# rojas-diego/tokengeex

Measured on AMD Instinct MI355X. Metric: MB/s raw bytes encoded (and tokens/s) at 32K/64K vocab, 1/2/4/8 GPUs, higher is better.
Workload: dtype f64

## Files before the change

include/tgx.h:

```cpp
#ifndef TGX_H
#define TGX_H

#include <stddef.h>
#include <stdint.h>

#ifdef __cplusplus
extern "C" {
#endif

#define TGX_ABI_VERSION 1

typedef enum tgx_status {
    TGX_OK = 0,
    TGX_ERR_IO = 1,
    TGX_ERR_JSON = 2,
    TGX_ERR_TOKEN_ID_OOB = 3,
    TGX_ERR_NO_PATH = 4,
    TGX_ERR_DEVICE = 5,
    TGX_ERR_Z_NOT_NORMAL = 6,
    TGX_ERR_INVALID = 7,
    TGX_ERR_UNSUPPORTED = 8
} tgx_status;

#define TGX_MAX_TOKEN_LEN 64
// ... 180 lines not shown
const void *tgx_text_bytes_device(const tgx_text *t);
const void *tgx_text_offsets_device(const tgx_text *t);
void tgx_text_free(tgx_text *t);
tgx_status tgx_corpus_from_text(const tgx_text *t, tgx_corpus **out);
tgx_status tgx_decode_rows_host(const uint8_t *vocab_bytes, const uint64_t *vocab_offs, uint32_t vocab_size,
                                const uint8_t *special_bytes, const uint64_t *special_offs, uint32_t n_specials,
                                const void *ids, uint32_t id_kind, const uint64_t *id_offs, uint64_t n_rows,
                                uint64_t row_len, const uint8_t *mask, const int32_t *lengths, uint32_t skip_id,
                                int include_special, uint8_t **out_text, uint64_t *out_offs, uint64_t *n_replaced,
                                uint64_t *bad_sample, uint64_t *bad_id);

#define TGX_SPAN_CHARS 8u
tgx_status tgx_result_spans_device(tgx_model *m, const tgx_result *r, const uint8_t *special_bytes,
                                   const uint64_t *special_offs, uint32_t n_specials, uint32_t flags, void *stream,
                                   void *d_spans);
tgx_status tgx_result_pad_spans_device(tgx_model *m, const tgx_result *r, const uint8_t *special_bytes,
                                       const uint64_t *special_offs, uint32_t n_specials, uint32_t row_len,
                                       uint32_t bos_id, uint32_t eos_id, uint32_t flags, void *stream, void *d_spans);
tgx_status tgx_spans_host(const uint8_t *vocab_bytes, const uint64_t *vocab_offs, uint32_t vocab_size,
                          const uint8_t *special_bytes, const uint64_t *special_offs, uint32_t n_specials,
                          const uint32_t *ids, const uint64_t *offs, uint64_t n_rows, uint32_t row_len,
                          uint32_t bos_id, uint32_t eos_id, uint32_t flags, void *out);

tgx_status tgx_corpus_upload(int device, const uint8_t *text, const uint64_t *offs,
                             uint64_t n_samples, tgx_corpus **out);
void tgx_corpus_free(tgx_corpus *c);
uint64_t tgx_corpus_num_samples(const tgx_corpus *c);
uint64_t tgx_corpus_num_bytes(const tgx_corpus *c);

tgx_status tgx_encode_corpus(tgx_model *m, tgx_corpus *c, double dropout, uint64_t seed,
                             tgx_result **out);

double tgx_sample_u01(uint64_t seed, uint64_t sample, uint64_t pos, uint32_t len);
tgx_status tgx_encode_batch_sample(tgx_model *m, const uint8_t *text, const uint64_t *offs,
                                   uint64_t n_samples, double alpha, uint64_t seed,
                                   double *logz, tgx_result **out);
tgx_status tgx_encode_corpus_sample(tgx_model *m, tgx_corpus *c, double alpha, uint64_t seed,
                                    double *logz, tgx_result **out);

#define TGX_MAX_NBEST 16
tgx_status tgx_encode_batch_nbest(tgx_model *m, const uint8_t *text, const uint64_t *offs, uint64_t n_samples,
                                  uint32_t nbest, double *scores, uint32_t *n_found, tgx_result **out);
tgx_status tgx_encode_corpus_nbest(tgx_model *m, tgx_corpus *c, uint32_t nbest,
                                   double *scores, uint32_t *n_found, tgx_result **out);

tgx_status tgx_count_tokens(tgx_model *m, tgx_corpus *c, uint64_t *freq);

tgx_status tgx_count_pairs(tgx_model *m, tgx_corpus *c, uint64_t **keys, uint64_t **counts,
                           uint64_t *n_pairs);
tgx_status tgx_count_pairs_top(tgx_model *m, tgx_corpus *c, uint64_t max_pairs, uint64_t **keys,
                               uint64_t **counts, uint64_t *n_pairs, uint64_t *n_total);

tgx_status tgx_estep(tgx_model *m, tgx_corpus *c, uint64_t snippet_len, double dropout,
                     uint64_t seed, double *expected, double *logz_sum);

void tgx_free(void *p);
void tgx_pool_trim(int device);
void *tgx_host_alloc(uint64_t bytes);
void tgx_host_free(void *p);

double tgx_digamma(double x);
tgx_status tgx_prune_m_step(const double *expected, const uint8_t *keep, uint32_t vocab_size,
                            uint32_t *out_idx, double *out_score, uint32_t *out_n);
tgx_status tgx_prune_alternatives(const tgx_flat_trie *trie, const uint8_t *bytes, const uint64_t *offs,
                                  const double *scores, uint32_t vocab_size, uint8_t *always_keep,
                                  uint32_t *alt_offs, uint32_t **alt_ids);
tgx_status tgx_model_prune_alternatives(const tgx_model *m, uint8_t *always_keep, uint32_t *alt_offs, uint32_t **alt_ids);
tgx_status tgx_prune_select(const uint64_t *freq, const uint8_t *keep, const uint8_t *always_keep,
                            const uint32_t *alt_offs, const uint32_t *alt_ids, const double *scores,
                            uint32_t vocab_size, uint64_t n_samples, uint32_t pruned_size,
                            uint32_t *out_idx, uint32_t *out_n);

int tgx_last_kernel_times(const tgx_model *m, const char **names, float *ms, int cap);
uint64_t tgx_last_algorithmic_bytes(const tgx_model *m);
uint32_t tgx_last_encode_waves_per_cu(const tgx_model *m);
uint64_t tgx_last_encode_redo_samples(const tgx_model *m);
uint64_t tgx_last_encode_long_samples(const tgx_model *m);
uint64_t tgx_last_estep_pieces(const tgx_model *m);
uint64_t tgx_last_estep_redo(const tgx_model *m);
uint32_t tgx_last_encode_corun_cus(const tgx_model *m);
uint32_t tgx_encode_corun_timeouts(const tgx_model *m);
uint32_t tgx_model_score_values(const tgx_model *m);
uint32_t tgx_last_encode_hot_values(const tgx_model *m);

static inline double tgx_dropout_u01(uint64_t seed, uint64_t sample, uint64_t pos, uint32_t len) {
    uint64_t x = seed ^ (sample * 0x9E3779B97F4A7C15ULL) ^ (pos * 0xC2B2AE3D27D4EB4FULL) ^
                 ((uint64_t)len * 0x165667B19E3779F9ULL);
    x ^= x >> 30;
    x *= 0xBF58476D1CE4E5B9ULL;
    x ^= x >> 27;
    x *= 0x94D049BB133111EBULL;
    x ^= x >> 31;
    return (double)(x >> 11) * (1.0 / 9007199254740992.0);
}

#ifdef __cplusplus
}
#endif
#endif
```

tokengeex_amd/_lib.py:

```python
from __future__ import annotations

import ctypes as C
import os

import numpy as np

_HERE = os.path.dirname(os.path.abspath(__file__))
LIB_PATH = os.path.join(_HERE, "libtgx.so")

OK, ERR_IO, ERR_JSON, ERR_TOKEN_ID_OOB, ERR_NO_PATH, ERR_DEVICE, ERR_Z_NOT_NORMAL, ERR_INVALID, \
    ERR_UNSUPPORTED = range(9)
MAX_TOKEN_LEN = 64
MAX_NBEST = 16
ESTEP_SNIPPET_LEN = 81920
NO_ID = 0xFFFFFFFF
LAYOUT_PAD_LEFT, LAYOUT_TRUNC_LEFT, LAYOUT_I64 = 1, 2, 4
FRONT_CRLF = 1
SPAN_CHARS = 8

_vp, _u64, _u32, _i, _d = C.c_void_p, C.c_uint64, C.c_uint32, C.c_int, C.c_double
_pvp, _pu64 = C.POINTER(C.c_void_p), C.POINTER(C.c_uint64)
SYMBOLS = {
    "tgx_last_error": (C.c_char_p, []),
    "tgx_last_error_detail": (None, [_pu64, _pu64, _pu64]),
    "tgx_abi_version": (_i, []),
    "tgx_device_count": (_i, []),
    "tgx_model_create": (_i, [_vp, _vp, _vp, _u32, _i, _pvp]),
    "tgx_model_create_ex": (_i, [_vp, _vp, _vp, _u32, _i, _u32, _pvp]),
    "tgx_model_create_derived": (_i, [_vp, _vp, _u32, _vp, _u32, _pvp]),
    "tgx_model_destroy": (None, [_vp]),
    "tgx_model_vocab_size": (_u32, [_vp]),
    "tgx_model_max_token_len": (_u32, [_vp]),
    "tgx_model_trie_bytes": (_u64, [_vp]),
    "tgx_model_device": (_i, [_vp]),
    "tgx_common_prefix_search": (_i, [_vp, _vp, _u64, _vp, _vp, _u64, _pu64]),
    "tgx_flat_trie_build": (_i, [_vp, _vp, _vp, _u32, _pvp]),
    "tgx_flat_trie_free": (None, [_vp]),
    "tgx_flat_trie_search": (_u64, [_vp, _vp, _u64, _vp, _vp, _u64]),
    "tgx_flat_trie_search8": (_u64, [_vp, _vp, _vp, _vp, _u32, _vp, _u64, _vp, _vp, _u64, C.POINTER(C.c_uint32), _pu64,
                                     C.POINTER(C.c_double)]),
    "tgx_flat_trie_stats": (None, [_vp, _pu64, _pu64, C.POINTER(C.c_uint32)]),
    "tgx_flat_trie_copy": (None, [_vp, _vp, _vp, _vp]),
    "tgx_tok_hash_selftest": (_i, [_vp, _vp, _u32, C.POINTER(C.c_uint32), _pu64]),
    "tgx_dropout_u01_host": (_d, [_u64, _u64, _u64, _u32]),
    "tgx_encode_batch": (_i, [_vp, _vp, _vp, _u64, _d, _u64, _pvp]),
    "tgx_encode_batch_host": (_i, [_vp, _vp, _vp, _u64, _d, _u64, _vp, _u64, _vp, _pu64]),
    "tgx_encode_batch_multi": (_i, [_vp, _u32, _vp, _vp, _u64, _d, _u64, _vp, _u64, _vp, _pu64]),
    "tgx_result_num_samples": (_u64, [_vp]),
    "tgx_result_num_tokens": (_u64, [_vp]),
    "tgx_result_ids": (_vp, [_vp]),
    "tgx_result_offsets": (_vp, [_vp]),
    "tgx_result_copy_ids": (_i, [_vp, _vp, _u64]),
    "tgx_result_copy_offsets": (_i, [_vp, _vp, _u64]),
    "tgx_result_ids_device": (_vp, [_vp]),
    "tgx_result_offsets_device": (_vp, [_vp]),
    "tgx_result_free": (None, [_vp]),
    "tgx_corpus_upload": (_i, [_i, _vp, _vp, _u64, _pvp]),
    "tgx_corpus_free": (None, [_vp]),
    "tgx_corpus_num_samples": (_u64, [_vp]),
    "tgx_corpus_num_bytes": (_u64, [_vp]),
    "tgx_encode_corpus": (_i, [_vp, _vp, _d, _u64, _pvp]),
    "tgx_count_tokens": (_i, [_vp, _vp, _vp]),
    "tgx_count_pairs": (_i, [_vp, _vp, _pvp, _pvp, _pu64]),
    "tgx_count_pairs_top": (_i, [_vp, _vp, _u64, _pvp, _pvp, _pu64, _pu64]),
    "tgx_estep": (_i, [_vp, _vp, _u64, _d, _u64, _vp, C.POINTER(C.c_double)]),
    "tgx_split_specials": (_i, [_vp, _vp, _u64, _vp, _vp, _u32, _vp, _pvp, _pvp, _pvp, _pu64]),
    "tgx_pack_segments": (_i, [_vp, _vp, _vp, _vp, _u64, _i, _vp, _vp, _pu64]),
    "tgx_normalize_segments": (_i, [_u32, _vp, _vp, _vp, _u64, _pvp, _pvp]),
    "tgx_unidata_version": (C.c_char_p, []),
    "tgx_assemble_ids": (_i, [_vp, _vp, _u64, _vp, _vp, _u32, _vp, _vp]),
    "tgx_decode_batch": (_i, [_vp, _vp, _u32, _vp, _vp, _u32, _vp, _vp, _u64, _i, _pvp, _vp, _pu64, _pu64]),
    "tgx_utf8_lossy": (_u64, [_vp, _u64, _vp]),
    "tgx_substring_df": (_i, [_i, _vp, _u64, _vp, _vp, _vp, _vp, _u64, _u32, _d, _u64, _pvp, _pvp, _pvp, _pu64, _pu64, _pu64]),
    "tgx_substring_df_top": (_i, [_i, _vp, _u64, _vp, _vp, _vp, _vp, _u64, _u32, _d, _u64, _u64, _pvp, _pvp, _pvp, _pu64, _pu64, _pu64,
                                  _pu64, C.POINTER(C.c_uint32)]),
    "tgx_generate_u01": (_d, [_u64, _u64, _u64]),
    "tgx_free": (None, [_vp]),
    "tgx_pool_trim": (None, [_i]),
    "tgx_host_alloc": (_vp, [_u64]),
    "tgx_host_free": (None, [_vp]),
    "tgx_digamma": (_d, [_d]),
    "tgx_prune_m_step": (_i, [_vp, _vp, _u32, _vp, _vp, C.POINTER(C.c_uint32)]),
    "tgx_prune_alternatives": (_i, [_vp, _vp, _vp, _vp, _u32, _vp, _vp, _pvp]),
    "tgx_model_prune_alternatives": (_i, [_vp, _vp, _vp, _pvp]),
    "tgx_prune_select": (_i, [_vp, _vp, _vp, _vp, _vp, _vp, _u32, _u64, _u32, _vp, C.POINTER(C.c_uint32)]),
    "tgx_last_kernel_times": (_i, [_vp, C.POINTER(C.c_char_p), C.POINTER(C.c_float), _i]),
    "tgx_last_algorithmic_bytes": (_u64, [_vp]),
    "tgx_last_encode_waves_per_cu": (_u32, [_vp]),
    "tgx_last_encode_redo_samples": (_u64, [_vp]),
    "tgx_model_score_values": (_u32, [_vp]),
    "tgx_last_encode_hot_values": (_u32, [_vp]),
    "tgx_last_encode_long_samples": (_u64, [_vp]),
    "tgx_last_estep_pieces": (_u64, [_vp]),
    "tgx_last_estep_redo": (_u64, [_vp]),
    "tgx_last_encode_corun_cus": (_u32, [_vp]),
    "tgx_encode_corun_timeouts": (_u32, [_vp]),
    "tgx_sample_u01": (_d, [_u64, _u64, _u64, _u32]),
    "tgx_encode_batch_sample": (_i, [_vp, _vp, _vp, _u64, _d, _u64, _vp, _pvp]),
    "tgx_encode_corpus_sample": (_i, [_vp, _vp, _d, _u64, _vp, _pvp]),
    "tgx_encode_batch_nbest": (_i, [_vp, _vp, _vp, _u64, _u32, _vp, _vp, _pvp]),
    "tgx_encode_corpus_nbest": (_i, [_vp, _vp, _u32, _vp, _vp, _pvp]),
    "tgx_result_device": (_i, [_vp]),
    "tgx_result_layout_info": (_i, [_vp, _u32, _u32, _pu64, _pu64]),
    "tgx_result_pad_device": (_i, [_vp, _u32, _u32, _u32, _u32, _u32, _vp, _vp, _vp, _vp, _pu64]),
    "tgx_result_pack_device": (_i, [_vp, _u32, _u32, _u32, _u32, _u32, _vp, _vp, _vp, _vp, _pu64]),
    "tgx_layout_pad_host": (_i, [_vp, _vp, _u64, _u32, _u32, _u32, _u32, _u32, _vp, _vp, _vp, _pu64]),
    "tgx_layout_pack_host": (_i, [_vp, _vp, _u64, _u32, _u32, _u32, _u32, _u32, _vp, _vp, _vp, _pu64]),
    "tgx_assemble_result": (_i, [_vp, _vp, _vp, _vp, _u64, _u32, _pvp]),
    "tgx_result_vocab_size": (_u32, [_vp]),
    "tgx_assemble_host": (_i, [_vp, _vp, _u64, _vp, _vp, _u64, _u32, _u32, _vp, _u64, _vp]),
    "tgx_decode_result": (_i, [_vp, _vp, _vp, _vp, _u32, _i, _vp, _pvp, _pu64, _pu64]),
    "tgx_decode_padded": (_i, [_vp, _vp, _u64, _u64, _u32, _vp, _vp, _u32, _vp, _vp, _u32, _i, _vp, _pvp, _pu64, _pu64]),
    "tgx_text_num_rows": (_u64, [_vp]),
    "tgx_text_num_bytes": (_u64, [_vp]),
    "tgx_text_num_replaced": (_u64, [_vp]),
    "tgx_text_device": (_i, [_vp]),
    "tgx_text_copy_bytes": (_i, [_vp, _vp, _u64]),
    "tgx_text_copy_offsets": (_i, [_vp, _vp, _u64]),
    "tgx_text_bytes_device": (_vp, [_vp]),
    "tgx_text_offsets_device": (_vp, [_vp]),
    "tgx_text_free": (None, [_vp]),
    "tgx_corpus_from_text": (_i, [_vp, _pvp]),
    "tgx_decode_rows_host": (_i, [_vp, _vp, _u32, _vp, _vp, _u32, _vp, _u32, _vp, _u64, _u64, _vp, _vp, _u32, _i, _pvp, _vp, _pu64,
                                  _pu64, _pu64]),
    "tgx_result_spans_device": (_i, [_vp, _vp, _vp, _vp, _u32, _u32, _vp, _vp]),
    "tgx_result_pad_spans_device": (_i, [_vp, _vp, _vp, _vp, _u32, _u32, _u32, _u32, _u32, _vp, _vp]),
    "tgx_spans_host": (_i, [_vp, _vp, _u32, _vp, _vp, _u32, _vp, _vp, _u64, _u32, _u32, _u32, _u32, _vp]),
    "tgx_result_window_info": (_i, [_vp, _u32, _u32, _u32, _u32, _u32, _pu64]),
    "tgx_result_window_pad_device": (_i, [_vp, _u32, _u32, _u32, _u32, _u32, _u32, _vp, _u64, _vp, _vp, _vp, _vp, _vp]),
    "tgx_result_window_spans_device": (_i, [_vp, _vp, _vp, _vp, _u32, _u32, _u32, _u32, _u32, _u32, _vp, _u64, _vp]),
    "tgx_layout_windows_host": (_i, [_vp, _vp, _u64, _u32, _u32, _u32, _u32, _u32, _u32, _u64, _vp, _vp, _vp, _vp, _vp, _pu64]),
    "tgx_window_spans_host": (_i, [_vp, _vp, _u32, _vp, _vp, _u32, _vp, _vp, _u64, _u32, _u32, _u32, _u32, _u32, _u64, _vp, _pu64]),
    "tgx_corpus_split_specials": (_i, [_vp, _vp, _vp, _u32, _u32, _pvp, _pvp]),
    "tgx_plan_num_samples": (_u64, [_vp]),
    "tgx_plan_num_segments": (_u64, [_vp]),
    "tgx_plan_num_encoded": (_u64, [_vp]),
    "tgx_plan_device": (_i, [_vp]),
    "tgx_plan_copy": (_i, [_vp, _vp, _u64, _vp, _u64]),
    "tgx_plan_free": (None, [_vp]),
    "tgx_assemble_result_plan": (_i, [_vp, _vp, _vp, _u32, _pvp]),
    "tgx_front_last_times": (_i, [C.POINTER(C.c_char_p), C.POINTER(C.c_float), _i]),
    "tgx_corpus_copy_text": (_i, [_vp, _vp, _u64]),
    "tgx_corpus_copy_offsets": (_i, [_vp, _vp, _u64]),
    "tgx_front_host": (_i, [_vp, _vp, _u64, _vp, _vp, _u32, _u32, _vp, _pvp, _pu64, _pvp, _pvp, _pu64]),
}


class TokenGeeXError(Exception):

    def __init__(self, message: str, status: int = -1, sample: int | None = None,
                 pos: int | None = None, length: int | None = None):
        super().__init__(message)
        self.status, self.sample, self.pos, self.length = status, sample, pos, length


def _share_torch_hip_runtime() -> None:
    import sys
    if os.environ.get("TGX_HIP_RUNTIME", "") == "system" or "torch" in sys.modules:
        return
    import importlib.util
    try:
        spec = importlib.util.find_spec("torch")
    except (ImportError, ValueError):
        return
    for root in (spec.submodule_search_locations or []) if spec else []:
        path = os.path.join(root, "lib", "libamdhip64.so")
        if os.path.exists(path):
            try:
                C.CDLL(path, mode=C.RTLD_GLOBAL)
            except OSError:
                pass
            return


# ... 880 lines not shown
        scores = np.empty(max(n * int(nbest), 1), np.float64)
        n_found = np.empty(max(n, 1), np.uint32)
        h = C.c_void_p()
        check(lib.tgx_encode_batch_nbest(self._h, ptr(flat) if flat.size else None, ptr(offs), n, int(nbest), ptr(scores),
                                         ptr(n_found), C.byref(h)))
        return NativeResult(h), scores[:n * int(nbest)], n_found[:n]

    def encode_corpus_nbest(self, corpus: NativeCorpus, nbest: int):
        n = corpus.num_samples
        scores = np.empty(max(n * int(nbest), 1), np.float64)
        n_found = np.empty(max(n, 1), np.uint32)
        h = C.c_void_p()
        check(lib.tgx_encode_corpus_nbest(self._h, corpus._h, int(nbest), ptr(scores), ptr(n_found), C.byref(h)))
        return NativeResult(h), scores[:n * int(nbest)], n_found[:n]

    def count_tokens(self, corpus: NativeCorpus, freq: np.ndarray | None = None) -> np.ndarray:
        if freq is None:
            freq = np.zeros(self.vocab_size, np.uint64)
        assert freq.dtype == np.uint64 and freq.shape[0] == self.vocab_size and freq.flags.c_contiguous
        check(lib.tgx_count_tokens(self._h, corpus._h, ptr(freq)))
        return freq

    def count_pairs(self, corpus: NativeCorpus) -> tuple[np.ndarray, np.ndarray]:
        keys, counts, n = C.c_void_p(), C.c_void_p(), C.c_uint64()
        check(lib.tgx_count_pairs(self._h, corpus._h, C.byref(keys), C.byref(counts), C.byref(n)))
        k = n.value
        ka = np.ctypeslib.as_array(C.cast(keys, C.POINTER(C.c_uint64)), shape=(max(k, 1),))[:k].copy()
        ca = np.ctypeslib.as_array(C.cast(counts, C.POINTER(C.c_uint64)), shape=(max(k, 1),))[:k].copy()
        lib.tgx_free(keys)
        lib.tgx_free(counts)
        return ka, ca

    def count_pairs_top(self, corpus: NativeCorpus, max_pairs: int) -> tuple[np.ndarray, np.ndarray, int]:
        keys, counts, n, tot = C.c_void_p(), C.c_void_p(), C.c_uint64(), C.c_uint64()
        check(lib.tgx_count_pairs_top(self._h, corpus._h, int(max_pairs), C.byref(keys), C.byref(counts),
                                      C.byref(n), C.byref(tot)))
        k = n.value
        ka = np.ctypeslib.as_array(C.cast(keys, C.POINTER(C.c_uint64)), shape=(max(k, 1),))[:k].copy()
        ca = np.ctypeslib.as_array(C.cast(counts, C.POINTER(C.c_uint64)), shape=(max(k, 1),))[:k].copy()
        lib.tgx_free(keys)
        lib.tgx_free(counts)
        return ka, ca, tot.value

    def estep(self, corpus: NativeCorpus, snippet_len: int = ESTEP_SNIPPET_LEN, dropout: float = 0.0,
              seed: int = 0, expected: np.ndarray | None = None) -> tuple[np.ndarray, float]:
        if expected is None:
            expected = np.zeros(self.vocab_size, np.float64)
        assert expected.dtype == np.float64 and expected.shape[0] == self.vocab_size
        z = C.c_double()
        check(lib.tgx_estep(self._h, corpus._h, snippet_len, float(dropout), seed & (2**64 - 1),
                            ptr(expected), C.byref(z)))
        return expected, z.value

    def common_prefix_search(self, s: bytes) -> list[tuple[int, int]]:
        buf = np.frombuffer(s, dtype=np.uint8)
        cap = len(s) + 1
        ids, lens = np.zeros(cap, np.uint32), np.zeros(cap, np.uint32)
        cnt = C.c_uint64()
        check(lib.tgx_common_prefix_search(self._h, ptr(buf) if len(s) else None, len(s), ptr(ids),
                                           ptr(lens), cap, C.byref(cnt)))
        return [(int(ids[i]), int(lens[i])) for i in range(cnt.value)]

    def last_kernel_times(self) -> dict[str, float]:
        names = (C.c_char_p * 8)()
        ms = (C.c_float * 8)()
        n = lib.tgx_last_kernel_times(self._h, names, ms, 8)
        return {names[i].decode(): float(ms[i]) for i in range(n)}

    def last_algorithmic_bytes(self) -> int:
        return lib.tgx_last_algorithmic_bytes(self._h)

    def last_encode_waves_per_cu(self) -> int:
        return lib.tgx_last_encode_waves_per_cu(self._h)

    def last_encode_redo_samples(self) -> int:
        return lib.tgx_last_encode_redo_samples(self._h)

    def score_values(self) -> int:
        return lib.tgx_model_score_values(self._h)

    def last_encode_hot_values(self) -> int:
        return lib.tgx_last_encode_hot_values(self._h)

    def last_encode_long_samples(self) -> int:
        return lib.tgx_last_encode_long_samples(self._h)

    def last_estep_pieces(self) -> int:
        return lib.tgx_last_estep_pieces(self._h)

    def last_estep_redo(self) -> int:
        return lib.tgx_last_estep_redo(self._h)

    def last_encode_corun_cus(self) -> int:
        return lib.tgx_last_encode_corun_cus(self._h)

    def encode_corun_timeouts(self) -> int:
        return lib.tgx_encode_corun_timeouts(self._h)


class FlatTrie:

    def __init__(self, tokens: list[bytes], scores):
        flat, offs = pack(tokens)
        sc = np.ascontiguousarray(scores, dtype=np.float64)
        h = C.c_void_p()
        check(lib.tgx_flat_trie_build(ptr(flat) if flat.size else None, ptr(offs), ptr(sc), len(tokens),
                                      C.byref(h)))
        self._h = h
        self._flat, self._offs, self._sc = flat, offs, sc

    def common_prefix_search8(self, s: bytes, max_hot: int = 6600):
        buf = np.frombuffer(s, dtype=np.uint8)
        cap = len(s) + 1
        ids, lens = np.zeros(cap, np.uint32), np.zeros(cap, np.uint32)
        nh, nc, cov = C.c_uint32(), C.c_uint64(), C.c_double()
        k = lib.tgx_flat_trie_search8(self._h, ptr(self._flat) if self._flat.size else None, ptr(self._offs), ptr(self._sc),
                                      max_hot, ptr(buf) if len(s) else None, len(s), ptr(ids), ptr(lens), cap,
                                      C.byref(nh), C.byref(nc), C.byref(cov))
        if k == 2**64 - 1:
            raise TokenGeeXError("8-byte records need fewer than 2^23 slots")
        return [(int(ids[i]), int(lens[i])) for i in range(k)], {"n_hot": nh.value, "n_cold": nc.value, "hot_coverage": cov.value}

    def __del__(self):
        if getattr(self, "_h", None):
            lib.tgx_flat_trie_free(self._h)
            self._h = None

    def common_prefix_search(self, s: bytes) -> list[tuple[int, int]]:
        buf = np.frombuffer(s, dtype=np.uint8)
        cap = len(s) + 1
        ids, lens = np.zeros(cap, np.uint32), np.zeros(cap, np.uint32)
        k = lib.tgx_flat_trie_search(self._h, ptr(buf) if len(s) else None, len(s), ptr(ids), ptr(lens), cap)
        return [(int(ids[i]), int(lens[i])) for i in range(k)]

    def stats(self) -> dict:
        a, b, c = C.c_uint64(), C.c_uint64(), C.c_uint32()
        lib.tgx_flat_trie_stats(self._h, C.byref(a), C.byref(b), C.byref(c))
        return {"n_slots": a.value, "n_nodes": b.value, "max_token_len": c.value,
                "fill": b.value / max(1, a.value)}

    @property
    def max_token_len(self) -> int:
        return self.stats()["max_token_len"]

    def table(self):
        n = self.stats()["n_slots"]
        check, base, tokid = np.zeros(n, np.uint32), np.zeros(n, np.uint32), np.zeros(n, np.uint32)
        lib.tgx_flat_trie_copy(self._h, ptr(check), ptr(base), ptr(tokid))
        return check, base, tokid


    def prune_alternatives(self, tokens: list[bytes], scores) -> tuple[np.ndarray, np.ndarray, np.ndarray]:
        flat, offs = pack(tokens)
        sc = np.ascontiguousarray(scores, dtype=np.float64)
        V = len(tokens)
        always_keep = np.zeros(V, np.uint8)
        alt_offs = np.zeros(V + 1, np.uint32)
        p = C.c_void_p()
        check(lib.tgx_prune_alternatives(self._h, ptr(flat) if flat.size else None, ptr(offs), ptr(sc), V,
                                         ptr(always_keep), ptr(alt_offs), C.byref(p)))
        k = int(alt_offs[V])
        ids = np.ctypeslib.as_array(C.cast(p, C.POINTER(C.c_uint32)), shape=(max(k, 1),))[:k].copy()
        lib.tgx_free(p)
        return always_keep, alt_offs, ids


# ... 58 lines not shown
```

tokengeex_amd/build.py:

```python
from __future__ import annotations

import os
import shutil
import subprocess
import sys

HERE = os.path.dirname(os.path.abspath(__file__))
CSRC = os.path.join(HERE, "csrc")
OUT = os.path.join(HERE, "libtgx.so")
SOURCES = ["kernels.hip", "estep.hip", "encode2.hip", "encode4l.hip", "encode5.hip", "estep4.hip", "estep4l.hip", "estep7.hip", "cuts.hip", "pairs.hip", "generate.hip", "sample.hip", "nbest.hip", "layout.hip", "assemble.hip", "decode.hip", "spans.hip", "front.hip", "tgx_api.cpp", "host_twins.cpp", "trie_build.cpp", "prune_host.cpp", "frontback.cpp", "unicode_norm.cpp"]
HEADERS = ["api_internal.h", "kernels.h", "sample.h", "nbest.h", "layout.h", "assemble.h", "decode.h", "spans.h", "front.h", "device_common.h", "trace_body.h", "trie_build.h", "unicode_tables.h", os.path.join("..", "..", "include", "tgx.h")]
ARCH = "gfx950"


def _hipcc() -> str:
    for cand in (os.environ.get("HIPCC"), shutil.which("hipcc"), "/opt/rocm/bin/hipcc"):
        if cand and os.path.exists(cand):
            return cand
    raise RuntimeError("hipcc not found")


def needs_build() -> bool:
    if not os.path.exists(OUT):
        return True
    t = os.path.getmtime(OUT)
    deps = [os.path.join(CSRC, f) for f in SOURCES + HEADERS] + [os.path.abspath(__file__)]
    return any(os.path.getmtime(d) > t for d in deps)


SYNTH_OUT = os.path.join(HERE, "libtgx_synth.so")


def build_synth(force: bool = False) -> str:
    src = os.path.join(CSRC, "synth_gen.c")
    if not force and os.path.exists(SYNTH_OUT) and os.path.getmtime(SYNTH_OUT) >= os.path.getmtime(src):
        return SYNTH_OUT
    subprocess.check_call(["gcc", "-O2", "-std=c11", "-fPIC", "-shared", "-o", SYNTH_OUT + ".tmp", src, "-lm"])
    os.replace(SYNTH_OUT + ".tmp", SYNTH_OUT)
    return SYNTH_OUT


FAST_OUT = os.path.join(HERE, "_tgxfast.so")


def build_pyfast(force: bool = False) -> str:
    import sysconfig
    src = os.path.join(CSRC, "pyfast.c")
    if not force and os.path.exists(FAST_OUT) and os.path.getmtime(FAST_OUT) >= os.path.getmtime(src):
        return FAST_OUT
    inc = sysconfig.get_paths()["include"]
    subprocess.check_call(["gcc", "-O2", "-std=c11", "-fPIC", "-shared", "-pthread", "-I", inc, "-o", FAST_OUT + ".tmp", src])
    os.replace(FAST_OUT + ".tmp", FAST_OUT)
    return FAST_OUT


def build(force: bool = False, verbose: bool = False) -> str:
    from concurrent.futures import ThreadPoolExecutor
    build_synth(force)
    build_pyfast(force)
    if not force and not needs_build():
        return OUT
    objdir = os.path.join(CSRC, "build")
    os.makedirs(objdir, exist_ok=True)
    hdr_time = max(os.path.getmtime(os.path.join(CSRC, h)) for h in HEADERS)
    hdr_time = max(hdr_time, os.path.getmtime(os.path.abspath(__file__)))
    flags = [f"--offload-arch={ARCH}", "-O3", "-std=c++17", "-fPIC",
             "-ffp-contract=off",
             "-munsafe-fp-atomics",
             "-Wall", "-Wno-unused-result", "-Wno-pass-failed", "-x", "hip"]
    flags += os.environ.get("TGX_EXTRA_HIPCC_FLAGS", "").split()
    jobs = []
    objs = []
    for s in SOURCES:
        src = os.path.join(CSRC, s)
        obj = os.path.join(objdir, s + ".o")
        objs.append(obj)
        if force or not os.path.exists(obj) or os.path.getmtime(obj) < max(os.path.getmtime(src), hdr_time):
            jobs.append([_hipcc()] + flags + ["-c", src, "-o", obj])

    def run(cmd):
        if verbose:
            print(" ".join(cmd), flush=True)
        subprocess.check_call(cmd)

    with ThreadPoolExecutor(max_workers=min(6, max(1, len(jobs)))) as ex:
        list(ex.map(run, jobs))
    link = [_hipcc(), f"--offload-arch={ARCH}", "-shared", "-fPIC"] + objs + ["-o", OUT + ".tmp", "-Wl,-rpath,/opt/rocm/lib"]
    if verbose:
        print(" ".join(link), flush=True)
    subprocess.check_call(link)
    os.replace(OUT + ".tmp", OUT)
    return OUT


# ... 3 lines not shown
```

tokengeex_amd/csrc/device_common.h:

```cpp
#pragma once
#include <hip/hip_runtime.h>
#include <stdint.h>

namespace tgx {

__device__ __forceinline__ uint32_t readlane_u32(uint32_t v, uint32_t lane) {
    return (uint32_t)__builtin_amdgcn_readlane((int)v, (int)lane);
}
__device__ __forceinline__ uint64_t readlane_u64(uint64_t v, uint32_t lane) {
    uint32_t lo = readlane_u32((uint32_t)v, lane);
    uint32_t hi = readlane_u32((uint32_t)(v >> 32), lane);
    return ((uint64_t)hi << 32) | lo;
}
__device__ __forceinline__ double readlane_f64(double v, uint32_t lane) {
    return __longlong_as_double((long long)readlane_u64((uint64_t)__double_as_longlong(v), lane));
}
__device__ __forceinline__ uint64_t first_u64(uint64_t v) {
    uint32_t lo = (uint32_t)__builtin_amdgcn_readfirstlane((int)(uint32_t)v);
    uint32_t hi = (uint32_t)__builtin_amdgcn_readfirstlane((int)(uint32_t)(v >> 32));
    return ((uint64_t)hi << 32) | lo;
}
__device__ __forceinline__ uint64_t rotl64(uint64_t x, uint32_t r) {
    r &= 63u;
    return (x << r) | (x >> ((64u - r) & 63u));
}

__device__ __forceinline__ double dropout_u01(uint64_t seed, uint64_t sample, uint64_t pos, uint32_t len) {
    uint64_t x = seed ^ (sample * 0x9E3779B97F4A7C15ULL) ^ (pos * 0xC2B2AE3D27D4EB4FULL) ^
                 ((uint64_t)len * 0x165667B19E3779F9ULL);
    x ^= x >> 30;
    x *= 0xBF58476D1CE4E5B9ULL;
    x ^= x >> 27;
    x *= 0x94D049BB133111EBULL;
    x ^= x >> 31;
    return (double)(x >> 11) * (1.0 / 9007199254740992.0);
}

template <class T>
__device__ __forceinline__ T lds_ld(uint32_t off) { return *(const __attribute__((address_space(3))) T*)(uintptr_t)off; }
template <class T>
__device__ __forceinline__ void lds_st(uint32_t off, T v) { *(__attribute__((address_space(3))) T*)(uintptr_t)off = v; }

typedef uint32_t u32x2_t __attribute__((ext_vector_type(2)));
typedef uint32_t u32x4_t __attribute__((ext_vector_type(4)));
__device__ __forceinline__ __amdgpu_buffer_rsrc_t make_rsrc(const void* base, uint32_t bytes) {
    return __builtin_amdgcn_make_buffer_rsrc(const_cast<void*>(base), 0, (int)bytes, 0x00020000);
}
__device__ __forceinline__ uint2 buf_ld8(__amdgpu_buffer_rsrc_t rs, uint32_t off) {
    const u32x2_t v = __builtin_amdgcn_raw_buffer_load_b64(rs, (int)off, 0, 0);
    return make_uint2(v.x, v.y);
}
__device__ __forceinline__ double buf_ld_f64(__amdgpu_buffer_rsrc_t rs, uint32_t off) {
    const u32x2_t v = __builtin_amdgcn_raw_buffer_load_b64(rs, (int)off, 0, 0);
    return __hiloint2double((int)v.y, (int)v.x);
}


constexpr uint32_t kFront = 2;
__host__ __device__ inline uint32_t wave_lds_entries(uint32_t lm) { return 64u * lm + 64u + kFront; }
__host__ __device__ inline uint32_t wave_lds_bytes(uint32_t lm) {
    return wave_lds_entries(lm) * 12u + 128u;
}

__device__ __forceinline__ uint32_t sel_u32(uint64_t mask, uint32_t t, uint32_t f) {
    uint32_t r;
    asm("v_cndmask_b32_e64 %0, %1, %2, %3" : "=v"(r) : "v"(f), "v"(t), "s"(mask));
    return r;
}
template <int IMM>
__device__ __forceinline__ uint32_t sel_imm_u32(uint64_t mask, uint32_t f) {
    uint32_t r;
    asm("v_cndmask_b32_e64 %0, %1, %2, %3" : "=v"(r) : "v"(f), "n"(IMM), "s"(mask));
    return r;
}
__device__ __forceinline__ double sel_f64(uint64_t mask, double t, double f) {
    const uint64_t tb = (uint64_t)__double_as_longlong(t), fb = (uint64_t)__double_as_longlong(f);
    const uint32_t lo = sel_u32(mask, (uint32_t)tb, (uint32_t)fb);
    const uint32_t hi = sel_u32(mask, (uint32_t)(tb >> 32), (uint32_t)(fb >> 32));
    return __longlong_as_double((long long)(((uint64_t)hi << 32) | lo));
}


template <int CTRL>
__device__ __forceinline__ uint32_t row_bcast_u32(uint32_t v) {
    return (uint32_t)__builtin_amdgcn_update_dpp(0, (int)v, CTRL, 0xF, 0xF, false);
}
template <int U>
__device__ __forceinline__ double row_bcast_f64(double v) {
    double r;
    asm volatile("s_nop 1\n\tv_mov_b64_dpp %0, %1 row_newbcast:%2 row_mask:0xf bank_mask:0xf"
                 : "=v"(r) : "v"(v), "n"(U));
    return r;
}

constexpr uint64_t kRowLane0 = 0x0001000100010001ULL;

__device__ __forceinline__ uint64_t wave_fetch_add(unsigned long long* counter, uint32_t n) {
    uint64_t got, saved;
    const uint64_t inc = n;
    const uint32_t zero = 0;
    asm volatile(
        "s_mov_b64 %1, exec\n\t"
        "s_mov_b64 exec, 1\n\t"
        "global_atomic_add_x2 %0, %2, %3, %4 sc0\n\t"
        "s_mov_b64 exec, %1\n\t"
        "s_waitcnt vmcnt(0)"
        : "=&v"(got), "=&s"(saved) : "v"(zero), "v"(inc), "s"(counter) : "memory");
    const uint32_t lo = (uint32_t)__builtin_amdgcn_readfirstlane((int)(uint32_t)got);
    const uint32_t hi = (uint32_t)__builtin_amdgcn_readfirstlane((int)(uint32_t)(got >> 32));
    return ((uint64_t)hi << 32) | lo;
}

__device__ __forceinline__ uint64_t claim_rows(unsigned long long* queue, bool need_new, uint32_t r) {
    const uint64_t want = __builtin_amdgcn_ballot_w64(need_new) & kRowLane0;
    uint64_t k = ~0ull;
    if (want != 0) {
        const uint64_t base = wave_fetch_add(queue, (uint32_t)__builtin_popcountll(want));
        if (need_new) k = base + (uint64_t)__builtin_popcountll(want & ((1ull << (r * 16u)) - 1ull));
    }
    return k;
}

__device__ __forceinline__ uint64_t claim_rows_chunk(unsigned long long* queue, bool need_new, uint32_t r, uint32_t chunk) {
    const uint64_t want = __builtin_amdgcn_ballot_w64(need_new) & kRowLane0;
    uint64_t k = ~0ull;
    if (want != 0) {
        const uint64_t base = wave_fetch_add(queue, (uint32_t)__builtin_popcountll(want) * chunk);
        if (need_new) k = base + (uint64_t)__builtin_popcountll(want & ((1ull << (r * 16u)) - 1ull)) * chunk;
    }
    return k;
}

__device__ __forceinline__ uint4 load_rec(const uint4* __restrict__ trie, uint32_t t) {
    uint4 r = trie[t];
    asm volatile("" : "+v"(r.x), "+v"(r.y), "+v"(r.z), "+v"(r.w));
    return r;
}

__device__ __forceinline__ uint64_t bp8_base(uint64_t beg, uint32_t s) { return (beg + 128ull * s) & ~3ull; }
__device__ __forceinline__ uint32_t bp8_perm(uint32_t j) { return (j & ~63u) | ((j & 15u) << 2) | ((j >> 4) & 3u); }


constexpr uint32_t kNoStep = 0xFFu;

template <int U>
__device__ __forceinline__ void relax4_step(double sv, double& acc, uint32_t& bpv, uint32_t& fin, uint32_t& fhi) {
    constexpr uint64_t MU = kRowLane0 << U;
    const double best = row_bcast_f64<U>(acc);
    fin = sel_u32(MU, bpv, fin);
    fhi = sel_u32(MU, (uint32_t)((uint64_t)__double_as_longlong(acc) >> 32), fhi);
    const double cand = best + sv;
    const uint64_t take = __builtin_amdgcn_fcmp(cand, acc, 2 ) | MU;
    acc = sel_f64(take, cand, acc);
    bpv = sel_imm_u32<U>(take, bpv);
}

template <int U>
__device__ __forceinline__ void relax5_step(double sv, double& acc, uint32_t& bpv, uint32_t& fin, uint32_t& fhi) {
    constexpr uint64_t MU = kRowLane0 << U;
    const double best = row_bcast_f64<U>(acc);
    fin = sel_u32(MU, bpv, fin);
    fhi = sel_u32(MU, (uint32_t)((uint64_t)__double_as_longlong(acc) >> 32), fhi);
    const double acc_r = sel_f64(MU, -__builtin_huge_val(), acc);
    const double cand = best + sv;
    const uint64_t take = __builtin_amdgcn_fcmp(cand, acc_r, 2 );
    asm("v_max_f64 %0, %1, %2" : "=v"(acc) : "v"(acc_r), "v"(cand));
    bpv = sel_imm_u32<U>(take, bpv);
}


__device__ __forceinline__ uint32_t rotl32_dev(uint32_t x, int r) { return __builtin_rotateleft32(x, (uint32_t)r); }
__device__ __forceinline__ uint64_t tok_hash64_dev(uint32_t w0, uint32_t w1, uint32_t w2, uint32_t w3, uint32_t len, uint32_t seed) {
    uint32_t a = (w0 ^ (len << 27) ^ seed) * 0x85EBCA6Bu;
    a ^= a >> 15;
    uint32_t b = a;
    a = (a + w1) * 0xC2B2AE35u;
    a ^= a >> 13;
    b = rotl32_dev(b, 11) ^ a;
    a = (a + w2) * 0x27D4EB2Fu;
    a ^= a >> 16;
    b = rotl32_dev(b, 11) ^ a;
    a = (a + w3) * 0x165667B1u;
    a ^= a >> 15;
    b = rotl32_dev(b, 11) + (w0 ^ rotl32_dev(w1, 8) ^ rotl32_dev(w2, 16) ^ rotl32_dev(w3, 24));
    return ((uint64_t)b << 32) | a;
}


__device__ __forceinline__ uint64_t tok_hash64_long_dev(const uint32_t* w, uint32_t len, uint32_t seed) {
    uint32_t a = (w[0] ^ (len << 27) ^ seed) * 0x85EBCA6Bu;
    a ^= a >> 15;
    uint32_t b = a;
    a = (a + w[1]) * 0xC2B2AE35u;
    a ^= a >> 13;
    b = rotl32_dev(b, 11) ^ a;
    a = (a + w[2]) * 0x27D4EB2Fu;
    a ^= a >> 16;
    b = rotl32_dev(b, 11) ^ a;
    a = (a + w[3]) * 0x165667B1u;
    a ^= a >> 15;
    b = rotl32_dev(b, 11) + (w[0] ^ rotl32_dev(w[1], 8) ^ rotl32_dev(w[2], 16) ^ rotl32_dev(w[3], 24));
    if (len > 16u) {
        a = (a + w[4]) * 0x85EBCA6Bu;
        a ^= a >> 15;
        b = rotl32_dev(b, 11) ^ a;
        a = (a + w[5]) * 0xC2B2AE35u;
        a ^= a >> 13;
        b = rotl32_dev(b, 11) ^ a;
        a = (a + w[6]) * 0x27D4EB2Fu;
        a ^= a >> 16;
        b = rotl32_dev(b, 11) ^ a;
        a = (a + w[7]) * 0x165667B1u;
        a ^= a >> 15;
        b = rotl32_dev(b, 11) + (w[4] ^ rotl32_dev(w[5], 8) ^ rotl32_dev(w[6], 16) ^ rotl32_dev(w[7], 24));
    }
    return ((uint64_t)b << 32) | a;
}


__device__ __forceinline__ int row_max_exponent(double acc) {
    int e = (acc == 0.0) ? -100000 : __builtin_amdgcn_frexp_exp(acc);
    e = max(e, __builtin_amdgcn_update_dpp(e, e, 0x121, 0xF, 0xF, false));
    e = max(e, __builtin_amdgcn_update_dpp(e, e, 0x122, 0xF, 0xF, false));
    e = max(e, __builtin_amdgcn_update_dpp(e, e, 0x124, 0xF, 0xF, false));
    e = max(e, __builtin_amdgcn_update_dpp(e, e, 0x128, 0xF, 0xF, false));
    return e;
}

template <int U>
__device__ __forceinline__ void e4l_fwd_step(double sv, double& acc, double& fin) {
    constexpr uint64_t MU = kRowLane0 << U;
    fin = sel_f64(MU, acc, fin);
    const double best = row_bcast_f64<U>(acc);
    const double cand = best * sv;
    acc = sel_f64(MU, cand, acc + cand);
}


}
```

tokengeex_amd/csrc/encode5.hip:

```cpp
#include <hip/hip_runtime.h>
#include <stdint.h>

#include <type_traits>

#include "device_common.h"
#include "kernels.h"

namespace tgx {

constexpr uint32_t kE5RowStride = 512;
constexpr uint32_t kE5GroupBytes = 4 * kE5RowStride;

template <int PPL>
struct WalkCtx {
    __amdgpu_buffer_rsrc_t trie;
    uint32_t s, l32;
    double dropout;
    uint64_t seed;
    bool estep_rule = false;
};

struct Res5 {
    __amdgpu_buffer_rsrc_t cold;
    uint32_t tab;
// ... 79 lines not shown
            uint32_t base[PPL], n_alive = 0;
#pragma unroll
            for (int g = 0; g < PPL; ++g) {
                bm[g] = __builtin_amdgcn_ballot_w64(alive[g]);
                base[g] = n_alive;
                n_alive += (uint32_t)__builtin_popcountll(bm[g]);
            }
            if (n_alive <= 64u) {
                pack<1>(W, R, bytes, maxd, wlane, alive, off_cut, bm, base, n_alive);
                return;
            }
            if (PPL >= 3 && n_alive <= 128u) {
                pack<(PPL >= 3 ? 2 : 1)>(W, R, bytes, maxd, wlane, alive, off_cut, bm, base, n_alive);
                return;
            }
#pragma unroll
            for (int g = 0; g < PPL; ++g) rec[g] = buf_ld8(W.trie, alive[g] ? off_cut[g] : 0u);
            Walk5<DROPOUT, LONG, RES, PPL, D + 1, SKIP, 0, PK>::run(W, R, bytes, maxd, pg, wlane, alive, rec, c);
        } else {
            Walk5<DROPOUT, LONG, RES, PPL, D + 1, SKIP, CK, PK>::run(W, R, bytes, maxd, pg, wlane, alive, rec, c);
        }
    }

    template <int P2>
    static __device__ __forceinline__ void pack(const WalkCtx<PPL>& W, Res5& R, const uint32_t (&bytes)[PPL][4], const uint32_t (&maxd)[PPL],
                                                const uint32_t (&wlane)[PPL], const bool (&alive)[PPL], const uint32_t (&off)[PPL],
                                                const uint64_t (&bm)[PPL], const uint32_t (&base)[PPL], uint32_t n_alive) {
        constexpr int Q0 = CK >> 2;
        constexpr int NW = 2 + 4 - Q0;
        const uint32_t lane = __builtin_amdgcn_mbcnt_hi(~0u, __builtin_amdgcn_mbcnt_lo(~0u, 0u));
        uint32_t v2[P2][NW];
#pragma unroll
        for (int t = 0; t < P2; ++t)
#pragma unroll
            for (int i = 0; i < NW; ++i) v2[t][i] = 0u;
#pragma unroll
        for (int g = 0; g < PPL; ++g) {
            const uint32_t cnt = (uint32_t)__builtin_popcountll(bm[g]);
            const uint32_t below = __builtin_amdgcn_mbcnt_hi((uint32_t)(bm[g] >> 32), __builtin_amdgcn_mbcnt_lo((uint32_t)bm[g], 0u));
            const uint32_t dst = (base[g] + (alive[g] ? below : cnt + lane - below)) & 63u;
            uint32_t v[NW];
            v[0] = off[g];
            v[1] = (PK ? wlane[g] : (wlane[g] | W.l32)) | (maxd[g] << 24);
#pragma unroll
            for (int q = Q0; q < 4; ++q) v[2 + q - Q0] = bytes[g][q];
            const uint32_t t = (lane - base[g]) & 63u;
            const bool got = t < cnt;
            const bool hi = base[g] + t >= 64u;
#pragma unroll
            for (int i = 0; i < NW; ++i) {
                const uint32_t x = (uint32_t)__builtin_amdgcn_ds_permute((int)(dst << 2), (int)v[i]);
#pragma unroll
                for (int s2 = 0; s2 < P2; ++s2)
                    if (got && (P2 == 1 || (s2 == 1) == hi)) v2[s2][i] = x;
            }
        }
        WalkCtx<P2> W2{W.trie, W.s, W.l32, W.dropout, W.seed, W.estep_rule};
        uint32_t bytes2[P2][4], maxd2[P2], pg2[P2], wl2[P2], c2[P2];
        bool alive2[P2];
        uint2 rec2[P2];
#pragma unroll
        for (int s2 = 0; s2 < P2; ++s2) {
            alive2[s2] = 64u * (uint32_t)s2 + lane < n_alive;
            wl2[s2] = v2[s2][1] & 0xFFFFFFu;
            maxd2[s2] = v2[s2][1] >> 24;
            pg2[s2] = 0u;
#pragma unroll
            for (int q = 0; q < 4; ++q) bytes2[s2][q] = q < Q0 ? 0u : v2[s2][2 + (q < Q0 ? 0 : q - Q0)];
            c2[s2] = (bytes2[s2][Q0] >> ((CK & 3) * 8)) & 0xFFu;
            rec2[s2] = buf_ld8(W.trie, alive2[s2] ? v2[s2][0] : 0u);
        }
        Walk5<DROPOUT, LONG, RES, P2, CK, SKIP, 0, true>::run(W2, R, bytes2, maxd2, pg2, wl2, alive2, rec2, c2);
    }
};
template <bool DROPOUT, bool LONG, bool RES, int PPL, bool SKIP, int CK, bool PK>
struct Walk5<DROPOUT, LONG, RES, PPL, 16, SKIP, CK, PK> {
    static __device__ __forceinline__ void run(const WalkCtx<PPL>&, Res5& R, const uint32_t (&)[PPL][4], const uint32_t (&)[PPL],
                                               const uint32_t (&)[PPL], const uint32_t (&)[PPL], bool (&)[PPL], uint2 (&)[PPL],
                                               uint32_t (&)[PPL]) {
        if (RES) R.complete();
    }
};

template <int N>
__device__ __forceinline__ void e5_scores_issue(uint32_t tab, const uint32_t (&iw)[8], int first, u32x2_t (&sp)[N]) {
#pragma unroll
    for (int u = 0; u < N; ++u) {
        const int v = first + u;
        const uint32_t a = (v & 1) ? ((iw[v >> 1] >> 16) << 3) : ((iw[v >> 1] & 0xFFFFu) << 3);
        sp[u] = lds_ld<u32x2_t>(tab + a);
    }
}
__device__ __forceinline__ double e5_score_value(const u32x2_t& p) { return __hiloint2double((int)p.y, (int)p.x); }

template <int N>
__device__ __forceinline__ void e5_scores_cold(uint32_t tab, __amdgpu_buffer_rsrc_t cold, const uint32_t (&iw)[8], int first,
                                               uint32_t hot_bytes, double (&sv)[N]) {
    uint32_t a[N];
#pragma unroll
    for (int u = 0; u < N; ++u) {
        const int v = first + u;
        a[u] = (v & 1) ? ((iw[v >> 1] >> 16) << 3) : ((iw[v >> 1] & 0xFFFFu) << 3);
        sv[u] = lds_ld<double>(tab + (a[u] < hot_bytes ? a[u] : 0u));
    }
    static_assert(N == 4 || N == 8, "e5_scores_cold: four or eight values at a time");
    if (N == 8) asm volatile("" : "+v"(sv[0]), "+v"(sv[1]), "+v"(sv[2]), "+v"(sv[3]), "+v"(sv[4 % N]), "+v"(sv[5 % N]), "+v"(sv[6 % N]), "+v"(sv[7 % N]));
    else asm volatile("" : "+v"(sv[0]), "+v"(sv[1]), "+v"(sv[2]), "+v"(sv[3]));
#pragma unroll
    for (int u = 0; u < N; ++u)
        if (a[u] >= hot_bytes) sv[u] = buf_ld_f64(cold, a[u] - hot_bytes);
}

template <bool COLD>
__device__ __forceinline__ double e5_score_one(uint32_t tab, __amdgpu_buffer_rsrc_t cold, uint32_t rank, uint32_t hot_bytes) {
    const uint32_t a = rank << 3;
    double v = lds_ld<double>(tab + ((!COLD || a < hot_bytes) ? a : 0u));
    if (COLD) {
        asm volatile("" : "+v"(v));
        if (a >= hot_bytes) v = buf_ld_f64(cold, a - hot_bytes);
    }
    return v;
}

constexpr uint32_t kE5LongCap = 62;
constexpr uint32_t kE5LongBytes = 8u + kE5LongCap * 4u;
constexpr uint32_t kFarCode = 0x80u;

__device__ __forceinline__ uint32_t e5_winner_len_m1(uint32_t code, uint32_t l) {
    return (code & kFarCode) ? (code & 31u) : ((l - code - 1u) & 15u);
}

template <int U>
__device__ __forceinline__ void relax5l_step(double sv, double& acc, uint32_t& bpv, double& far, uint32_t& fbp, uint32_t& fin, double& fval) {
    constexpr uint64_t MU = kRowLane0 << U;
    fin = sel_u32(MU, bpv, fin);
    fval = sel_f64(MU, acc, fval);
    const double best = row_bcast_f64<U>(acc);
    const double cur = sel_f64(MU, far, acc);
    const uint32_t curbp = sel_u32(MU, fbp, bpv);
    far = sel_f64(MU, -__builtin_huge_val(), far);
    const double cand = best + sv;
    const uint64_t take = __builtin_amdgcn_fcmp(cand, cur, 2 );
    asm("v_max_f64 %0, %1, %2" : "=v"(acc) : "v"(cur), "v"(cand));
    bpv = sel_imm_u32<U>(take, curbp);
}

template <bool DROPOUT>
__device__ __forceinline__ void e5_long_tail(__amdgpu_buffer_rsrc_t trie, const uint8_t* __restrict__ text16, uint32_t rec_x, bool alive,
                                             uint32_t maxd, uint32_t lane, uint32_t g, uint32_t list_off, double dropout, uint64_t seed,
                                             uint32_t s, uint32_t pg) {
    bool more = alive && maxd > 16u;
    if (__builtin_amdgcn_ballot_w64(more) == 0) return;
    struct __attribute__((packed, aligned(1))) Bytes16 { uint32_t w[4]; };
    Bytes16 b{{0u, 0u, 0u, 0u}};
    if (more) b = *reinterpret_cast<const Bytes16*>(text16);
    uint32_t x = rec_x;
#pragma unroll 1
    for (uint32_t d = 16u; d < 32u; ++d) {
        more = more && d < maxd;
        if (__builtin_amdgcn_ballot_w64(more) == 0) break;
        const uint32_t bi = d - 16u;
        const uint32_t word = (bi & 8u) ? ((bi & 4u) ? b.w[3] : b.w[2]) : ((bi & 4u) ? b.w[1] : b.w[0]);
        const uint32_t c = (word >> ((bi & 3u) * 8u)) & 0xFFu;
        const uint2 rec = buf_ld8(trie, more ? ((x ^ (c << 3)) & 0xFFFFFFu) : 0u);
        more = more && (rec.x >> 24) == c;
        const uint32_t rank = rec.y & 0xFFFFu;
        bool term = more && rank != 0u;
        if (DROPOUT) {
            if (term) term = dropout < dropout_u01(seed, s, pg, d + 1u);
        }
        if (term) {
            const uint32_t slot = __hip_atomic_fetch_add((__attribute__((address_space(3))) uint32_t*)(uintptr_t)list_off, 1u, __ATOMIC_RELAXED, __HIP_MEMORY_SCOPE_WORKGROUP);
            if (slot < kE5LongCap) lds_st<uint32_t>(list_off + 8u + slot * 4u, lane | (g << 6) | (d << 8) | (rank << 16));
        }
        x = rec.x;
    }
}

#define E5_STAMP(i)                                                    \
    if (P.stamps) {                                                    \
        __builtin_amdgcn_sched_barrier(0);                             \
        const uint64_t _now = (uint64_t)__builtin_amdgcn_s_memtime(); \
        __builtin_amdgcn_s_waitcnt(0xC07F);                            \
        __builtin_amdgcn_sched_barrier(0);                             \
        seg[i] += _now - t_last;                                       \
        t_last = _now;                                                 \
    }

template <bool DROPOUT, bool COLD, int PPL, bool LONG, int CK = 0>
__global__ __launch_bounds__(1024, (PPL == 1 ? 8 : (PPL == 2 ? 6 : (PPL == 3 ? 4 : 1)))) void encode5_kernel(EncodeParams P, Encode5Params Q) {
    static_assert(!LONG || PPL == 4, "the long-token build runs four positions per lane");
    extern __shared__ __align__(16) unsigned char smem[];
    constexpr uint32_t LM = LONG ? 32 : 16;
    constexpr uint32_t SPAN = 16u * PPL;
    const uint32_t lane = threadIdx.x & 63u;
    const uint32_t l = lane & 15u, r = lane >> 4;
    const uint32_t wave = threadIdx.x >> 6;
    const uint2* __restrict__ trie = reinterpret_cast<const uint2*>(Q.trie8);
    const __amdgpu_buffer_rsrc_t trie_b = make_rsrc(Q.trie8, Q.trie_bytes);
    const uint32_t lds0 = (uint32_t)reinterpret_cast<uintptr_t>(smem);
    double* const score_tab = reinterpret_cast<double*>(smem);
    const uint32_t hot_bytes = 8u * (Q.n_hot + 1u);
    const __amdgpu_buffer_rsrc_t values = make_rsrc(reinterpret_cast<const unsigned char*>(Q.values) + hot_bytes, 8u * (Q.n_values - Q.n_hot));
    const uint2* rootc = reinterpret_cast<const uint2*>(smem + Q.root_off);
    unsigned char* wbase = smem + Q.idx_off + (size_t)wave * (PPL * kE5GroupBytes);
    {
        for (uint32_t i = threadIdx.x; i <= Q.n_hot; i += blockDim.x) score_tab[i] = Q.values[i];
        uint2* rw = reinterpret_cast<uint2*>(smem + Q.root_off);
        for (uint32_t i = threadIdx.x; i < 256u; i += blockDim.x) rw[i] = trie[(Q.root_base & ~255u) + i];
        if (Q.started && threadIdx.x == 0u) __hip_atomic_fetch_add(Q.started, 1u, __ATOMIC_RELAXED, __HIP_MEMORY_SCOPE_SYSTEM);
        __syncthreads();
    }
    const __amdgpu_buffer_rsrc_t cold_values = values;

    uint32_t s = 0, n = 0, p0 = 0;
    uint64_t beg = 0;
    bool live = false, need_new = true;
    const double ninf = -__builtin_huge_val();
    double acc = ninf, far = ninf;
    uint32_t bpv = kNoStep, fbp = kFarCode;
    bool redo = false;
    uint32_t wn[4 * PPL + 1];
    uint32_t pk = 0, pk_j = 0;
    bool pk_dirty = false;
#pragma unroll
    for (int q = 0; q <= 4 * PPL; ++q) wn[q] = 0;
    const uint32_t my_col = r * kE5RowStride + ((l - 1u) & 15u) * 32u;
    const uint32_t wbase_off = lds0 + Q.idx_off + wave * (PPL * kE5GroupBytes);
    const uint32_t wr_off = wbase_off + r * kE5RowStride + l * 2u;
    const uint32_t col_off = wbase_off + my_col;
    const uint32_t list_off = lds0 + Q.list_off + wave * ((kE5LongBytes + 15u) & ~15u);
    uint64_t seg[5] = {0, 0, 0, 0, 0};
    uint64_t t_last = P.stamps ? (uint64_t)__builtin_amdgcn_s_memtime() : 0;
    uint32_t iters = 0;

    uint64_t local_next = 0, local_end = 0;
    for (;;) {
        {
            uint64_t k = ~0ull;
            const bool have_local = need_new && local_next < local_end;
            if (have_local) k = local_next++;
            const uint64_t kc = claim_rows_chunk(P.queue, need_new && !have_local, r, Q.claim_chunk);
            if (need_new && !have_local) {
                k = kc;
                local_next = kc + 1u;
                local_end = kc + Q.claim_chunk;
            }
            if (need_new) {
                live = k < P.n_samples;
                if (live) {
                    s = P.order[k];
                    beg = P.offs[s];
                    n = (uint32_t)(P.offs[s + 1] - beg);
                }
            }
        }
        if (need_new) {
            p0 = 0;
            acc = (l == 0u) ? 0.0 : ninf;
            bpv = kNoStep;
            pk_dirty = false;
            if (LONG) {
                far = ninf;
                fbp = kFarCode;
                redo = false;
            }
        }
        const bool fresh_row = need_new;
        need_new = false;
        if (__builtin_amdgcn_ballot_w64(live) == 0) break;
        iters++;
        E5_STAMP(0)

        const uintptr_t addr = reinterpret_cast<uintptr_t>(P.text + (live ? beg + p0 + l : 0));
        const uint32_t sh = (uint32_t)(addr & 3u);
        const uint32_t* __restrict__ wp = reinterpret_cast<const uint32_t*>(addr & ~uintptr_t(3));
        uint32_t w[4 * PPL + 1];
        if (fresh_row) {
#pragma unroll
            for (int q = 0; q <= 4 * PPL; ++q) w[q] = wp[q];
        } else {
#pragma unroll
            for (int q = 0; q <= 4 * PPL; ++q) w[q] = wn[q];
        }
        uint32_t bytes[PPL][4];
#pragma unroll
        for (int g = 0; g < PPL; ++g)
#pragma unroll
            for (int q = 0; q < 4; ++q) bytes[g][q] = __builtin_amdgcn_alignbyte(w[4 * g + q + 1], w[4 * g + q], sh);

#pragma unroll
        for (int g = 0; g < PPL; ++g) {
            uint4* mine = reinterpret_cast<uint4*>(wbase + g * kE5GroupBytes + my_col);
            mine[0] = make_uint4(0, 0, 0, 0);
            mine[1] = make_uint4(0, 0, 0, 0);
        }
        if (LONG && lane == 0u) lds_st<uint32_t>(list_off, 0u);
        __builtin_amdgcn_wave_barrier();
        E5_STAMP(1)

        uint32_t pg[PPL], maxd[PPL];
        uint32_t wlane[PPL];
        bool alive[PPL];
        uint2 rec[PPL];
        uint32_t c[PPL];
#pragma unroll
        for (int g = 0; g < PPL; ++g) {
            pg[g] = p0 + 16u * g + l;
            const uint32_t rem = (live && pg[g] < n) ? (n - pg[g]) : 0u;
            maxd[g] = rem < LM ? rem : LM;
            alive[g] = maxd[g] > 0 && !(P.flags & 1u);
            wlane[g] = wr_off + g * kE5GroupBytes;
            c[g] = bytes[g][0] & 0xFFu;
            rec[g] = rootc[(Q.root_base ^ c[g]) & 255u];
        }
        {
            uint32_t l32 = l * 32u;
            asm volatile("" : "+v"(l32));
            WalkCtx<PPL> W{trie_b, s, l32, P.dropout, P.seed};
            Res5 no_res{};
            Walk5<DROPOUT, LONG, false, PPL, 0, COLD && PPL < 4, CK>::run(W, no_res, bytes, maxd, pg, wlane, alive, rec, c);
        }
        if (LONG) {
#pragma unroll
            for (int g = 0; g < PPL; ++g)
                e5_long_tail<DROPOUT>(trie_b, P.text + (live ? beg + pg[g] + 16u : 0), rec[g].x, alive[g], maxd[g], lane, (uint32_t)g, list_off,
                                      P.dropout, P.seed, s, pg[g]);
        }
        __builtin_amdgcn_wave_barrier();
        E5_STAMP(2)
        {
            const uint32_t* __restrict__ np = wp + 4 * PPL;
#pragma unroll
            for (int q = 0; q <= 4 * PPL; ++q) wn[q] = np[q];
        }

        if (!(P.flags & 32u)) __builtin_amdgcn_s_setprio(0);
        uint32_t fin[PPL];
        bool reached[PPL];
        if (!(P.flags & 2u)) {
            uint32_t iw[8], iwn[8];
            auto load_iw = [&](int g, uint32_t (&w)[8]) {
                const u32x4_t ia = lds_ld<u32x4_t>(col_off + g * kE5GroupBytes), ib = lds_ld<u32x4_t>(col_off + g * kE5GroupBytes + 16u);
                w[0] = ia.x; w[1] = ia.y; w[2] = ia.z; w[3] = ia.w;
                w[4] = ib.x; w[5] = ib.y; w[6] = ib.z; w[7] = ib.w;
            };
            u32x2_t sa[4], sb[4];
            load_iw(0, iw);
            if (!COLD) e5_scores_issue<4>(lds0, iw, 0, sa);
#pragma unroll
            for (int g = 0; g < PPL; ++g) {
                uint32_t (&cw)[8] = (g & 1) ? iwn : iw;
                uint32_t (&nw)[8] = (g & 1) ? iw : iwn;
                fin[g] = kNoStep;
                uint32_t fhi = 0xFFF00000u;
                bool slow = false;
                uint32_t n_list = 0;
                if (LONG) {
                    n_list = (uint32_t)__builtin_amdgcn_readfirstlane((int)lds_ld<uint32_t>(list_off));
                    slow = n_list != 0u || __builtin_amdgcn_ballot_w64((uint32_t)((uint64_t)__double_as_longlong(far) >> 32) != 0xFFF00000u) != 0;
                }
                if (LONG && slow) {
                    auto rank_of = [&](int u) { return (u & 1) ? (cw[u >> 1] >> 16) : (cw[u >> 1] & 0xFFFFu); };
                    double fval = ninf;
                    relax5l_step<0>(e5_score_one<COLD>(lds0, cold_values, rank_of(0), hot_bytes), acc, bpv, far, fbp, fin[g], fval);
                    relax5l_step<1>(e5_score_one<COLD>(lds0, cold_values, rank_of(1), hot_bytes), acc, bpv, far, fbp, fin[g], fval);
                    relax5l_step<2>(e5_score_one<COLD>(lds0, cold_values, rank_of(2), hot_bytes), acc, bpv, far, fbp, fin[g], fval);
                    relax5l_step<3>(e5_score_one<COLD>(lds0, cold_values, rank_of(3), hot_bytes), acc, bpv, far, fbp, fin[g], fval);
                    relax5l_step<4>(e5_score_one<COLD>(lds0, cold_values, rank_of(4), hot_bytes), acc, bpv, far, fbp, fin[g], fval);
                    relax5l_step<5>(e5_score_one<COLD>(lds0, cold_values, rank_of(5), hot_bytes), acc, bpv, far, fbp, fin[g], fval);
                    relax5l_step<6>(e5_score_one<COLD>(lds0, cold_values, rank_of(6), hot_bytes), acc, bpv, far, fbp, fin[g], fval);
                    relax5l_step<7>(e5_score_one<COLD>(lds0, cold_values, rank_of(7), hot_bytes), acc, bpv, far, fbp, fin[g], fval);
                    relax5l_step<8>(e5_score_one<COLD>(lds0, cold_values, rank_of(8), hot_bytes), acc, bpv, far, fbp, fin[g], fval);
                    relax5l_step<9>(e5_score_one<COLD>(lds0, cold_values, rank_of(9), hot_bytes), acc, bpv, far, fbp, fin[g], fval);
                    relax5l_step<10>(e5_score_one<COLD>(lds0, cold_values, rank_of(10), hot_bytes), acc, bpv, far, fbp, fin[g], fval);
                    relax5l_step<11>(e5_score_one<COLD>(lds0, cold_values, rank_of(11), hot_bytes), acc, bpv, far, fbp, fin[g], fval);
                    relax5l_step<12>(e5_score_one<COLD>(lds0, cold_values, rank_of(12), hot_bytes), acc, bpv, far, fbp, fin[g], fval);
                    relax5l_step<13>(e5_score_one<COLD>(lds0, cold_values, rank_of(13), hot_bytes), acc, bpv, far, fbp, fin[g], fval);
                    relax5l_step<14>(e5_score_one<COLD>(lds0, cold_values, rank_of(14), hot_bytes), acc, bpv, far, fbp, fin[g], fval);
                    relax5l_step<15>(e5_score_one<COLD>(lds0, cold_values, rank_of(15), hot_bytes), acc, bpv, far, fbp, fin[g], fval);
                    const uint32_t cnt = n_list < kE5LongCap ? n_list : kE5LongCap;
#pragma unroll 1
                    for (uint32_t i = 0; i < cnt; ++i) {
                        const uint32_t e = (uint32_t)__builtin_amdgcn_readfirstlane((int)lds_ld<uint32_t>(list_off + 8u + i * 4u));
                        if (((e >> 6) & 3u) != (uint32_t)g) continue;
                        const uint32_t src = e & 63u, d = (e >> 8) & 31u;
                        const double score = e5_score_one<COLD>(lds0, cold_values, e >> 16, hot_bytes);
                        const double cand = readlane_f64(fval, src) + score;
                        const uint32_t tt = (src & 15u) + d + 1u;
                        const bool mine = (lane >> 4) == (src >> 4) && l == (tt & 15u);
                        const bool to_far = tt >= 32u;
                        const double curv = to_far ? far : acc;
                        const uint32_t curc = to_far ? fbp : bpv;
                        const bool longer = !(curc & kFarCode) || d > (curc & 31u);
                        const bool take = mine && (cand > curv || (cand == curv && longer));
                        if (take && to_far) {
                            far = cand;
                            fbp = kFarCode | d;
                        }
                        if (take && !to_far) {
                            acc = cand;
                            bpv = kFarCode | d;
                        }
                    }
                    reached[g] = fval > ninf;
                    if (g + 1 < PPL) {
                        load_iw(g + 1, nw);
                        if (!COLD) e5_scores_issue<4>(lds0, nw, 0, sa);
                    }
                    continue;
                }
                if (COLD) {
                    double sv[8], sw[8];
                    e5_scores_cold<8>(lds0, cold_values, cw, 0, hot_bytes, sv);
                    e5_scores_cold<8>(lds0, cold_values, cw, 8, hot_bytes, sw);
                    if (g + 1 < PPL) load_iw(g + 1, nw);
                    relax5_step<0>(sv[0], acc, bpv, fin[g], fhi);
                    relax5_step<1>(sv[1], acc, bpv, fin[g], fhi);
                    relax5_step<2>(sv[2], acc, bpv, fin[g], fhi);
                    relax5_step<3>(sv[3], acc, bpv, fin[g], fhi);
                    relax5_step<4>(sv[4], acc, bpv, fin[g], fhi);
                    relax5_step<5>(sv[5], acc, bpv, fin[g], fhi);
                    relax5_step<6>(sv[6], acc, bpv, fin[g], fhi);
                    relax5_step<7>(sv[7], acc, bpv, fin[g], fhi);
                    relax5_step<8>(sw[0], acc, bpv, fin[g], fhi);
                    relax5_step<9>(sw[1], acc, bpv, fin[g], fhi);
                    relax5_step<10>(sw[2], acc, bpv, fin[g], fhi);
                    relax5_step<11>(sw[3], acc, bpv, fin[g], fhi);
                    relax5_step<12>(sw[4], acc, bpv, fin[g], fhi);
                    relax5_step<13>(sw[5], acc, bpv, fin[g], fhi);
                    relax5_step<14>(sw[6], acc, bpv, fin[g], fhi);
                    relax5_step<15>(sw[7], acc, bpv, fin[g], fhi);
                } else {
                    e5_scores_issue<4>(lds0, cw, 4, sb);
                    if (g + 1 < PPL) load_iw(g + 1, nw);
                    relax5_step<0>(e5_score_value(sa[0]), acc, bpv, fin[g], fhi);
                    relax5_step<1>(e5_score_value(sa[1]), acc, bpv, fin[g], fhi);
                    relax5_step<2>(e5_score_value(sa[2]), acc, bpv, fin[g], fhi);
                    relax5_step<3>(e5_score_value(sa[3]), acc, bpv, fin[g], fhi);
                    e5_scores_issue<4>(lds0, cw, 8, sa);
                    relax5_step<4>(e5_score_value(sb[0]), acc, bpv, fin[g], fhi);
                    relax5_step<5>(e5_score_value(sb[1]), acc, bpv, fin[g], fhi);
                    relax5_step<6>(e5_score_value(sb[2]), acc, bpv, fin[g], fhi);
                    relax5_step<7>(e5_score_value(sb[3]), acc, bpv, fin[g], fhi);
                    e5_scores_issue<4>(lds0, cw, 12, sb);
                    relax5_step<8>(e5_score_value(sa[0]), acc, bpv, fin[g], fhi);
                    relax5_step<9>(e5_score_value(sa[1]), acc, bpv, fin[g], fhi);
                    relax5_step<10>(e5_score_value(sa[2]), acc, bpv, fin[g], fhi);
                    relax5_step<11>(e5_score_value(sa[3]), acc, bpv, fin[g], fhi);
                    if (g + 1 < PPL) e5_scores_issue<4>(lds0, nw, 0, sa);
                    relax5_step<12>(e5_score_value(sb[0]), acc, bpv, fin[g], fhi);
                    relax5_step<13>(e5_score_value(sb[1]), acc, bpv, fin[g], fhi);
                    relax5_step<14>(e5_score_value(sb[2]), acc, bpv, fin[g], fhi);
                    relax5_step<15>(e5_score_value(sb[3]), acc, bpv, fin[g], fhi);
                }
                reached[g] = fhi != 0xFFF00000u;
            }
        } else {
#pragma unroll
            for (int g = 0; g < PPL; ++g) {
                fin[g] = kNoStep;
                reached[g] = true;
            }
        }
        __builtin_amdgcn_wave_barrier();
        if (!(P.flags & 32u)) __builtin_amdgcn_s_setprio(2);
        E5_STAMP(3)

        uint8_t* const bpw = P.bp8 + bp8_base(beg, s);
#pragma unroll
        for (int g = 0; g < PPL; ++g)
            if (live && pg[g] >= 1u && pg[g] <= n) {
                const uint32_t b = reached[g] ? (LONG ? e5_winner_len_m1(fin[g], l) : ((l - fin[g] - 1u) & 15u)) : 0xFFu;
                const uint32_t j = pg[g] - 1u, kq = (j >> 4) & 3u;
                pk = (kq == 0u) ? b : (pk | (b << (8u * kq)));
                pk_j = j;
                pk_dirty = true;
                if (kq == 3u) {
                    __builtin_nontemporal_store(pk, reinterpret_cast<uint32_t*>(bpw + (bp8_perm(j) & ~3u)));
                    pk_dirty = false;
                }
            }
        if (LONG) {
            const uint32_t n_all = (uint32_t)__builtin_amdgcn_readfirstlane((int)lds_ld<uint32_t>(list_off));
            if (n_all > kE5LongCap) {
                if (live && !redo && l == 0u) P.redo_list[atomicAdd(P.redo_count, 1ULL)] = s;
                redo = true;
            }
        }
        if (live && n - p0 < SPAN && pk_dirty) {
            __builtin_nontemporal_store(pk, reinterpret_cast<uint32_t*>(bpw + (bp8_perm(pk_j) & ~3u)));
            pk_dirty = false;
        }
        if (live) {
            const uint32_t left = n - p0;
            if (left < SPAN) {
#pragma unroll
                for (int g = 0; g < PPL; ++g)
                    if (left == 16u * g + l) P.status[s] = (n == 0u || reached[g]) ? 1u : 0u;
                need_new = true;
            } else {
                p0 += SPAN;
            }
        }
        E5_STAMP(4)
    }
    if (P.stamps && lane == 0) {
        unsigned long long* o = P.stamps + (size_t)(blockIdx.x * (blockDim.x >> 6) + wave) * 8u;
        for (int i = 0; i < 5; ++i) o[i] = seg[i];
        o[5] = iters;
    }
}

constexpr uint32_t kE6Walkers = 3;
constexpr uint32_t kE6Slots = kE6Walkers + 2u;
struct E6Ctrl {
    uint32_t epoch;
    uint32_t s, n, trip0;
    uint64_t beg;
    uint32_t relax_done;
    uint32_t pad_;
    uint32_t walk_done[8];
    uint32_t ack[4];
    uint32_t pool_used[8];
    uint32_t pad2_[4];
};
constexpr uint32_t kE6Done = 0xFFFFFFFFu;

__device__ __forceinline__ uint32_t lds_load(const uint32_t* p) { return __hip_atomic_load(p, __ATOMIC_RELAXED, __HIP_MEMORY_SCOPE_WORKGROUP); }
__device__ __forceinline__ void lds_store(uint32_t* p, uint32_t v) { __hip_atomic_store(p, v, __ATOMIC_RELAXED, __HIP_MEMORY_SCOPE_WORKGROUP); }

template <bool COLD>
__device__ __forceinline__ void e6_load_quarter(uint32_t tab, __amdgpu_buffer_rsrc_t cold, uint32_t hot_bytes,
                                                const uint32_t (&iw)[8], int q, double (&sv)[4]) {
    if (COLD) {
        e5_scores_cold<4>(tab, cold, iw, 4 * q, hot_bytes, sv);
    } else {
        u32x2_t sp[4];
        e5_scores_issue<4>(tab, iw, 4 * q, sp);
#pragma unroll
        for (int u = 0; u < 4; ++u) sv[u] = e5_score_value(sp[u]);
    }
}

template <bool DROPOUT, bool COLD>
__global__ __launch_bounds__(64 * (1 + 4 * kE6Walkers), 8) void encode6_kernel(EncodeParams P, Encode5Params Q) {
    extern __shared__ __align__(16) unsigned char smem[];
    constexpr uint32_t LM = 16;
    constexpr uint32_t K = kE6Walkers, G = kE6Slots;
    const uint32_t lane = threadIdx.x & 63u;
    const uint32_t l = lane & 15u, r = lane >> 4;
    const uint32_t wave = (uint32_t)__builtin_amdgcn_readfirstlane((int)(threadIdx.x >> 6));
    const uint2* __restrict__ trie = reinterpret_cast<const uint2*>(Q.trie8);
    const __amdgpu_buffer_rsrc_t trie_b = make_rsrc(Q.trie8, Q.trie_bytes);
    const uint32_t lds0 = (uint32_t)reinterpret_cast<uintptr_t>(smem);
    double* const score_tab = reinterpret_cast<double*>(smem);
    const uint32_t shift = COLD ? 4u * G * Q.pool : 0u;
    const uint32_t hot_bytes = 8u * (1u + shift + Q.n_hot);
    const __amdgpu_buffer_rsrc_t values = make_rsrc(reinterpret_cast<const unsigned char*>(Q.values) + 8u * (Q.n_hot + 1u), 8u * (Q.n_values - Q.n_hot));
    const uint2* rootc = reinterpret_cast<const uint2*>(smem + Q.root_off);
    E6Ctrl* const ctrl_all = reinterpret_cast<E6Ctrl*>(smem + Q.ctrl_off);
    {
        if (threadIdx.x == 0u) score_tab[0] = Q.values[0];
        for (uint32_t i = threadIdx.x; i < shift; i += blockDim.x) score_tab[1u + i] = Q.values[0];
        for (uint32_t i = threadIdx.x; i < Q.n_hot; i += blockDim.x) score_tab[1u + shift + i] = Q.values[1u + i];
        uint2* rw = reinterpret_cast<uint2*>(smem + Q.root_off);
        for (uint32_t i = threadIdx.x; i < 256u; i += blockDim.x) rw[i] = trie[(Q.root_base & ~255u) + i];
        uint32_t* cw = reinterpret_cast<uint32_t*>(ctrl_all);
        for (uint32_t i = threadIdx.x; i < 4u * sizeof(E6Ctrl) / 4u; i += blockDim.x) cw[i] = 0u;
        uint4* ring = reinterpret_cast<uint4*>(smem + Q.ring_off);
        for (uint32_t i = threadIdx.x; i < 4u * G * kE5GroupBytes / 16u; i += blockDim.x) ring[i] = make_uint4(0, 0, 0, 0);
        __syncthreads();
    }
    const double ninf = -__builtin_huge_val();

    if (wave == 0u) {
        __builtin_amdgcn_s_setprio(3);
        E6Ctrl* const ctrl = ctrl_all + r;
        uint32_t s = 0, n = 0, n_trips = 0, tau = 0, trip0 = 0, epoch = 0, slot = 0;
        uint64_t beg = 0;
        bool live = false, need_new = true, exhausted = false;
        double acc = ninf;
        uint32_t bpv = kNoStep, pk = 0, pk_j = 0;
        bool pk_dirty = false;
        for (;;) {
            if (__builtin_amdgcn_ballot_w64(need_new) != 0) {
                for (;;) {
                    const bool read = !need_new || epoch == 0u || l >= K || lds_load(&ctrl->ack[l]) == epoch;
                    if (__builtin_amdgcn_ballot_w64(!read) == 0) break;
                    __builtin_amdgcn_s_sleep(1);
                }
                const uint64_t k = claim_rows(P.queue, need_new && !exhausted, r);
                if (need_new) {
                    live = !exhausted && k < P.n_samples;
                    if (live) {
                        s = P.order[k];
                        beg = P.offs[s];
                        n = (uint32_t)(P.offs[s + 1] - beg);
                        n_trips = n / 64u + 1u;
                        tau = 0;
                        acc = (l == 0u) ? 0.0 : ninf;
                        bpv = kNoStep;
                        pk_dirty = false;
                        if (l == 0u) {
                            ctrl->s = s;
                            ctrl->n = n;
                            ctrl->beg = beg;
                            ctrl->trip0 = trip0;
                        }
                    } else {
                        exhausted = true;
                    }
                }
                __builtin_amdgcn_fence(__ATOMIC_RELEASE, "workgroup");
                if (need_new) {
                    if (live) epoch++;
                    if (l == 0u) lds_store(&ctrl->epoch, live ? epoch : kE6Done);
                }
                need_new = false;
            }
            if (__builtin_amdgcn_ballot_w64(live) == 0) break;

            const uint32_t t = trip0 + tau;
            for (;;) {
                const bool ready = !live || lds_load(&ctrl->walk_done[slot]) == t + 1u;
                if (__builtin_amdgcn_ballot_w64(!ready) == 0) break;
                __builtin_amdgcn_s_sleep(1);
            }
            __builtin_amdgcn_fence(__ATOMIC_ACQUIRE, "workgroup");

            const uint32_t p0 = tau * 64u;
            const unsigned char* sbase = smem + Q.ring_off + (r * G + slot) * kE5GroupBytes + ((l - 1u) & 15u) * 32u;
            auto load_iw = [&](int g, uint32_t (&iw)[8]) {
                const uint4* ip = reinterpret_cast<const uint4*>(sbase + g * kE5RowStride);
                const uint4 ia = ip[0], ib = ip[1];
                iw[0] = ia.x; iw[1] = ia.y; iw[2] = ia.z; iw[3] = ia.w;
                iw[4] = ib.x; iw[5] = ib.y; iw[6] = ib.z; iw[7] = ib.w;
            };
            const double acc_in = acc;
            const uint32_t bpv_in = bpv;
            uint32_t fin[4];
            bool reached[4];
            auto relax_trip = [&](auto cold_tag) {
                constexpr bool C = decltype(cold_tag)::value;
                uint32_t iwa[8], iwb[8];
                double sva[4], svb[4];
                load_iw(0, iwa);
                e6_load_quarter<C>(lds0, values, hot_bytes, iwa, 0, sva);
#pragma unroll
                for (int g = 0; g < 4; ++g) {
                    uint32_t (&iw)[8] = (g & 1) ? iwb : iwa;
                    uint32_t (&iwn)[8] = (g & 1) ? iwa : iwb;
                    fin[g] = kNoStep;
                    uint32_t fhi = 0xFFF00000u;
                    e6_load_quarter<C>(lds0, values, hot_bytes, iw, 1, svb);
                    if (g < 3) load_iw(g + 1, iwn);
                    relax5_step<0>(sva[0], acc, bpv, fin[g], fhi);
                    relax5_step<1>(sva[1], acc, bpv, fin[g], fhi);
                    relax5_step<2>(sva[2], acc, bpv, fin[g], fhi);
                    relax5_step<3>(sva[3], acc, bpv, fin[g], fhi);
                    e6_load_quarter<C>(lds0, values, hot_bytes, iw, 2, sva);
                    relax5_step<4>(svb[0], acc, bpv, fin[g], fhi);
                    relax5_step<5>(svb[1], acc, bpv, fin[g], fhi);
                    relax5_step<6>(svb[2], acc, bpv, fin[g], fhi);
                    relax5_step<7>(svb[3], acc, bpv, fin[g], fhi);
                    e6_load_quarter<C>(lds0, values, hot_bytes, iw, 3, svb);
                    relax5_step<8>(sva[0], acc, bpv, fin[g], fhi);
                    relax5_step<9>(sva[1], acc, bpv, fin[g], fhi);
                    relax5_step<10>(sva[2], acc, bpv, fin[g], fhi);
                    relax5_step<11>(sva[3], acc, bpv, fin[g], fhi);
                    if (g < 3) e6_load_quarter<C>(lds0, values, hot_bytes, iwn, 0, sva);
                    relax5_step<12>(svb[0], acc, bpv, fin[g], fhi);
                    relax5_step<13>(svb[1], acc, bpv, fin[g], fhi);
                    relax5_step<14>(svb[2], acc, bpv, fin[g], fhi);
                    relax5_step<15>(svb[3], acc, bpv, fin[g], fhi);
                    reached[g] = fhi != 0xFFF00000u;
                }
            };
            bool unresolved = false;
            if (COLD) unresolved = live && (Q.pool == 0u || lds_load(&ctrl->pool_used[slot]) > Q.pool);
            if (COLD && __builtin_expect(__builtin_amdgcn_ballot_w64(unresolved) != 0, 0)) relax_trip(std::true_type{});
            else relax_trip(std::false_type{});
            if (!live) {
                acc = acc_in;
                bpv = bpv_in;
            }
            __builtin_amdgcn_fence(__ATOMIC_RELEASE, "workgroup");
            if (live && l == 0u) lds_store(&ctrl->relax_done, t + 1u);
            if (live) {
                uint8_t* const bpw = P.bp8 + bp8_base(beg, s);
#pragma unroll
                for (int g = 0; g < 4; ++g) {
                    const uint32_t pgq = p0 + 16u * g + l;
                    if (pgq >= 1u && pgq <= n) {
                        const uint32_t b = reached[g] ? ((l - fin[g] - 1u) & 15u) : 0xFFu;
                        const uint32_t j = pgq - 1u, kq = (j >> 4) & 3u;
                        pk = (kq == 0u) ? b : (pk | (b << (8u * kq)));
                        pk_j = j;
                        pk_dirty = true;
                        if (kq == 3u) {
                            __builtin_nontemporal_store(pk, reinterpret_cast<uint32_t*>(bpw + (bp8_perm(j) & ~3u)));
                            pk_dirty = false;
                        }
                    }
                }
                const uint32_t left = n - p0;
                if (left < 64u) {
                    if (pk_dirty) __builtin_nontemporal_store(pk, reinterpret_cast<uint32_t*>(bpw + (bp8_perm(pk_j) & ~3u)));
#pragma unroll
                    for (int g = 0; g < 4; ++g)
                        if (left == 16u * g + l) P.status[s] = (n == 0u || reached[g]) ? 1u : 0u;
                    trip0 += n_trips;
                    need_new = true;
                } else {
                    tau++;
                }
                slot = (slot + 1u == G) ? 0u : slot + 1u;
            }
        }
        return;
    }

    const uint32_t rw = (wave - 1u) & 3u, jw = (wave - 1u) >> 2;
    E6Ctrl* const ctrl = ctrl_all + rw;
    uint32_t seen = 0;
    for (;;) {
        uint32_t e;
        while ((e = lds_load(&ctrl->epoch)) == seen) __builtin_amdgcn_s_sleep(2);
        if (e == kE6Done) break;
        seen = e;
        __builtin_amdgcn_fence(__ATOMIC_ACQUIRE, "workgroup");
        const uint32_t s = ctrl->s, n = ctrl->n, trip0 = ctrl->trip0;
        const uint64_t beg = ctrl->beg;
        __builtin_amdgcn_fence(__ATOMIC_RELEASE, "workgroup");
        if (lane == 0u) lds_store(&ctrl->ack[jw], e);
        const uint32_t n_trips = n / 64u + 1u;
        const uint32_t tau0 = (jw + K - trip0 % K) % K;
        uint32_t slot = (trip0 + tau0) % G;
        for (uint32_t tau = tau0; tau < n_trips; tau += K, slot = (slot + K >= G) ? slot + K - G : slot + K) {
            const uint32_t t = trip0 + tau;
            while (t >= lds_load(&ctrl->relax_done) + G) __builtin_amdgcn_s_sleep(1);
            __builtin_amdgcn_fence(__ATOMIC_ACQUIRE, "workgroup");
            const uint32_t p0 = tau * 64u, pgl = p0 + lane;
            const uintptr_t addr = reinterpret_cast<uintptr_t>(P.text + beg + pgl);
            const uint32_t sh = (uint32_t)(addr & 3u);
            const uint32_t* __restrict__ wp = reinterpret_cast<const uint32_t*>(addr & ~uintptr_t(3));
            uint32_t wv[5];
#pragma unroll
            for (int q = 0; q < 5; ++q) wv[q] = wp[q];
            uint32_t bytes[1][4];
#pragma unroll
            for (int q = 0; q < 4; ++q) bytes[0][q] = __builtin_amdgcn_alignbyte(wv[q + 1], wv[q], sh);
            const uint32_t slot_off = Q.ring_off + (rw * G + slot) * kE5GroupBytes;
            {
// ... 166 lines not shown
                e5_scores_cold<8>(lds0, cold_values, iw, 0, hot_bytes, sv);
                e5_scores_cold<8>(lds0, cold_values, iw, 8, hot_bytes, sw);
            } else {
                u32x2_t sa[8], sb[8];
                e5_scores_issue<8>(lds0, iw, 0, sa);
                e5_scores_issue<8>(lds0, iw, 8, sb);
#pragma unroll
                for (int u = 0; u < 8; ++u) {
                    sv[u] = e5_score_value(sa[u]);
                    sw[u] = e5_score_value(sb[u]);
                }
            }
            double fin = 0.0;
            e4l_fwd_step<0>(sv[0], acc, fin);
            e4l_fwd_step<1>(sv[1], acc, fin);
            e4l_fwd_step<2>(sv[2], acc, fin);
            e4l_fwd_step<3>(sv[3], acc, fin);
            e4l_fwd_step<4>(sv[4], acc, fin);
            e4l_fwd_step<5>(sv[5], acc, fin);
            e4l_fwd_step<6>(sv[6], acc, fin);
            e4l_fwd_step<7>(sv[7], acc, fin);
            e4l_fwd_step<8>(sw[0], acc, fin);
            e4l_fwd_step<9>(sw[1], acc, fin);
            e4l_fwd_step<10>(sw[2], acc, fin);
            e4l_fwd_step<11>(sw[3], acc, fin);
            e4l_fwd_step<12>(sw[4], acc, fin);
            e4l_fwd_step<13>(sw[5], acc, fin);
            e4l_fwd_step<14>(sw[6], acc, fin);
            e4l_fwd_step<15>(sw[7], acc, fin);
            if (live && pg[g] <= n) {
                P.alpha[beg + s + pg[g]] = fin;
                if (!(fin > 0.0 && fin <= 1.7976931348623157e308)) atomicMax(P.range_flag, 1ULL);
                if (l == 0u) P.alpha_exp[ebase + (pg[g] >> 4)] = erow;
                if (pg[g] == n) {
                    const double z = log(fin) + (double)erow * 0.6931471805599453;
                    P.zarr[s] = z;
                    zsum += z;
                    const double az = fabs(z);
                    if (!(az >= 2.2250738585072014e-308 && az <= 1.7976931348623157e308)) atomicMin(P.err_snip, (unsigned long long)s);
                }
            }
            const int e = row_max_exponent(acc);
            if (e > -100000) {
                acc = ldexp(acc, -e);
                erow += e;
            }
        }
        __builtin_amdgcn_wave_barrier();
        if (live) {
            if (n - p0 < SPAN) need_new = true;
            else p0 += SPAN;
        }
    }
    if (zsum != 0.0) atomicAdd(P.logz_sum, zsum);
}

typedef void (*estep5_fn)(Estep4Params, Encode5Params);
static estep5_fn pick_estep5(bool dropout, bool cold, int ppl) {
#define TGX_E5F(D, C)                                                                        \
    (ppl == 1 ? estep5_fwd_kernel<D, C, 1> : ppl == 2 ? estep5_fwd_kernel<D, C, 2> : ppl == 3 ? estep5_fwd_kernel<D, C, 3> : estep5_fwd_kernel<D, C, 4>)
    if (dropout) return cold ? TGX_E5F(true, true) : TGX_E5F(true, false);
    return cold ? TGX_E5F(false, true) : TGX_E5F(false, false);
#undef TGX_E5F
}
hipError_t estep5_waves_per_simd(bool dropout, bool cold, int ppl, int* out) {
    hipFuncAttributes attr;
    hipError_t e = hipFuncGetAttributes(&attr, reinterpret_cast<const void*>(pick_estep5(dropout, cold, ppl)));
    if (e != hipSuccess) return e;
    const int regs = (attr.numRegs + 7) & ~7;
    *out = regs > 0 ? (512 / regs > 8 ? 8 : 512 / regs) : 8;
    return hipSuccess;
}
hipError_t launch_estep5_fwd(const Estep4Params& p, Encode5Params q, bool cold, int ppl, int waves, uint32_t blocks, hipStream_t stream) {
    const uint32_t lds = encode5_lds_layout(q.n_hot, false, waves, ppl, &q.list_off, &q.root_off, &q.idx_off);
    if (lds > 160u * 1024u || q.n_hot > q.n_values || (!cold && q.n_hot != q.n_values) || ppl < 1 || ppl > 4) return hipErrorInvalidValue;
    estep5_fn fn = pick_estep5(p.dropout > 0.0, cold, ppl);
    hipError_t e = hipFuncSetAttribute(reinterpret_cast<const void*>(fn), hipFuncAttributeMaxDynamicSharedMemorySize, 160 * 1024);
    if (e != hipSuccess) return e;
    hipLaunchKernelGGL(fn, dim3(blocks), dim3(64u * (uint32_t)waves), lds, stream, p, q);
    return hipGetLastError();
}

typedef void (*encode5_fn)(EncodeParams, Encode5Params);
static encode5_fn pick_encode5(bool dropout, bool cold, int ppl, bool long_tokens, int compact) {
    if (long_tokens) {
        if (cold) return dropout ? encode5_kernel<true, true, 4, true> : encode5_kernel<false, true, 4, true>;
        return dropout ? encode5_kernel<true, false, 4, true> : encode5_kernel<false, false, 4, true>;
    }
    if (dropout) {
        if (cold) {
            if (ppl == 1) return encode5_kernel<true, true, 1, false>;
            if (ppl == 2) return encode5_kernel<true, true, 2, false>;
            if (ppl == 3) return encode5_kernel<true, true, 3, false>;
            return encode5_kernel<true, true, 4, false>;
        }
        if (ppl == 1) return encode5_kernel<true, false, 1, false>;
        if (ppl == 2) return encode5_kernel<true, false, 2, false>;
        if (ppl == 3) return encode5_kernel<true, false, 3, false>;
        return encode5_kernel<true, false, 4, false>;
    }
#define TGX_E5K(C, PL) \
    (compact == 4 ? encode5_kernel<false, C, PL, false, 4> : compact == 5 ? encode5_kernel<false, C, PL, false, 5> \
     : compact == 6 ? encode5_kernel<false, C, PL, false, 6> : compact == 7 ? encode5_kernel<false, C, PL, false, 7> \
     : compact == 8 ? encode5_kernel<false, C, PL, false, 8> : encode5_kernel<false, C, PL, false, 0>)
    if (cold) {
        if (ppl == 1) return encode5_kernel<false, true, 1, false>;
        if (ppl == 2) return TGX_E5K(true, 2);
        if (ppl == 3) return TGX_E5K(true, 3);
        return TGX_E5K(true, 4);
    }
    if (ppl == 1) return encode5_kernel<false, false, 1, false>;
    if (ppl == 2) return TGX_E5K(false, 2);
    if (ppl == 3) return TGX_E5K(false, 3);
    return TGX_E5K(false, 4);
#undef TGX_E5K
}

uint32_t encode5_lds_layout(uint32_t n_hot, bool long_tokens, int waves, int ppl, uint32_t* list_off, uint32_t* root_off, uint32_t* idx_off) {
    const uint32_t lo = (8u * (n_hot + 1u) + 15u) & ~15u;
    const uint32_t score_bytes = lo + (long_tokens ? (uint32_t)waves * ((kE5LongBytes + 15u) & ~15u) : 0u);
    if (list_off) *list_off = lo;
    const uint32_t ro = (score_bytes + 15u) & ~15u;
    const uint32_t io = (ro + 2048u + 511u) & ~511u;
    if (root_off) *root_off = ro;
    if (idx_off) *idx_off = io;
    return io + (uint32_t)waves * (uint32_t)ppl * kE5GroupBytes;
}
uint32_t encode5_max_hot(bool long_tokens, int waves, int ppl, uint32_t budget) {
    const uint32_t fixed = encode5_lds_layout(0u, long_tokens, waves, ppl, nullptr, nullptr, nullptr) + 512u;
    return budget > fixed + 64u ? (budget - fixed) / 8u : 0u;
}

hipError_t encode5_waves_per_simd(bool dropout, bool cold, int ppl, bool long_tokens, int compact, int* out) {
    hipFuncAttributes attr;
    hipError_t e = hipFuncGetAttributes(&attr, reinterpret_cast<const void*>(pick_encode5(dropout, cold, ppl, long_tokens, compact)));
    if (e != hipSuccess) return e;
    const int regs = (attr.numRegs + 7) & ~7;
    *out = regs > 0 ? (512 / regs > 8 ? 8 : 512 / regs) : 8;
    return hipSuccess;
}

uint32_t encode6_lds_layout(uint32_t n_hot, uint32_t pool, uint32_t* root_off, uint32_t* ctrl_off, uint32_t* ring_off) {
    const uint32_t score_bytes = 8u * (1u + 4u * kE6Slots * pool + n_hot);
    const uint32_t ro = (score_bytes + 15u) & ~15u;
    const uint32_t co = ro + 2048u;
    const uint32_t go = (co + 4u * (uint32_t)sizeof(E6Ctrl) + 511u) & ~511u;
    if (root_off) *root_off = ro;
    if (ctrl_off) *ctrl_off = co;
    if (ring_off) *ring_off = go;
    return go + 4u * kE6Slots * kE5GroupBytes;
}
uint32_t encode6_pool_total(uint32_t pool) { return 4u * kE6Slots * pool; }
uint32_t encode6_max_hot(uint32_t budget, uint32_t pool) {
    const uint32_t fixed = encode6_lds_layout(0u, pool, nullptr, nullptr, nullptr) + 512u;
    return budget > fixed + 64u ? (budget - fixed) / 8u : 0u;
}
hipError_t launch_encode6(const EncodeParams& p, Encode5Params q, bool cold, uint32_t blocks, hipStream_t stream) {
    q.ring_slots = kE6Slots;
    if (!cold) q.pool = 0u;
    const uint32_t lds = encode6_lds_layout(q.n_hot, q.pool, &q.root_off, &q.ctrl_off, &q.ring_off);
    if (lds > 160u * 1024u || q.n_hot > q.n_values || (!cold && q.n_hot != q.n_values) ||
        (uint64_t)q.n_values + 4ull * kE6Slots * q.pool > 65535ull)
        return hipErrorInvalidValue;
    auto fn = cold ? (p.dropout > 0.0 ? encode6_kernel<true, true> : encode6_kernel<false, true>)
                   : (p.dropout > 0.0 ? encode6_kernel<true, false> : encode6_kernel<false, false>);
    hipError_t e = hipFuncSetAttribute(reinterpret_cast<const void*>(fn), hipFuncAttributeMaxDynamicSharedMemorySize, 160 * 1024);
    if (e != hipSuccess) return e;
    hipLaunchKernelGGL(fn, dim3(blocks), dim3(64u * (1u + 4u * kE6Walkers)), lds, stream, p, q);
    return hipGetLastError();
}

hipError_t launch_encode5(const EncodeParams& p, Encode5Params q, bool cold, int ppl, bool long_tokens, int compact, int waves, uint32_t blocks,
                          uint32_t min_lds, hipStream_t stream) {
    uint32_t lds = encode5_lds_layout(q.n_hot, long_tokens, waves, ppl, &q.list_off, &q.root_off, &q.idx_off);
    if (lds > 160u * 1024u || q.n_hot > q.n_values || (!cold && q.n_hot != q.n_values) || (long_tokens && ppl != 4) ||
        (compact != 0 && (compact < 4 || compact > 8)))
        return hipErrorInvalidValue;
    encode5_fn fn = pick_encode5(p.dropout > 0.0, cold, ppl, long_tokens, compact);
    hipError_t e = hipFuncSetAttribute(reinterpret_cast<const void*>(fn), hipFuncAttributeMaxDynamicSharedMemorySize, 160 * 1024);
    if (e != hipSuccess) return e;
    if (lds < min_lds && min_lds <= 160u * 1024u) lds = min_lds;
    hipLaunchKernelGGL(fn, dim3(blocks), dim3(64u * (uint32_t)waves), lds, stream, p, q);
    return hipGetLastError();
}

}
```

tokengeex_amd/csrc/kernels.h:

```cpp
#pragma once
#include <hip/hip_runtime.h>
#include <stdint.h>

#include "decode.h"
#include "spans.h"

namespace tgx {

constexpr uint32_t kTraceStride = 2;

struct EncodeParams {
    const uint8_t* text;
    const uint64_t* offs;
    const uint32_t* order;
    uint64_t n_samples;
    const void* trie;
    const uint32_t* tokid;
    uint32_t root_base;
    uint32_t n_slots;
    uint32_t lm;
    uint32_t* bp;
    uint32_t* tmp;
    uint32_t* counts;
    uint32_t* status;
// ... 155 lines not shown
struct Estep7Params {
    const uint8_t* text;
    const Estep7Work* work;
    Estep7Work host_work;
    const void* trie8t;
    uint32_t n_slots;
    uint32_t root_base;
    const double* wtab;
    uint32_t n_tok;
    uint32_t ovf_limit;
    uint32_t n_hot;
    double* expected;
    double dropout;
    uint64_t seed;
    uint32_t claim_chunk;
    uint32_t root_off, zero_off, idx_off;
    uint32_t flags;
    unsigned long long* stamps;
};
struct Estep7RedoParams {
    const uint8_t* text;
    const uint64_t* redo_offs;
    const uint32_t* redo_sample;
    const uint64_t* redo_base;
    const uint32_t* redo_snip;
    uint64_t n_redo;
    const uint64_t* tbase;
    const void* trie8t;
    uint32_t n_slots;
    uint32_t root_base;
    const double* wtab;
    uint32_t n_tok, n_hot;
    double* expected;
    double* zsnip;
    double* logz_sum;
    unsigned long long* range_flag;
    unsigned long long* queue;
    double* alpha;
    int32_t* aexp;
    unsigned char* mscratch;
    double dropout;
    uint64_t seed;
    uint32_t root_off, zero_off, idx_off;
};
uint32_t estep7_redo_max_hot(bool wide);
hipError_t launch_estep7_redo(Estep7RedoParams p, bool wide, uint32_t num_cus, hipStream_t stream);
uint32_t estep7_lds_layout(uint32_t n_hot, bool wide, int waves, int ppl, uint32_t* root_off, uint32_t* zero_off, uint32_t* idx_off);
uint32_t estep7_max_hot(bool wide, int waves, int ppl, uint32_t budget);
hipError_t estep7_waves_per_simd(bool dropout, bool cold, bool wide, int ppl, int* out);
hipError_t launch_estep7(Estep7Params p, bool wide, int ppl, int waves, uint32_t blocks, hipStream_t stream);
hipError_t launch_match_count(const uint8_t* text, uint64_t n_bytes, uint32_t chunk, uint64_t stride, const void* trie8t, uint32_t n_slots,
                              uint32_t root_base, uint32_t n_tok, unsigned int* counts, uint32_t num_cus, hipStream_t stream);
hipError_t launch_value_count(const uint8_t* text, uint64_t n_bytes, uint32_t chunk, uint64_t stride, const void* trie8, uint32_t n_slots,
                              uint32_t root_base, uint32_t n_values, uint32_t max_len, unsigned int* counts, uint32_t num_cus, hipStream_t stream);
hipError_t launch_rank_remap(void* trie8t, uint32_t n_slots, const uint32_t* perm, hipStream_t stream);
hipError_t launch_snip_z_check(const double* zsnip, uint64_t n_snips, unsigned long long* err_snip, hipStream_t stream);
hipError_t launch_piece_z_add(const double* zarr, const uint32_t* psnip, const uint32_t* order, uint64_t n_order, double* zsnip, hipStream_t stream);

hipError_t estep4_prepare();
hipError_t launch_estep4_fwd(const Estep4Params& p, uint32_t num_cus, hipStream_t stream);
hipError_t launch_estep4_bwd(const Estep4Params& p, uint32_t num_cus, hipStream_t stream);
hipError_t estep4l_prepare();
hipError_t launch_estep4l_fwd(const Estep4Params& p, int ppl, bool long_tokens, uint32_t num_cus, hipStream_t stream);
hipError_t launch_estep4l_bwd(const Estep4Params& p, int ppl, bool long_tokens, uint32_t num_cus, uint32_t groups_wanted, hipStream_t stream);
hipError_t launch_estep4_reduce(const double* rep, double* out, uint32_t n_slots, uint32_t n_replicas,
                                hipStream_t stream);

uint32_t estep_lds_bytes_per_block(uint32_t lm);
uint32_t estep_waves_per_block(uint32_t lm);
hipError_t estep_max_blocks_per_cu(uint32_t lm, int* out);
hipError_t launch_estep(const EstepParams& p, uint32_t blocks, hipStream_t stream);

uint32_t encode_lds_bytes_per_block(uint32_t lm);
uint32_t encode_waves_per_block(uint32_t lm);
hipError_t encode_max_blocks_per_cu(uint32_t lm, int* out);
hipError_t launch_encode(const EncodeParams& p, uint32_t blocks, hipStream_t stream);
uint32_t encode4_group_bytes();
hipError_t encode4_waves_per_simd(bool dropout, int ppl, bool root, int* out);
hipError_t launch_encode4(const EncodeParams& p, int ppl, int waves, uint32_t blocks, bool root, hipStream_t stream);
uint32_t encode4_lds_bytes(int waves, int ppl, bool root);
hipError_t launch_trace(const EncodeParams& p, uint32_t blocks, hipStream_t stream);
uint32_t encode5_lds_layout(uint32_t n_hot, bool long_tokens, int waves, int ppl, uint32_t* list_off, uint32_t* root_off, uint32_t* idx_off);
uint32_t encode5_max_hot(bool long_tokens, int waves, int ppl, uint32_t budget);
hipError_t encode5_waves_per_simd(bool dropout, bool cold, int ppl, bool long_tokens, int compact, int* out);
uint32_t encode6_lds_layout(uint32_t n_hot, uint32_t pool, uint32_t* root_off, uint32_t* ctrl_off, uint32_t* ring_off);
uint32_t encode6_max_hot(uint32_t budget, uint32_t pool);
uint32_t encode6_pool_total(uint32_t pool);
hipError_t estep5_waves_per_simd(bool dropout, bool cold, int ppl, int* out);
hipError_t launch_estep5_fwd(const struct Estep4Params& p, Encode5Params q, bool cold, int ppl, int waves, uint32_t blocks, hipStream_t stream);
hipError_t launch_encode6(const EncodeParams& p, Encode5Params q, bool cold, uint32_t blocks, hipStream_t stream);
hipError_t launch_encode5(const EncodeParams& p, Encode5Params q, bool cold, int ppl, bool long_tokens, int compact, int waves, uint32_t blocks,
                          uint32_t min_lds, hipStream_t stream);
hipError_t launch_encode2(const EncodeParams& p, uint32_t num_cus, bool permuted, hipStream_t stream);
hipError_t launch_trace32(const EncodeParams& p, uint32_t blocks, bool permuted, hipStream_t stream);
hipError_t launch_encode4l(const EncodeParams& p, uint32_t num_cus, hipStream_t stream);
hipError_t scan_temp_bytes(uint64_t n, size_t* bytes);
hipError_t launch_scan(uint32_t* counts, uint64_t* offsets, uint64_t n, void* temp, size_t temp_bytes, hipStream_t stream);
hipError_t launch_compact(const CompactParams& p, uint32_t blocks, bool rows, hipStream_t stream);

struct LayoutParams {
    const uint32_t* ids;
    const uint64_t* offs;
    uint64_t n_rows;
    uint32_t len;
    uint32_t pad, bos, eos;
    uint32_t flags;
    void* out;
    uint8_t* mask;
    int32_t* lengths;
    int32_t* doc;
    int32_t* pos;
    unsigned long long* counter;
};
hipError_t launch_layout_max_row(const uint64_t* offs, uint64_t n_rows, unsigned long long* max_out, hipStream_t stream);
hipError_t launch_layout_pad(const LayoutParams& p, hipStream_t stream);
hipError_t launch_layout_pack(const LayoutParams& p, uint64_t n_stream, uint64_t n_out, hipStream_t stream);
struct WindowParams {
    LayoutParams base;
    const uint64_t* wo;
    uint32_t stride;
    int32_t* window_row;
    int32_t* window_first;
};
hipError_t launch_layout_window_count(const uint64_t* offs, uint64_t n_rows, uint32_t room, uint32_t step, uint32_t* counts,
                                      unsigned long long* max_out, hipStream_t stream);
hipError_t launch_layout_windows(const WindowParams& q, uint64_t n_windows, hipStream_t stream);

struct AssembleParams {
    const uint32_t* ids;
    const uint64_t* offs;
    const uint64_t* seg_offs;
    const int32_t* seg_special;
    uint64_t* rank;
    uint64_t* starts;
    uint64_t n_segs, n_samples;
    uint64_t n_out;
    uint32_t vocab_size;
    uint32_t* out_ids;
    uint64_t* out_offs;
};
hipError_t assemble_scan_temp_bytes(uint64_t n_segs, size_t* bytes);
hipError_t launch_assemble_ranks(int32_t* seg_special, uint64_t* rank, uint64_t n_segs, void* temp, size_t temp_bytes, hipStream_t stream);
hipError_t launch_assemble_starts(const AssembleParams& p, hipStream_t stream);
hipError_t launch_assemble_fill(const AssembleParams& p, hipStream_t stream);

struct DecodeParams {
    DecodeTables tab;
    DecodeSrc src;
    uint32_t* meta;
    uint64_t* starts;
    uint64_t* specials;
    unsigned long long* bad_pos;
    unsigned long long* n_replaced;
    unsigned long long* n_specials_live;
    uint64_t n_raw;
    uint8_t* raw;
    uint32_t* flags;
    uint32_t* codes;
    uint64_t* row_offs;
    uint64_t* gpos;
    uint8_t* out;
};
hipError_t decode_scan_temp_bytes(uint64_t n, size_t* bytes);
hipError_t launch_decode_meta(const DecodeParams& p, void* temp, size_t temp_bytes, hipStream_t stream);
hipError_t launch_decode_specials(const DecodeParams& p, void* temp, size_t temp_bytes, hipStream_t stream);
hipError_t launch_decode_fill(const DecodeParams& p, hipStream_t stream);
hipError_t launch_decode_rows(const DecodeParams& p, hipStream_t stream);
hipError_t launch_decode_utf8(const DecodeParams& p, hipStream_t stream);
hipError_t decode_expand_temp_bytes(uint64_t n_groups, size_t* bytes);
hipError_t launch_decode_positions(const DecodeParams& p, void* temp, size_t temp_bytes, hipStream_t stream);
hipError_t launch_decode_expand(const DecodeParams& p, hipStream_t stream);

struct SpanParams {
    SpanTables tab;
    const uint32_t* ids;
// ... 19 lines not shown
```

tokengeex_amd/csrc/tgx_api.cpp:

```cpp
#include <hip/hip_runtime.h>

#include <algorithm>
#include <unordered_set>
#include <cstdarg>
#include <cstddef>
#include <cstdio>
#include <cstdlib>
#include <cmath>
#include <cstring>
#include <chrono>
#include <condition_variable>
#include <memory>
#include <mutex>
#include <new>
#include <numeric>
#include <string>
#include <thread>
#include <vector>

#include "../../include/tgx.h"
#include "api_internal.h"
#include "assemble.h"
#include "decode.h"
#include "front.h"
#include "kernels.h"
#include "layout.h"
#include "spans.h"
#include "nbest.h"
#include "sample.h"
#include "trie_build.h"

using namespace tgx::host;

tgx_status tgx_set_error(tgx_status st, const char* msg) {
    g_err_msg = msg ? msg : "";
    return st;
}
namespace {

#define HIP_TRY(expr)                                                                     \
    do {                                                                                  \
        hipError_t _e = (expr);                                                           \
        if (_e != hipSuccess)                                                             \
            return fail(TGX_ERR_DEVICE, "HIP error %d (%s) at %s:%d: %s", (int)_e,        \
                        hipGetErrorString(_e), __FILE__, __LINE__, #expr);                \
    } while (0)

struct PoolEntry {
    void* ptr;
    size_t bytes;
    int device;
};
std::mutex g_pool_mu;
std::vector<PoolEntry> g_pool;
size_t g_pool_bytes = 0;
constexpr size_t kPoolMaxBytes = 64ull << 30;

void pool_trim(int device) {
    std::vector<PoolEntry> victims;
    {
        std::lock_guard<std::mutex> lk(g_pool_mu);
        for (size_t i = 0; i < g_pool.size();) {
            if (device < 0 || g_pool[i].device == device) {
                victims.push_back(g_pool[i]);
                g_pool_bytes -= g_pool[i].bytes;
                g_pool.erase(g_pool.begin() + (long)i);
            } else {
                i++;
            }
        }
    }
    if (victims.empty()) return;
    int prev = -1;
    (void)hipGetDevice(&prev);
    for (const PoolEntry& e : victims) {
        (void)hipSetDevice(e.device);
        (void)hipFree(e.ptr);
    }
    if (prev >= 0) (void)hipSetDevice(prev);
}

hipError_t pool_alloc(int device, size_t bytes, void** out) {
    if (bytes == 0) bytes = 256;
    bytes = (bytes + 255) & ~size_t(255);
    {
        std::lock_guard<std::mutex> lk(g_pool_mu);
        size_t best = g_pool.size();
        for (size_t i = 0; i < g_pool.size(); i++) {
            const PoolEntry& e = g_pool[i];
            if (e.device != device || e.bytes < bytes || e.bytes > bytes * 2 + (1u << 20)) continue;
            if (best == g_pool.size() || e.bytes < g_pool[best].bytes) best = i;
        }
        if (best != g_pool.size()) {
            *out = g_pool[best].ptr;
            g_pool_bytes -= g_pool[best].bytes;
            g_pool.erase(g_pool.begin() + (long)best);
            return hipSuccess;
        }
    }
    hipError_t e = hipMalloc(out, bytes);
    if (e == hipErrorOutOfMemory) {
        (void)hipGetLastError();
        pool_trim(device);
        e = hipMalloc(out, bytes);
    }
    return e;
}

size_t rounded(size_t bytes) {
// ... 68 lines not shown
        ptr_ = nullptr;
    }
    T* get() const { return ptr_; }
    operator T*() const { return ptr_; }

private:
    int device_ = 0;
    T* ptr_ = nullptr;
    size_t bytes_ = 0;
};

struct KernelTime {
    const char* name;
    hipEvent_t start, stop;
    bool used;
};
constexpr int kMaxTimed = 8;
constexpr int kE5CompactDepth = 5;

struct DeviceCtrl {
    unsigned long long queue;
    unsigned long long err;
    unsigned long long queue6;
    struct Estep {
        unsigned long long queue;
        unsigned long long redo_count;
        unsigned long long queue_bwd;
        unsigned long long range_flag;
    } estep;
    unsigned long long encode_redo;
    unsigned long long longest;
    unsigned long long err_piece;
};
static_assert(offsetof(DeviceCtrl::Estep, redo_count) == 8 && offsetof(DeviceCtrl::Estep, queue_bwd) == 16 &&
                  offsetof(DeviceCtrl::Estep, range_flag) == 24 && sizeof(DeviceCtrl::Estep) == 32,
              "the E-step words are cleared by one memset");
struct HostCtrl {
    unsigned long long err;
    unsigned long long total_tokens;
};

}

struct tgx_model {
    int device = 0;
    uint32_t vocab_size = 0;
    uint32_t lm = 0;
    bool scores_finite = true;
    tgx::FlatTrie flat;
    void* d_trie = nullptr;
    uint32_t* d_tokid = nullptr;
    DeviceCtrl* d_ctrl = nullptr;
    HostCtrl* h_ctrl = nullptr;
    hipStream_t stream = nullptr;
    hipStream_t stream2 = nullptr;
    hipEvent_t ev_fork = nullptr, ev_join = nullptr;
    unsigned int* h_started = nullptr;
    int num_cus = 0;
    int blocks_per_cu = 0;
    std::vector<uint8_t> vocab_bytes;
    std::vector<uint64_t> vocab_offs;
    std::vector<double> vocab_scores;
    tgx::FlatTrie flat_rev;
    void* d_trie_rev = nullptr;
    bool rev_host_built = false;
    void* d_trie_w = nullptr;
    void* d_trie_rev_w = nullptr;
    uint64_t last_long_samples = 0;
    uint64_t last_estep_pieces = 0;
    uint32_t last_corun_cus = 0;
    double e7_overflow_share = 0.0;
    bool values_ranked = false;
    uint32_t corun_wait_timeouts = 0;
    uint64_t last_redo_samples = 0;
    int last_encode_waves_per_cu = 0;
    bool estep_linear_ok = false;
    tgx::TokHashTable tokhash;
    void* d_tokhash = nullptr;
    void* d_trie8 = nullptr;
    double* d_values = nullptr;
    std::vector<double> value_coverage;
    uint32_t n_values = 0, root_base8 = 0;
    uint32_t last_n_hot = 0;
    bool have_trie8 = false;
    bool encode_tables_ready = false;
    bool estep_trie8_tried = false;
    uint64_t estep_calls = 0;
    bool have_wvalues = false;
    double* d_wvalues = nullptr;
    bool tokhash_host_built = false;
    void* d_trie8t = nullptr;
    double* d_wtab = nullptr;
    std::vector<uint32_t> id_of_rank;
    uint32_t n_tok7 = 0, root_base7 = 0;
    bool trie8t_tried = false, have_trie8t = false;
    uint64_t last_estep_redo = 0;
    uint8_t* d_dec_len = nullptr;
    void* d_dec_slots = nullptr;
    uint8_t* d_dec_bytes = nullptr;
    uint64_t* d_dec_offs = nullptr;
    bool decode_tables_ready = false;
    uint16_t* d_span_words = nullptr;
    bool span_words_ready = false;
    int estep_blocks_per_cu = 0;
    KernelTime timed[kMaxTimed] = {};
    int n_timed = 0;
    uint64_t last_alg_bytes = 0;
    std::mutex mu;
};

struct tgx_corpus {
    int device = 0;
    uint64_t n_samples = 0, n_bytes = 0, max_len = 0;
    std::vector<uint64_t> h_offs;
    std::vector<uint32_t> h_sorted_len;
    std::vector<uint64_t> h_sorted_cum;
    PoolBuf<uint8_t> d_text_alloc;
    uint8_t* d_text = nullptr;
    PoolBuf<uint64_t> d_offs;
    PoolBuf<uint32_t> d_order;
    PoolBuf<uint32_t> d_bp, d_tmp, d_counts, d_status;
    PoolBuf<void> d_scan_tmp;
    size_t scan_tmp_bytes = 0;
    struct EstepWork {
        uint64_t snippet_len = 0;
        std::vector<uint64_t> soffs, sbase;
        std::vector<uint32_t> ssample, order;
        PoolBuf<uint64_t> d_soffs, d_sbase;
        PoolBuf<uint32_t> d_order, d_ssample;
        uint32_t window = 0;
        uint64_t n_windows = 0;
        PoolBuf<uint32_t> d_win_snip, d_win_k;
    } es;
    std::mutex mu;
};

struct tgx_result {
    int device = 0;
    uint32_t vocab_size = 0;
    uint64_t n_samples = 0, n_tokens = 0;
    PoolBuf<uint32_t> d_ids;
    PoolBuf<uint64_t> d_offs;
    std::unique_ptr<uint32_t[]> h_ids;
    std::vector<uint64_t> h_offs;
    bool have_ids = false, have_offs = false;
};

namespace {

class Pass {
public:
    explicit Pass(tgx_model* m) : m_(m) {}
    Pass(const Pass&) = delete;
    Pass& operator=(const Pass&) = delete;
    ~Pass() {
        if (ok_) return;
        (void)hipStreamSynchronize(m_->stream);
        if (m_->stream2) (void)hipStreamSynchronize(m_->stream2);
    }

    template <class T>
    hipError_t alloc(size_t bytes, T** out) {
        PoolBuf<void> b;
        const hipError_t e = b.alloc(m_->device, bytes);
        *out = static_cast<T*>(b.get());
        if (e == hipSuccess) scratch_.push_back(std::move(b));
// ... 197 lines not shown
        perm[order[r]] = r + 1u;
        v2[r + 1u] = values[order[r]];
        if (!w2.empty()) w2[r + 1u] = wvalues[order[r]];
        run += cnt[order[r]];
        cov[r + 1u] = total ? (double)run / (double)total : 1.0;
    }
    cov[nv] = 1.0;
    ok = hipMemcpyAsync(d_perm, perm.data(), ((size_t)nv + 1) * 4, hipMemcpyHostToDevice, m->stream) == hipSuccess &&
         tgx::launch_rank_remap(m->d_trie8, (uint32_t)m->flat.table.size(), d_perm, m->stream) == hipSuccess &&
         hipMemcpyAsync(m->d_values, v2.data(), ((size_t)nv + 1) * 8, hipMemcpyHostToDevice, m->stream) == hipSuccess &&
         (w2.empty() || hipMemcpyAsync(m->d_wvalues, w2.data(), ((size_t)nv + 1) * 8, hipMemcpyHostToDevice, m->stream) == hipSuccess) &&
         hipStreamSynchronize(m->stream) == hipSuccess;
    if (!ok) return fail(TGX_ERR_DEVICE, "value re-rank failed: %s", hipGetErrorString(hipGetLastError()));
    m->value_coverage = std::move(cov);
    hp.mark("re-rank");
    return pass.done();
}

tgx::EncodeParams base_encode_params(const tgx_model* m, const tgx_corpus* c, uint64_t seed) {
    tgx::EncodeParams p{};
    p.text = c->d_text;
    p.offs = c->d_offs;
    p.order = c->d_order;
    p.n_samples = c->n_samples;
    p.trie = m->d_trie;
    p.tokid = m->d_tokid;
    p.root_base = m->flat.table[0].base & ~tgx::kTerminalBit;
    p.lm = m->lm;
    p.n_slots = (uint32_t)m->flat.table.size();
    p.bp = c->d_bp;
    p.tmp = c->d_tmp;
    p.counts = c->d_counts;
    p.status = c->d_status;
    p.bp8 = reinterpret_cast<uint8_t*>(c->d_bp.get());
    p.tokhash = m->d_tokhash;
    p.tokhash_mask = m->tokhash.mask;
    p.tokhash_seed = m->tokhash.seed;
    p.err_sample = &m->d_ctrl->err;
    p.queue = &m->d_ctrl->queue;
    p.seed = seed;
    p.trace_carry = (c->n_samples && c->n_bytes / c->n_samples < 2048) ? 1u : 0u;
    p.trace_stride = tgx::kTraceStride;
    return p;
}

tgx_status redo_long_matches(tgx_model* m, tgx_corpus* c, const tgx::EncodeParams& p) {
    unsigned long long n_redo = 0;
    HIP_TRY(hipMemcpyAsync(&n_redo, &m->d_ctrl->encode_redo, 8, hipMemcpyDeviceToHost, m->stream));
    HIP_TRY(hipStreamSynchronize(m->stream));
    if (n_redo > c->n_samples) return fail(TGX_ERR_DEVICE, "redo list longer than the batch");
    m->last_redo_samples = n_redo;
    if (n_redo) {
        tgx::EncodeParams q = p;
        q.order = c->d_counts;
        q.n_samples = n_redo;
        HIP_TRY(hipMemsetAsync(&m->d_ctrl->queue, 0x00, 8, m->stream));
        time_begin(m, "encode2_kernel");
        HIP_TRY(tgx::launch_encode2(q, (uint32_t)m->num_cus, true, m->stream));
        time_end(m);
    }
    return TGX_OK;
}

tgx_status run_encode_kernel(tgx_model* m, tgx_corpus* c, double dropout, uint64_t seed, Pass& pass) {
    tgx_status st = ensure_scratch(c);
    if (st != TGX_OK) return st;
    HIP_TRY(hipMemsetAsync(&m->d_ctrl->queue, 0x00, 8, m->stream));
    HIP_TRY(hipMemsetAsync(&m->d_ctrl->err, 0xFF, 8, m->stream));
    tgx::EncodeParams p = base_encode_params(m, c, seed);
    p.dropout = dropout;
    if (const char* e = knob("TGX_TRACE_CARRY")) p.trace_carry = atoi(e) ? 1u : 0u;
    if (const char* e = knob("TGX_TRACE_STRIDE")) p.trace_stride = (uint32_t)std::min(3, std::max(0, atoi(e)));
    p.flags = debug_flags();
    const char* force = knob("TGX_PATH");
    const bool use4 = m->lm <= 16 && m->scores_finite && m->d_tokhash && !(force && strcmp(force, "fused") == 0);
    const bool use2 = !use4 && m->lm <= 32 && m->scores_finite && m->d_tokhash && !(force && strcmp(force, "fused") == 0);
    const bool long_tokens = m->lm > 16;
    const bool use5 = (use4 || use2) && m->have_trie8 &&
                      !(force && (strcmp(force, "rows4") == 0 || strcmp(force, "rows2") == 0 || strcmp(force, "rows4l") == 0));
    if (debug_on())
        fprintf(stderr, "[tgx] encode: S=%llu N=%llu lm=%u path=%s slots=%zu root_base=%u values=%u\n",
                (unsigned long long)c->n_samples, (unsigned long long)c->n_bytes, p.lm, use4 ? (use5 ? "rows5" : "rows4") : (use2 ? "rows2" : "fused"),
                m->flat.table.size(), p.root_base, m->n_values);
    if (use5) {
        {
            const tgx_status rst = ensure_value_ranks(m, c);
            if (rst != TGX_OK) return rst;
        }
        m->last_redo_samples = 0;
        int e6_bpc = 2;
        if (const char* e = knob("TGX_E6_BPC")) e6_bpc = std::min(4, std::max(1, atoi(e)));
        uint32_t n_hot6 = std::min(m->n_values, tgx::encode6_max_hot(160u * 1024u / (uint32_t)e6_bpc, 0u));
        uint32_t pool6 = 0;
        bool e6_usable = true;
        if (n_hot6 < m->n_values) {
            pool6 = 128;
            if (const char* e = knob("TGX_E6_POOL")) pool6 = (uint32_t)std::min(192, std::max(0, atoi(e)));
            if ((uint64_t)m->n_values + tgx::encode6_pool_total(pool6) > 65535ull) {
                pool6 = 0;
                e6_usable = knob("TGX_E6_POOL") != nullptr || knob("TGX_LONG_THRESHOLD") != nullptr;
            }
            n_hot6 = std::min(m->n_values, tgx::encode6_max_hot(160u * 1024u / (uint32_t)e6_bpc, pool6));
        }
        n_hot6 = knob_cap_hot("TGX_E5_HOT", n_hot6);
        const bool cold6 = n_hot6 < m->n_values;
        uint64_t n_long = 0;
        uint32_t corun_cus = 0;
        if (c->n_samples && !long_tokens && e6_usable) {
            const auto count_ge = [&](uint64_t thr) {
                return (uint64_t)(std::partition_point(c->h_sorted_len.begin(), c->h_sorted_len.end(),
                                                       [thr](uint32_t len) { return len >= thr; }) - c->h_sorted_len.begin());
            };
            if (const char* e = knob("TGX_LONG_THRESHOLD")) {
                const uint64_t thr = (uint64_t)std::max(0ll, atoll(e));
                if (thr) n_long = count_ge(thr);
            } else {
                const double N = (double)c->n_bytes;
                const double c5 = m->n_values > tgx::encode5_max_hot(false, 8, 4, 160u * 1024u) ? 0.135e-6 : 0.108e-6;
                auto cost = [&](uint64_t k) {
                    const double bytes_long = k ? (double)c->h_sorted_cum[k - 1] : 0.0;
                    const double t6 = k ? std::max((double)c->h_sorted_len[0] * (cold6 ? 0.042e-6 : 0.0369e-6), bytes_long / (cold6 ? 46e9 : 55e9)) + 20e-6 : 0.0;
                    const double rest_max = k < c->n_samples ? (double)c->h_sorted_len[k] : 0.0;
                    const double t5 = std::max(rest_max * c5, (N - bytes_long) / 88e9);
                    return t6 + t5;
                };
                double best = cost(0);
                for (uint64_t thr = 1024; thr <= c->max_len; thr *= 2) {
                    const uint64_t k = count_ge(thr);
                    const double ck = cost(k);
                    if (k && ck < best * 0.9) {
                        best = ck;
                        n_long = k;
                    }
                }
                const double c6 = cold6 ? 0.042e-6 : 0.0369e-6, r6 = (cold6 ? 46e9 : 55e9) / (double)m->num_cus;
                double best_co = best * 0.9;
                uint64_t k_co = 0;
                static const uint64_t thrs[] = {8192, 12288, 16384, 24576, 32768, 40960, 49152};
                static const uint32_t shares[] = {32, 48, 64, 96, 128, 160, 192};
                const bool corun_off = (knob("TGX_CORUN") && atoi(knob("TGX_CORUN")) == 0) || m->corun_wait_timeouts != 0 ||
                                       m->n_values > tgx::encode5_max_hot(false, 8, 4, 160u * 1024u);
                for (uint64_t thr : thrs) {
                    if (corun_off || thr > c->max_len || e6_bpc != 2) break;
                    const uint64_t k = count_ge(thr);
                    if (!k || k >= c->n_samples) continue;
                    const double bytes_long = (double)c->h_sorted_cum[k - 1];
                    const double r_max = (double)c->h_sorted_len[k], r_bytes = N - bytes_long;
                    for (uint32_t X : shares) {
                        if ((int)X >= m->num_cus) break;
                        const double t6 = std::max((double)c->h_sorted_len[0] * c6, bytes_long / (X * r6)) + 20e-6;
                        const double t5 = std::max(r_max * 0.12e-6, r_bytes / ((double)(m->num_cus - (int)X) / (double)m->num_cus * 70e9));
                        const double t = std::max(t5, t6);
                        if (t < best_co) {
                            best_co = t;
                            k_co = k;
                            corun_cus = X;
                        }
                    }
                }
                if (corun_cus) n_long = k_co;
            }
            if (const char* e = knob("TGX_CORUN")) {
                const int v = atoi(e);
                corun_cus = (v > 0 && v < m->num_cus && n_long > 0 && n_long < c->n_samples && e6_bpc == 2) ? (uint32_t)v : 0u;
            }
        }
        const int cus5 = m->num_cus - (int)corun_cus;
        const uint64_t rest_n = c->n_samples - n_long;
        const uint64_t rest_bytes = c->n_bytes - (n_long ? c->h_sorted_cum[n_long - 1] : 0);
        const uint64_t rest_max = rest_n ? c->h_sorted_len[n_long] : 0;
        int ppl = 4, bpc = 1, hot_waves = 16;
        int compact = kE5CompactDepth;
        if (const char* e = knob("TGX_E5_COMPACT")) compact = (strcmp(e, "off") == 0 || atoi(e) == 0) ? 0 : std::min(8, std::max(4, atoi(e)));
        {
            int ps4 = 0;
            HIP_TRY(tgx::encode5_waves_per_simd(dropout > 0.0, false, 4, long_tokens, compact, &ps4));
            hot_waves = std::min(16, ps4 * 4);
            const int least = long_tokens ? 12 : 13;
            while (hot_waves >= least && m->n_values > tgx::encode5_max_hot(long_tokens, hot_waves, 4, 160u * 1024u)) hot_waves--;
            if (hot_waves < least) {
                hot_waves = 0;
                if (!long_tokens) {
                    if (m->n_values <= tgx::encode5_max_hot(false, 13, 3, 160u * 1024u)) {
                        ppl = 3;
                        hot_waves = 13;
                    } else if (m->n_values <= tgx::encode5_max_hot(false, 16, 2, 160u * 1024u)) {
                        ppl = 2;
                    } else {
                        ppl = 3;
                    }
                }
            }
        }
        int balance_waves = 0;
        if (rest_max > 0) {
            const uint64_t rows_bal = (rest_bytes + rest_max - 1) / rest_max;
            const uint64_t wb = (rows_bal + 4ull * (uint64_t)cus5 - 1) / (4ull * (uint64_t)cus5);
            if (wb <= 10) {
                balance_waves = (int)std::max<uint64_t>(4, wb);
                ppl = 4;
                hot_waves = 0;
            }
        }
        if (const char* e = long_tokens ? nullptr : knob("TGX_PPL")) {
            const int v = atoi(e);
            if (v >= 1 && v <= 4) {
                ppl = v;
                bpc = ppl >= 3 ? 1 : 2;
            }
        }
        knob_int("TGX_BPC", 1, 8, &bpc);
        const uint32_t budget = 160u * 1024u / (uint32_t)bpc;
        bool cold = false;
        int per_simd = 0;
        HIP_TRY(tgx::encode5_waves_per_simd(dropout > 0.0, false, ppl, long_tokens, compact, &per_simd));
        int waves = std::min(16, (per_simd / bpc) * 4);
        if ((ppl == 4 || ppl == 3) && bpc == 1 && hot_waves > 0) waves = std::min(waves, hot_waves);
        if (m->n_values > tgx::encode5_max_hot(long_tokens, waves, ppl, budget)) {
            cold = true;
            HIP_TRY(tgx::encode5_waves_per_simd(dropout > 0.0, true, ppl, long_tokens, compact, &per_simd));
            waves = std::min(16, (per_simd / bpc) * 4);
        }
        if (balance_waves > 0 && ppl == 4 && bpc == 1) waves = std::min(waves, balance_waves);
        waves = waves_for_units(waves, rest_n, (uint64_t)cus5 * bpc);
        knob_int("TGX_WAVES", 1, 16, &waves);
        while (waves > 1 && tgx::encode5_max_hot(long_tokens, waves, ppl, budget) < 16u) waves--;
        uint32_t n_hot = std::min(m->n_values, tgx::encode5_max_hot(long_tokens, waves, ppl, budget));
        n_hot = knob_cap_hot("TGX_E5_HOT", n_hot);
        cold = n_hot < m->n_values;
        m->last_n_hot = n_hot;
        m->last_encode_waves_per_cu = std::min(bpc, per_simd / ((waves + 3) / 4)) * waves;
        const uint64_t rows_per_block = 4 * (uint64_t)waves;
        const uint32_t blocks5 = (uint32_t)std::max<uint64_t>(
            1, std::min<uint64_t>((rest_n + rows_per_block - 1) / rows_per_block, (uint64_t)cus5 * bpc));
        tgx::Encode5Params q{};
        q.trie8 = m->d_trie8;
        q.trie_bytes = (uint32_t)(m->flat.table.size() * sizeof(tgx::Trie8Rec));
        q.values = m->d_values;
        q.root_base = m->root_base8;
        q.n_values = m->n_values;
        q.n_hot = n_hot;
        q.claim_chunk = claim_chunk_for(c->n_bytes, c->n_samples);
        if (const char* e = knob("TGX_CLAIM_CHUNK")) q.claim_chunk = (uint32_t)std::min(64, std::max(1, atoi(e)));
        m->last_long_samples = n_long;
        m->last_corun_cus = n_long ? corun_cus : 0u;
        tgx::EncodeParams p6 = p;
        tgx::Encode5Params q6 = q;
        uint32_t blocks6 = 0;
        if (n_long) {
            p6.n_samples = n_long;
            blocks6 = (uint32_t)std::min<uint64_t>((n_long + 3) / 4, (uint64_t)(corun_cus ? (int)corun_cus : m->num_cus) * (uint64_t)e6_bpc);
            q6.n_hot = n_hot6;
            q6.pool = cold6 ? pool6 : 0u;
            if (!corun_cus) {
                time_begin(m, "encode6_kernel");
                HIP_TRY(tgx::launch_encode6(p6, q6, cold6, blocks6, m->stream));
                time_end(m);
                HIP_TRY(hipMemsetAsync(&m->d_ctrl->queue, 0x00, 8, m->stream));
            } else {
                if (!m->stream2) {
                    HIP_TRY(hipStreamCreateWithFlags(&m->stream2, hipStreamNonBlocking));
                    HIP_TRY(hipEventCreateWithFlags(&m->ev_fork, hipEventDisableTiming));
                    HIP_TRY(hipEventCreateWithFlags(&m->ev_join, hipEventDisableTiming));
                    HIP_TRY(hipHostMalloc((void**)&m->h_started, 64, hipHostMallocMapped | hipHostMallocPortable));
                }
                *reinterpret_cast<volatile unsigned int*>(m->h_started) = 0u;
                q.started = m->h_started;
                p6.queue = &m->d_ctrl->queue6;
                HIP_TRY(hipMemsetAsync(&m->d_ctrl->queue6, 0x00, 8, m->stream));
                HIP_TRY(hipEventRecord(m->ev_fork, m->stream));
                HIP_TRY(hipStreamWaitEvent(m->stream2, m->ev_fork, 0));
            }
            p.order = c->d_order + n_long;
            p.n_samples = c->n_samples - n_long;
        }
        const Stamps stamps5 = stamps_begin(m, pass, '1', (size_t)blocks5 * (size_t)waves);
        p.stamps = stamps5.d;
        time_begin(m, "encode5_kernel");
        {
            if (long_tokens) {
                p.redo_count = &m->d_ctrl->encode_redo;
                p.redo_list = c->d_counts;
                HIP_TRY(hipMemsetAsync(&m->d_ctrl->encode_redo, 0x00, 8, m->stream));
            }
            const hipError_t le = tgx::launch_encode5(p, q, cold, ppl, long_tokens, compact, waves, blocks5, corun_cus && n_long ? 84u * 1024u : 0u, m->stream);
            if (le != hipSuccess) return fail(TGX_ERR_DEVICE, "encode5 launch failed: %s", hipGetErrorString(le));
        }
        bool joined = false, joined_slot = false;
        if (n_long && corun_cus) {
            const bool slot = m->n_timed + 1 < kMaxTimed;
            if (slot) {
                KernelTime& tb = m->timed[m->n_timed + 1];
                tb.name = "encode6_kernel";
                tb.used = true;
                (void)hipEventRecord(tb.start, m->stream2);
            }
            {
                const auto t0 = std::chrono::steady_clock::now();
                volatile unsigned int* started = m->h_started;
                bool timed_out = false;
                while (*started < blocks5 && !(timed_out = std::chrono::steady_clock::now() - t0 >= std::chrono::milliseconds(2))) {
                }
                if (timed_out && *started < blocks5) m->corun_wait_timeouts++;
            }
            const hipError_t l6 = tgx::launch_encode6(p6, q6, cold6, blocks6, m->stream2);
            if (slot) (void)hipEventRecord(m->timed[m->n_timed + 1].stop, m->stream2);
            (void)hipEventRecord(m->ev_join, m->stream2);
            if (l6 != hipSuccess) return fail(TGX_ERR_DEVICE, "encode6 launch failed: %s", hipGetErrorString(l6));
            joined = true;
            joined_slot = slot;
        }
        time_end(m);
        if (joined) {
            if (joined_slot) m->n_timed++;
            HIP_TRY(hipStreamWaitEvent(m->stream, m->ev_join, 0));
        }
        if (stamps5.d) stamps_report(m, stamps5, ppl, "encode5 stamps", "iteration", {"switch", "text+reset", "walk", "relax", "store"});
        p.stamps = nullptr;
        if (long_tokens) {
            const tgx_status rst = redo_long_matches(m, c, p);
            if (rst != TGX_OK) return rst;
        }
        p.order = c->d_order;
        p.n_samples = c->n_samples;
        const uint32_t blocks_t = trace_blocks(m, c->n_samples);
        Stamps stamps_t;
        if (!long_tokens) stamps_t = stamps_begin(m, pass, '2', (size_t)blocks_t * 4);
        p.stamps = stamps_t.d;
        time_begin(m, long_tokens ? "trace32_kernel" : "trace_kernel");
        if (long_tokens) HIP_TRY(tgx::launch_trace32(p, blocks_t, true, m->stream));
        else HIP_TRY(tgx::launch_trace(p, blocks_t, m->stream));
        time_end(m);
        if (stamps_t.d) stamps_report(m, stamps_t, 0, "trace stamps", "window", {"setup", "loads", "hops", "append+lookups", "-"});
        p.stamps = nullptr;
    } else if (use4) {
        int ppl = 1, waves = 10, bpc = 2;
        const double gbps4[3] = {60.0, 50.0, 34.0}, chain4_ms[3] = {13.5, 10.7, 9.1};
        auto cost4 = [&](double bytes, double longest, int* ppl_out) {
            double best_t = 0;
            int best_ppl = 1;
            for (int i = 0; i < 3; i++) {
                const double t = std::max(bytes / (gbps4[i] * 1e9), longest / 65536.0 * chain4_ms[i] * 1e-3);
                if (i == 0 || t < best_t * 0.95) {
                    best_t = t;
                    best_ppl = 1 << i;
                }
            }
            if (ppl_out) *ppl_out = best_ppl;
            return best_t;
        };
        m->last_long_samples = 0;
        m->last_redo_samples = 0;
        cost4((double)c->n_bytes, c->n_samples ? (double)c->h_sorted_len[0] : 0.0, &ppl);
        if (const char* e = knob("TGX_PPL")) {
            const int v = atoi(e);
            if (v == 1 || v == 2 || v == 4) ppl = v;
        }
        if (ppl == 2) { waves = 5; bpc = 2; }
        if (ppl == 4) { waves = 5; bpc = 1; }
        knob_int("TGX_WAVES", 1, 16, &waves);
        knob_int("TGX_BPC", 1, 8, &bpc);
        bool root = ppl == 1;
        if (const char* e = knob("TGX_ROOT")) root = root && atoi(e) != 0;
        while (waves > 1 && tgx::encode4_lds_bytes(waves, ppl, root) > (160u * 1024u) / (uint32_t)bpc) waves--;
        {
            int per_simd = 0;
            HIP_TRY(tgx::encode4_waves_per_simd(dropout > 0.0, ppl, root, &per_simd));
            if (bpc * ((waves + 3) / 4) > per_simd && ppl == 1) {
                waves = 4;
                bpc = std::min(5, per_simd);
                root = false;
                HIP_TRY(tgx::encode4_waves_per_simd(dropout > 0.0, ppl, root, &per_simd));
            }
            m->last_encode_waves_per_cu = std::min(bpc * ((waves + 3) / 4), per_simd) * 4 >= bpc * waves
                                              ? bpc * waves
                                              : per_simd / ((waves + 3) / 4) * waves;
        }
        const uint64_t rows_per_block = 4 * (uint64_t)waves;
        const uint32_t blocks4 = (uint32_t)std::max<uint64_t>(
            1, std::min<uint64_t>((p.n_samples + rows_per_block - 1) / rows_per_block, (uint64_t)m->num_cus * bpc));
        Stamps stamps4;
        if (dropout <= 0.0 && ppl == 1) stamps4 = stamps_begin(m, pass, '1', (size_t)blocks4 * (size_t)waves);
        p.stamps = stamps4.d;
        time_begin(m, "encode4_kernel");
        HIP_TRY(tgx::launch_encode4(p, ppl, waves, blocks4, root, m->stream));
        time_end(m);
        if (stamps4.d) stamps_report(m, stamps4, 0, "stamps", "iteration", {"switch", "text", "walk", "relax", "store"});
        p.stamps = nullptr;
// ... 157 lines not shown
tgx_status tgx_model_create(const uint8_t* bytes, const uint64_t* offs, const double* scores,
                            uint32_t vocab_size, int device, tgx_model** out) {
    return tgx_model_create_ex(bytes, offs, scores, vocab_size, device, 0, out);
}

tgx_status tgx_model_create_ex(const uint8_t* bytes, const uint64_t* offs, const double* scores,
                               uint32_t vocab_size, int device, uint32_t flags, tgx_model** out) {
    if (!out) return fail(TGX_ERR_INVALID, "tgx_model_create: out is NULL");
    *out = nullptr;
    if (vocab_size && (!offs || !scores)) return fail(TGX_ERR_INVALID, "tgx_model_create: NULL vocab");
    if (vocab_size && !bytes && offs[vocab_size] != offs[0]) return fail(TGX_ERR_INVALID, "tgx_model_create: NULL token bytes");
    int ndev = 0;
    if (const tgx_status dst = require_device(&ndev)) return dst;
    if (device < 0 || device >= ndev)
        return fail(TGX_ERR_INVALID, "device %d out of range (have %d)", device, ndev);

    tgx::HostPhases hp("tgx_model_create");
    tgx_model* m = new tgx_model();
    m->device = device;
    m->vocab_size = vocab_size;
    static const uint64_t zero_offs[1] = {0};
    bool fused_estep = vocab_size != 0;
    for (uint32_t i = 0; i < vocab_size && fused_estep; i++)
        fused_estep = offs[i + 1] - offs[i] <= 16 && scores[i] >= -300.0 && scores[i] <= 300.0;
    std::thread rev_builder;
    if ((flags & TGX_MODEL_FOR_ESTEP) && vocab_size && !fused_estep)
        rev_builder = std::thread([m, bytes, offs, scores, vocab_size]() {
            const uint64_t o0 = offs[0];
            std::vector<uint8_t> rev((size_t)(offs[vocab_size] - o0));
            std::vector<uint64_t> ro(vocab_size + 1);
            for (uint32_t i = 0; i <= vocab_size; i++) ro[i] = offs[i] - o0;
            for (uint32_t i = 0; i < vocab_size; i++)
                for (uint64_t k = ro[i]; k < ro[i + 1]; k++) rev[k] = bytes[o0 + ro[i + 1] - 1 - (k - ro[i])];
            tgx::build_flat_trie(rev.data(), ro.data(), scores, vocab_size, &m->flat_rev);
        });
    std::thread hash_early;
    if (!(flags & TGX_MODEL_FOR_ESTEP) && vocab_size) {
        bool finite = true;
        uint64_t longest = 0;
        for (uint32_t i = 0; i < vocab_size; i++) {
            finite = finite && (scores[i] - scores[i] == 0.0);
            longest = std::max<uint64_t>(longest, offs[i + 1] - offs[i]);
        }
        if (finite && longest <= 32) {
            hash_early = std::thread([m, bytes, offs, vocab_size]() {
                std::vector<uint64_t> ro(vocab_size + 1);
                for (uint32_t i = 0; i <= vocab_size; i++) ro[i] = offs[i] - offs[0];
                tgx::build_tok_hash(bytes + offs[0], ro.data(), vocab_size, &m->tokhash);
            });
        }
    }
    hp.mark("scan of the vocabulary");
    tgx::build_flat_trie(bytes, vocab_size ? offs : zero_offs, scores, vocab_size, &m->flat);
    hp.mark("build_flat_trie");
    if (hash_early.joinable()) {
        hash_early.join();
        m->tokhash_host_built = true;
    }
    if (rev_builder.joinable()) {
        rev_builder.join();
        m->rev_host_built = true;
    }
    hp.mark("join hash / reverse builders");
    const tgx_status fst = finish_model_create(m, bytes, offs, scores, vocab_size, device, flags, out);
    hp.mark("finish (device tables)");
    return fst;
}

static tgx_status finish_model_create(tgx_model* m, const uint8_t* bytes, const uint64_t* offs, const double* scores,
                                      uint32_t vocab_size, int device, uint32_t flags, tgx_model** out) {
    std::unique_ptr<tgx_model, void (*)(tgx_model*)> owner(m, tgx_model_destroy);
    if (m->flat.max_token_len > TGX_MAX_TOKEN_LEN)
        return fail(TGX_ERR_UNSUPPORTED, "token of %u bytes exceeds TGX_MAX_TOKEN_LEN (%d)", m->flat.max_token_len,
                    TGX_MAX_TOKEN_LEN);
    if (m->flat.table.size() >= (1u << 26)) return fail(TGX_ERR_UNSUPPORTED, "trie needs more than 2^26 slots");
    m->lm = std::max<uint32_t>(4, (m->flat.max_token_len + 3) & ~3u);
    if (vocab_size) {
        m->vocab_bytes.assign(bytes + offs[0], bytes + offs[vocab_size]);
        m->vocab_offs.resize(vocab_size + 1);
        for (uint32_t i = 0; i <= vocab_size; i++) m->vocab_offs[i] = offs[i] - offs[0];
        m->vocab_scores.assign(scores, scores + vocab_size);
        for (uint32_t i = 0; i < vocab_size; i++)
            if (!(scores[i] - scores[i] == 0.0)) m->scores_finite = false;
    } else {
        m->vocab_offs.assign(1, 0);
    }

    HIP_TRY(hipSetDevice(device));
    hipDeviceProp_t prop;
    HIP_TRY(hipGetDeviceProperties(&prop, device));
    m->num_cus = prop.multiProcessorCount;
    HIP_TRY(hipStreamCreateWithFlags(&m->stream, hipStreamNonBlocking));
    size_t tbytes = m->flat.table.size() * sizeof(tgx::TrieRec);
    HIP_TRY(hipMalloc(&m->d_trie, tbytes));
    HIP_TRY(hipMalloc((void**)&m->d_tokid, m->flat.tokid.size() * 4));
    HIP_TRY(hipMalloc((void**)&m->d_ctrl, sizeof(DeviceCtrl)));
    if (!(flags & TGX_MODEL_FOR_ESTEP)) {
        const tgx_status est = ensure_encode_tables(m);
        if (est != TGX_OK) return est;
    }
    HIP_TRY(hipHostMalloc((void**)&m->h_ctrl, sizeof(HostCtrl), hipHostMallocDefault));
    HIP_TRY(hipMemcpyAsync(m->d_trie, m->flat.table.data(), tbytes, hipMemcpyHostToDevice, m->stream));
    HIP_TRY(hipMemcpyAsync(m->d_tokid, m->flat.tokid.data(), m->flat.tokid.size() * 4, hipMemcpyHostToDevice, m->stream));
    for (int i = 0; i < kMaxTimed; i++) {
        m->timed[i].used = false;
        m->timed[i].name = "";
        HIP_TRY(hipEventCreate(&m->timed[i].start));
        HIP_TRY(hipEventCreate(&m->timed[i].stop));
    }
    {
        int occ = 0;
        HIP_TRY(tgx::encode_max_blocks_per_cu(m->lm, &occ));
        m->blocks_per_cu = std::max(1, std::min(occ, 16));
    }
    HIP_TRY(hipStreamSynchronize(m->stream));
    *out = owner.release();
    return TGX_OK;
}

tgx_status tgx_model_create_derived(const tgx_model* parent, const uint32_t* keep_ids, uint32_t n_keep, const double* scores,
                                    uint32_t flags, tgx_model** out) {
    if (!out) return fail(TGX_ERR_INVALID, "tgx_model_create_derived: out is NULL");
    *out = nullptr;
    if (!parent || (n_keep && (!keep_ids || !scores))) return fail(TGX_ERR_INVALID, "tgx_model_create_derived: NULL argument");
    tgx::HostPhases hp("tgx_model_create_derived");
    const uint32_t PV = parent->vocab_size;
    for (uint32_t i = 0; i < n_keep; i++)
        if (keep_ids[i] >= PV || (i && keep_ids[i] <= keep_ids[i - 1])) return fail(TGX_ERR_INVALID, "tgx_model_create_derived: keep_ids must ascend within the parent's vocabulary");
    if (!(flags & TGX_MODEL_FOR_ESTEP) && parent->flat.table.size() > tgx::kTrie8MaxSlots && (uint64_t)n_keep * 2 <= PV)
        return fail(TGX_ERR_UNSUPPORTED, "tgx_model_create_derived: the parent's table has more slots than 8-byte records address; build this model from scratch");
    {
        uint64_t non_empty = 0, terminals = 0;
        for (uint32_t i = 0; i < PV; i++) non_empty += parent->vocab_offs[i + 1] > parent->vocab_offs[i];
        for (uint32_t t : parent->flat.tokid) terminals += t != tgx::kNoToken;
        if (terminals != non_empty) return fail(TGX_ERR_UNSUPPORTED, "tgx_model_create_derived: the parent vocabulary has duplicate tokens");
    }
    tgx_model* m = new tgx_model();
    m->device = parent->device;
    m->vocab_size = n_keep;
    std::vector<uint32_t> new_id(PV, tgx::kNoToken);
    for (uint32_t i = 0; i < n_keep; i++) new_id[keep_ids[i]] = i;
    std::vector<uint8_t> bytes;
    std::vector<uint64_t> offs(n_keep + 1, 0);
    uint32_t longest = 0;
    for (uint32_t i = 0; i < n_keep; i++) {
        const uint64_t b = parent->vocab_offs[keep_ids[i]], e = parent->vocab_offs[keep_ids[i] + 1];
        offs[i + 1] = offs[i] + (e - b);
        longest = std::max<uint32_t>(longest, (uint32_t)(e - b));
    }
    bytes.resize(offs[n_keep]);
    for (uint32_t i = 0; i < n_keep; i++) {
        const uint64_t b = parent->vocab_offs[keep_ids[i]], e = parent->vocab_offs[keep_ids[i] + 1];
        if (e > b) memcpy(bytes.data() + offs[i], parent->vocab_bytes.data() + b, (size_t)(e - b));
    }
    hp.mark("checks + bytes");
    auto derive = [&](const tgx::FlatTrie& src, tgx::FlatTrie* dst) {
        *dst = src;
        dst->max_token_len = longest;
        for (size_t t = 0; t < dst->tokid.size(); t++) {
            const uint32_t old = dst->tokid[t];
            if (old == tgx::kNoToken) continue;
            const uint32_t nid = new_id[old];
            tgx::TrieRec& r = dst->table[t];
            if (nid == tgx::kNoToken) {
                dst->tokid[t] = tgx::kNoToken;
                r.base &= ~tgx::kTerminalBit;
// ... 2907 lines not shown
        parts.push_back({ids, tc});
        time_begin(m, "nbest_compact_kernel");
        if (tgx::launch_nbest_compact(p, r->d_offs + R0, ids, (uint32_t)m->num_cus, m->stream) != hipSuccess)
            return fail(TGX_ERR_DEVICE, "nbest_compact_kernel launch failed");
        time_end(m);
        if (total && tgx::launch_offs_add(r->d_offs + R0, ns * k, total, m->stream) != hipSuccess)
            return fail(TGX_ERR_DEVICE, "offset launch failed");
        total += tc;
    }
    r->n_tokens = total;
    if (!r->d_ids) {
        if (r->d_ids.alloc(m->device, (size_t)total * 4 + 256) != hipSuccess)
            return fail(TGX_ERR_DEVICE, "out of device memory (result ids)");
        uint64_t at = 0;
        for (auto& pt : parts) {
            if (pt.second && hipMemcpyAsync(r->d_ids + at, pt.first, (size_t)pt.second * 4, hipMemcpyDeviceToDevice, m->stream) != hipSuccess)
                return fail(TGX_ERR_DEVICE, "n-best gather failed");
            at += pt.second;
        }
    }
    if ((scores && rows_all && hipMemcpyAsync(scores, d_scores, (size_t)rows_all * 8, hipMemcpyDeviceToHost, m->stream) != hipSuccess) ||
        (n_found && S && hipMemcpyAsync(n_found, d_nfound, (size_t)S * 4, hipMemcpyDeviceToHost, m->stream) != hipSuccess) ||
        hipStreamSynchronize(m->stream) != hipSuccess)
        return fail(TGX_ERR_DEVICE, "n-best pass failed: %s", hipGetErrorString(hipGetLastError()));
    m->h_ctrl->err = ~0ULL;
    if (hipMemcpy(&m->h_ctrl->err, &m->d_ctrl->err, 8, hipMemcpyDeviceToHost) != hipSuccess)
        return fail(TGX_ERR_DEVICE, "n-best pass failed");
    const tgx_status st = check_no_path(m, c);
    if (st != TGX_OK) return st;
    m->last_alg_bytes = c->n_bytes + 4 * r->n_tokens + 8 * (rows_all + 1) + 12 * rows_all;
    *out = pass.release_result();
    return pass.done();
}

tgx_status tgx_encode_corpus_nbest(tgx_model* m, tgx_corpus* c, uint32_t nbest, double* scores, uint32_t* n_found, tgx_result** out) {
    if (const tgx_status dst = require_device()) return dst;
    if (!m || !c || !out) return fail(TGX_ERR_INVALID, "tgx_encode_corpus_nbest: NULL argument");
    *out = nullptr;
    if (m->device != c->device) return fail(TGX_ERR_INVALID, "model and corpus on different devices");
    std::lock_guard<std::mutex> lk(m->mu);
    const tgx_status st = nbest_check(m, nbest);
    if (st != TGX_OK) return st;
    std::lock_guard<std::mutex> lkc(c->mu);
    return nbest_corpus_locked(m, c, nbest, scores, n_found, out);
}

tgx_status tgx_encode_batch_nbest(tgx_model* m, const uint8_t* text, const uint64_t* offs, uint64_t n_samples, uint32_t nbest,
                                  double* scores, uint32_t* n_found, tgx_result** out) {
    if (const tgx_status dst = require_device()) return dst;
    if (!m || !out) return fail(TGX_ERR_INVALID, "tgx_encode_batch_nbest: NULL argument");
    *out = nullptr;
    {
        std::lock_guard<std::mutex> lk(m->mu);
        const tgx_status st = nbest_check(m, nbest);
        if (st != TGX_OK) return st;
    }
    return on_uploaded_batch(m, text, offs, n_samples, [&](tgx_corpus* c) { return tgx_encode_corpus_nbest(m, c, nbest, scores, n_found, out); });
}


int tgx_last_kernel_times(const tgx_model* m, const char** names, float* ms, int cap) {
    if (!m) return 0;
    int n = 0;
    for (int i = 0; i < m->n_timed && n < cap; i++) {
        float t = 0.f;
        if (hipEventElapsedTime(&t, m->timed[i].start, m->timed[i].stop) != hipSuccess) t = -1.f;
        if (names) names[n] = m->timed[i].name;
        if (ms) ms[n] = t;
        n++;
    }
    return n;
}

uint32_t tgx_last_encode_waves_per_cu(const tgx_model* m) { return m ? (uint32_t)m->last_encode_waves_per_cu : 0u; }
uint64_t tgx_last_algorithmic_bytes(const tgx_model* m) { return m ? m->last_alg_bytes : 0; }
uint64_t tgx_last_encode_redo_samples(const tgx_model* m) { return m ? m->last_redo_samples : 0; }
uint64_t tgx_last_encode_long_samples(const tgx_model* m) { return m ? m->last_long_samples : 0; }
uint64_t tgx_last_estep_pieces(const tgx_model* m) { return m ? m->last_estep_pieces : 0; }
uint64_t tgx_last_estep_redo(const tgx_model* m) { return m ? m->last_estep_redo : 0; }
uint32_t tgx_last_encode_corun_cus(const tgx_model* m) { return m ? m->last_corun_cus : 0; }
uint32_t tgx_encode_corun_timeouts(const tgx_model* m) { return m ? m->corun_wait_timeouts : 0; }
uint32_t tgx_model_score_values(const tgx_model* m) { return m && m->have_trie8 ? m->n_values : 0u; }
uint32_t tgx_last_encode_hot_values(const tgx_model* m) { return m ? m->last_n_hot : 0u; }
```

Measured before the change: 71520.

## Add lean encode5 relax step with cheaper reset, DPP broadcast and fetch

Adds lean template variants of the encode5/encode6 Viterbi relax kernels. When scores have a bounded exponent, the step drops the per-step finish-high tracking and resets the accumulator by patching its high word, except in groups that contain a sample end. It also swaps the inline-asm row broadcast for the mov_dpp builtin and computes score-table addresses with a single SDWA shift. The lean path is gated by a host check on score magnitudes and an env knob, which adds kernel instantiations and a correctness dependence on that score-range assumption.

Result: faster. 72240 (median of 6 runs) (+1.0%).

```diff
diff --git a/include/tgx.h b/include/tgx.h
--- a/include/tgx.h
+++ b/include/tgx.h
@@ -286,6 +286,7 @@
 uint32_t tgx_encode_corun_timeouts(const tgx_model *m);
 uint32_t tgx_model_score_values(const tgx_model *m);
 uint32_t tgx_last_encode_hot_values(const tgx_model *m);
+uint32_t tgx_last_encode_lean_items(const tgx_model *m);
 
 static inline double tgx_dropout_u01(uint64_t seed, uint64_t sample, uint64_t pos, uint32_t len) {
     uint64_t x = seed ^ (sample * 0x9E3779B97F4A7C15ULL) ^ (pos * 0xC2B2AE3D27D4EB4FULL) ^
diff --git a/tokengeex_amd/_lib.py b/tokengeex_amd/_lib.py
--- a/tokengeex_amd/_lib.py
+++ b/tokengeex_amd/_lib.py
@@ -90,6 +90,7 @@
     "tgx_last_encode_redo_samples": (_u64, [_vp]),
     "tgx_model_score_values": (_u32, [_vp]),
     "tgx_last_encode_hot_values": (_u32, [_vp]),
+    "tgx_last_encode_lean_items": (_u32, [_vp]),
     "tgx_last_encode_long_samples": (_u64, [_vp]),
     "tgx_last_estep_pieces": (_u64, [_vp]),
     "tgx_last_estep_redo": (_u64, [_vp]),
@@ -1136,6 +1137,13 @@
     def last_encode_hot_values(self) -> int:
         return lib.tgx_last_encode_hot_values(self._h)
 
+    def last_encode_lean_items(self) -> tuple[int, int]:
+        v = lib.tgx_last_encode_lean_items(self._h)
+        return v & 0xFF, (v >> 8) & 0xFF
+
+    def last_encode_lean_step(self) -> bool:
+        return bool(self.last_encode_lean_items()[0] & 1)
+
     def last_encode_long_samples(self) -> int:
         return lib.tgx_last_encode_long_samples(self._h)
 
diff --git a/tokengeex_amd/build.py b/tokengeex_amd/build.py
--- a/tokengeex_amd/build.py
+++ b/tokengeex_amd/build.py
@@ -9,7 +9,7 @@
 CSRC = os.path.join(HERE, "csrc")
 OUT = os.path.join(HERE, "libtgx.so")
 SOURCES = ["kernels.hip", "estep.hip", "encode2.hip", "encode4l.hip", "encode5.hip", "estep4.hip", "estep4l.hip", "estep7.hip", "cuts.hip", "pairs.hip", "generate.hip", "sample.hip", "nbest.hip", "layout.hip", "assemble.hip", "decode.hip", "spans.hip", "front.hip", "tgx_api.cpp", "host_twins.cpp", "trie_build.cpp", "prune_host.cpp", "frontback.cpp", "unicode_norm.cpp"]
-HEADERS = ["api_internal.h", "kernels.h", "sample.h", "nbest.h", "layout.h", "assemble.h", "decode.h", "spans.h", "front.h", "device_common.h", "trace_body.h", "trie_build.h", "unicode_tables.h", os.path.join("..", "..", "include", "tgx.h")]
+HEADERS = ["api_internal.h", "kernels.h", "sample.h", "nbest.h", "layout.h", "assemble.h", "decode.h", "spans.h", "front.h", "device_common.h", "lean_gate.h", "trace_body.h", "trie_build.h", "unicode_tables.h", os.path.join("..", "..", "include", "tgx.h")]
 ARCH = "gfx950"
 
 
diff --git a/tokengeex_amd/csrc/device_common.h b/tokengeex_amd/csrc/device_common.h
--- a/tokengeex_amd/csrc/device_common.h
+++ b/tokengeex_amd/csrc/device_common.h
@@ -91,6 +91,19 @@
     asm volatile("s_nop 1\n\tv_mov_b64_dpp %0, %1 row_newbcast:%2 row_mask:0xf bank_mask:0xf"
                  : "=v"(r) : "v"(v), "n"(U));
     return r;
+}
+
+template <int U>
+__device__ __forceinline__ double row_bcast_f64_b(double v) {
+    return __longlong_as_double(__builtin_amdgcn_mov_dpp(__double_as_longlong(v), 0x150 + U, 0xF, 0xF, false));
+}
+
+template <int H>
+__device__ __forceinline__ uint32_t word_times8(uint32_t w) {
+    uint32_t a;
+    if (H) asm("v_lshlrev_b32_sdwa %0, 3, %1 dst_sel:DWORD dst_unused:UNUSED_PAD src0_sel:DWORD src1_sel:WORD_1" : "=v"(a) : "v"(w));
+    else asm("v_lshlrev_b32_sdwa %0, 3, %1 dst_sel:DWORD dst_unused:UNUSED_PAD src0_sel:DWORD src1_sel:WORD_0" : "=v"(a) : "v"(w));
+    return a;
 }
 
 constexpr uint64_t kRowLane0 = 0x0001000100010001ULL;
@@ -155,13 +168,37 @@
     bpv = sel_imm_u32<U>(take, bpv);
 }
 
-template <int U>
+constexpr int kLeanStep = 1, kLeanBcast = 2, kLeanFetch = 4;
+constexpr uint32_t kLeanResetHi = 0xFFEFFFFFu;
+constexpr uint32_t kLeanUnreachedHi = 0xFFE00000u;
+template <int LN>
+__device__ __forceinline__ bool relax5_reached(uint32_t fhi) { return (LN & kLeanStep) ? fhi < kLeanUnreachedHi : fhi != 0xFFF00000u; }
+
+template <int U, int LN = 0>
 __device__ __forceinline__ void relax5_step(double sv, double& acc, uint32_t& bpv, uint32_t& fin, uint32_t& fhi) {
     constexpr uint64_t MU = kRowLane0 << U;
-    const double best = row_bcast_f64<U>(acc);
+    double best;
+    if constexpr ((LN & kLeanBcast) != 0) best = row_bcast_f64_b<U>(acc);
+    else best = row_bcast_f64<U>(acc);
     fin = sel_u32(MU, bpv, fin);
     fhi = sel_u32(MU, (uint32_t)((uint64_t)__double_as_longlong(acc) >> 32), fhi);
     const double acc_r = sel_f64(MU, -__builtin_huge_val(), acc);
+    const double cand = best + sv;
+    const uint64_t take = __builtin_amdgcn_fcmp(cand, acc_r, 2 );
+    asm("v_max_f64 %0, %1, %2" : "=v"(acc) : "v"(acc_r), "v"(cand));
+    bpv = sel_imm_u32<U>(take, bpv);
+}
+
+template <int U, int LN>
+__device__ __forceinline__ void relax5_lean_step(double sv, double& acc, uint32_t& bpv, uint32_t& fin) {
+    constexpr uint64_t MU = kRowLane0 << U;
+    double best;
+    if constexpr ((LN & kLeanBcast) != 0) best = row_bcast_f64_b<U>(acc);
+    else best = row_bcast_f64<U>(acc);
+    fin = sel_u32(MU, bpv, fin);
+    const uint64_t ab = (uint64_t)__double_as_longlong(acc);
+    const uint32_t hi_r = sel_u32(MU, kLeanResetHi, (uint32_t)(ab >> 32));
+    const double acc_r = __hiloint2double((int)hi_r, (int)(uint32_t)ab);
     const double cand = best + sv;
     const uint64_t take = __builtin_amdgcn_fcmp(cand, acc_r, 2 );
     asm("v_max_f64 %0, %1, %2" : "=v"(acc) : "v"(acc_r), "v"(cand));
diff --git a/tokengeex_amd/csrc/encode5.hip b/tokengeex_amd/csrc/encode5.hip
--- a/tokengeex_amd/csrc/encode5.hip
+++ b/tokengeex_amd/csrc/encode5.hip
@@ -185,26 +185,35 @@
     }
 };
 
-template <int N>
+template <int N, int LN = 0>
 __device__ __forceinline__ void e5_scores_issue(uint32_t tab, const uint32_t (&iw)[8], int first, u32x2_t (&sp)[N]) {
 #pragma unroll
     for (int u = 0; u < N; ++u) {
         const int v = first + u;
-        const uint32_t a = (v & 1) ? ((iw[v >> 1] >> 16) << 3) : ((iw[v >> 1] & 0xFFFFu) << 3);
-        sp[u] = lds_ld<u32x2_t>(tab + a);
+        if constexpr ((LN & kLeanFetch) != 0) {
+            sp[u] = lds_ld<u32x2_t>((v & 1) ? word_times8<1>(iw[v >> 1]) : word_times8<0>(iw[v >> 1]));
+        } else {
+            const uint32_t a = (v & 1) ? ((iw[v >> 1] >> 16) << 3) : ((iw[v >> 1] & 0xFFFFu) << 3);
+            sp[u] = lds_ld<u32x2_t>(tab + a);
+        }
     }
 }
 __device__ __forceinline__ double e5_score_value(const u32x2_t& p) { return __hiloint2double((int)p.y, (int)p.x); }
 
-template <int N>
+template <int N, int LN = 0>
 __device__ __forceinline__ void e5_scores_cold(uint32_t tab, __amdgpu_buffer_rsrc_t cold, const uint32_t (&iw)[8], int first,
                                                uint32_t hot_bytes, double (&sv)[N]) {
     uint32_t a[N];
 #pragma unroll
     for (int u = 0; u < N; ++u) {
         const int v = first + u;
-        a[u] = (v & 1) ? ((iw[v >> 1] >> 16) << 3) : ((iw[v >> 1] & 0xFFFFu) << 3);
-        sv[u] = lds_ld<double>(tab + (a[u] < hot_bytes ? a[u] : 0u));
+        if constexpr ((LN & kLeanFetch) != 0) {
+            a[u] = (v & 1) ? word_times8<1>(iw[v >> 1]) : word_times8<0>(iw[v >> 1]);
+            sv[u] = lds_ld<double>(a[u] < hot_bytes ? a[u] : 0u);
+        } else {
+            a[u] = (v & 1) ? ((iw[v >> 1] >> 16) << 3) : ((iw[v >> 1] & 0xFFFFu) << 3);
+            sv[u] = lds_ld<double>(tab + (a[u] < hot_bytes ? a[u] : 0u));
+        }
     }
     static_assert(N == 4 || N == 8, "e5_scores_cold: four or eight values at a time");
     if (N == 8) asm volatile("" : "+v"(sv[0]), "+v"(sv[1]), "+v"(sv[2]), "+v"(sv[3]), "+v"(sv[4 % N]), "+v"(sv[5 % N]), "+v"(sv[6 % N]), "+v"(sv[7 % N]));
@@ -290,9 +299,10 @@
         t_last = _now;                                                 \
     }
 
-template <bool DROPOUT, bool COLD, int PPL, bool LONG, int CK = 0>
+template <bool DROPOUT, bool COLD, int PPL, bool LONG, int CK = 0, int LN = 0>
 __global__ __launch_bounds__(1024, (PPL == 1 ? 8 : (PPL == 2 ? 6 : (PPL == 3 ? 4 : 1)))) void encode5_kernel(EncodeParams P, Encode5Params Q) {
     static_assert(!LONG || PPL == 4, "the long-token build runs four positions per lane");
+    static_assert(LN == 0 || (!LONG && !DROPOUT), "the long-token and dropout builds keep the kernel as it was");
     extern __shared__ __align__(16) unsigned char smem[];
     constexpr uint32_t LM = LONG ? 32 : 16;
     constexpr uint32_t SPAN = 16u * PPL;
@@ -450,7 +460,13 @@
             };
             u32x2_t sa[4], sb[4];
             load_iw(0, iw);
-            if (!COLD) e5_scores_issue<4>(lds0, iw, 0, sa);
+            if (!COLD) e5_scores_issue<4, LN>(lds0, iw, 0, sa);
+            uint32_t end_groups = 0;
+            if (LN & kLeanStep) {
+                const uint32_t g_end = (live && n - p0 < SPAN) ? ((n - p0) >> 4) : 0xFFu;
+#pragma unroll
+                for (int g = 0; g < PPL; ++g) end_groups |= (__builtin_amdgcn_ballot_w64(g_end == (uint32_t)g) != 0 ? 1u : 0u) << g;
+            }
 #pragma unroll
             for (int g = 0; g < PPL; ++g) {
                 uint32_t (&cw)[8] = (g & 1) ? iwn : iw;
@@ -513,51 +529,89 @@
                     }
                     continue;
                 }
-                if (COLD) {
-                    double sv[8], sw[8];
-                    e5_scores_cold<8>(lds0, cold_values, cw, 0, hot_bytes, sv);
-                    e5_scores_cold<8>(lds0, cold_values, cw, 8, hot_bytes, sw);
-                    if (g + 1 < PPL) load_iw(g + 1, nw);
-                    relax5_step<0>(sv[0], acc, bpv, fin[g], fhi);
-                    relax5_step<1>(sv[1], acc, bpv, fin[g], fhi);
-                    relax5_step<2>(sv[2], acc, bpv, fin[g], fhi);
-                    relax5_step<3>(sv[3], acc, bpv, fin[g], fhi);
-                    relax5_step<4>(sv[4], acc, bpv, fin[g], fhi);
-                    relax5_step<5>(sv[5], acc, bpv, fin[g], fhi);
-                    relax5_step<6>(sv[6], acc, bpv, fin[g], fhi);
-                    relax5_step<7>(sv[7], acc, bpv, fin[g], fhi);
-                    relax5_step<8>(sw[0], acc, bpv, fin[g], fhi);
-                    relax5_step<9>(sw[1], acc, bpv, fin[g], fhi);
-                    relax5_step<10>(sw[2], acc, bpv, fin[g], fhi);
-                    relax5_step<11>(sw[3], acc, bpv, fin[g], fhi);
-                    relax5_step<12>(sw[4], acc, bpv, fin[g], fhi);
-                    relax5_step<13>(sw[5], acc, bpv, fin[g], fhi);
-                    relax5_step<14>(sw[6], acc, bpv, fin[g], fhi);
-                    relax5_step<15>(sw[7], acc, bpv, fin[g], fhi);
+                if constexpr (LN == 0) {
+                    if (COLD) {
+                        double sv[8], sw[8];
+                        e5_scores_cold<8>(lds0, cold_values, cw, 0, hot_bytes, sv);
+                        e5_scores_cold<8>(lds0, cold_values, cw, 8, hot_bytes, sw);
+                        if (g + 1 < PPL) load_iw(g + 1, nw);
+                        relax5_step<0>(sv[0], acc, bpv, fin[g], fhi);
+                        relax5_step<1>(sv[1], acc, bpv, fin[g], fhi);
+                        relax5_step<2>(sv[2], acc, bpv, fin[g], fhi);
+                        relax5_step<3>(sv[3], acc, bpv, fin[g], fhi);
+                        relax5_step<4>(sv[4], acc, bpv, fin[g], fhi);
+                        relax5_step<5>(sv[5], acc, bpv, fin[g], fhi);
+                        relax5_step<6>(sv[6], acc, bpv, fin[g], fhi);
+                        relax5_step<7>(sv[7], acc, bpv, fin[g], fhi);
+                        relax5_step<8>(sw[0], acc, bpv, fin[g], fhi);
+                        relax5_step<9>(sw[1], acc, bpv, fin[g], fhi);
+                        relax5_step<10>(sw[2], acc, bpv, fin[g], fhi);
+                        relax5_step<11>(sw[3], acc, bpv, fin[g], fhi);
+                        relax5_step<12>(sw[4], acc, bpv, fin[g], fhi);
+                        relax5_step<13>(sw[5], acc, bpv, fin[g], fhi);
+                        relax5_step<14>(sw[6], acc, bpv, fin[g], fhi);
+                        relax5_step<15>(sw[7], acc, bpv, fin[g], fhi);
+                    } else {
+                        e5_scores_issue<4>(lds0, cw, 4, sb);
+                        if (g + 1 < PPL) load_iw(g + 1, nw);
+                        relax5_step<0>(e5_score_value(sa[0]), acc, bpv, fin[g], fhi);
+                        relax5_step<1>(e5_score_value(sa[1]), acc, bpv, fin[g], fhi);
+                        relax5_step<2>(e5_score_value(sa[2]), acc, bpv, fin[g], fhi);
+                        relax5_step<3>(e5_score_value(sa[3]), acc, bpv, fin[g], fhi);
+                        e5_scores_issue<4>(lds0, cw, 8, sa);
+                        relax5_step<4>(e5_score_value(sb[0]), acc, bpv, fin[g], fhi);
+                        relax5_step<5>(e5_score_value(sb[1]), acc, bpv, fin[g], fhi);
+                        relax5_step<6>(e5_score_value(sb[2]), acc, bpv, fin[g], fhi);
+                        relax5_step<7>(e5_score_value(sb[3]), acc, bpv, fin[g], fhi);
+                        e5_scores_issue<4>(lds0, cw, 12, sb);
+                        relax5_step<8>(e5_score_value(sa[0]), acc, bpv, fin[g], fhi);
+                        relax5_step<9>(e5_score_value(sa[1]), acc, bpv, fin[g], fhi);
+                        relax5_step<10>(e5_score_value(sa[2]), acc, bpv, fin[g], fhi);
+                        relax5_step<11>(e5_score_value(sa[3]), acc, bpv, fin[g], fhi);
+                        if (g + 1 < PPL) e5_scores_issue<4>(lds0, nw, 0, sa);
+                        relax5_step<12>(e5_score_value(sb[0]), acc, bpv, fin[g], fhi);
+                        relax5_step<13>(e5_score_value(sb[1]), acc, bpv, fin[g], fhi);
+                        relax5_step<14>(e5_score_value(sb[2]), acc, bpv, fin[g], fhi);
+                        relax5_step<15>(e5_score_value(sb[3]), acc, bpv, fin[g], fhi);
+                    }
+                    reached[g] = fhi != 0xFFF00000u;
                 } else {
-                    e5_scores_issue<4>(lds0, cw, 4, sb);
-                    if (g + 1 < PPL) load_iw(g + 1, nw);
-                    relax5_step<0>(e5_score_value(sa[0]), acc, bpv, fin[g], fhi);
-                    relax5_step<1>(e5_score_value(sa[1]), acc, bpv, fin[g], fhi);
-                    relax5_step<2>(e5_score_value(sa[2]), acc, bpv, fin[g], fhi);
-                    relax5_step<3>(e5_score_value(sa[3]), acc, bpv, fin[g], fhi);
-                    e5_scores_issue<4>(lds0, cw, 8, sa);
-                    relax5_step<4>(e5_score_value(sb[0]), acc, bpv, fin[g], fhi);
-                    relax5_step<5>(e5_score_value(sb[1]), acc, bpv, fin[g], fhi);
-                    relax5_step<6>(e5_score_value(sb[2]), acc, bpv, fin[g], fhi);
-                    relax5_step<7>(e5_score_value(sb[3]), acc, bpv, fin[g], fhi);
-                    e5_scores_issue<4>(lds0, cw, 12, sb);
-                    relax5_step<8>(e5_score_value(sa[0]), acc, bpv, fin[g], fhi);
-                    relax5_step<9>(e5_score_value(sa[1]), acc, bpv, fin[g], fhi);
-                    relax5_step<10>(e5_score_value(sa[2]), acc, bpv, fin[g], fhi);
-                    relax5_step<11>(e5_score_value(sa[3]), acc, bpv, fin[g], fhi);
-                    if (g + 1 < PPL) e5_scores_issue<4>(lds0, nw, 0, sa);
-                    relax5_step<12>(e5_score_value(sb[0]), acc, bpv, fin[g], fhi);
-                    relax5_step<13>(e5_score_value(sb[1]), acc, bpv, fin[g], fhi);
-                    relax5_step<14>(e5_score_value(sb[2]), acc, bpv, fin[g], fhi);
-                    relax5_step<15>(e5_score_value(sb[3]), acc, bpv, fin[g], fhi);
-                }
-                reached[g] = fhi != 0xFFF00000u;
+                    const bool full = !(LN & kLeanStep) || ((end_groups >> g) & 1u) != 0u;
+#define E5_STEP(U, SV)                                                   \
+        if (FULL) relax5_step<U, LN>(SV, acc, bpv, fin[g], fhi);              \
+        else relax5_lean_step<U, LN>(SV, acc, bpv, fin[g]);
+                    auto steps = [&](auto full_tag) {
+                        constexpr bool FULL = decltype(full_tag)::value;
+                        if (COLD) {
+                            double sv[8], sw[8];
+                            e5_scores_cold<8, LN>(lds0, cold_values, cw, 0, hot_bytes, sv);
+                            e5_scores_cold<8, LN>(lds0, cold_values, cw, 8, hot_bytes, sw);
+                            if (g + 1 < PPL) load_iw(g + 1, nw);
+                            E5_STEP(0, sv[0]) E5_STEP(1, sv[1]) E5_STEP(2, sv[2]) E5_STEP(3, sv[3])
+                            E5_STEP(4, sv[4]) E5_STEP(5, sv[5]) E5_STEP(6, sv[6]) E5_STEP(7, sv[7])
+                            E5_STEP(8, sw[0]) E5_STEP(9, sw[1]) E5_STEP(10, sw[2]) E5_STEP(11, sw[3])
+                            E5_STEP(12, sw[4]) E5_STEP(13, sw[5]) E5_STEP(14, sw[6]) E5_STEP(15, sw[7])
+                        } else {
+                            e5_scores_issue<4, LN>(lds0, cw, 4, sb);
+                            if (g + 1 < PPL) load_iw(g + 1, nw);
+                            E5_STEP(0, e5_score_value(sa[0])) E5_STEP(1, e5_score_value(sa[1]))
+                            E5_STEP(2, e5_score_value(sa[2])) E5_STEP(3, e5_score_value(sa[3]))
+                            e5_scores_issue<4, LN>(lds0, cw, 8, sa);
+                            E5_STEP(4, e5_score_value(sb[0])) E5_STEP(5, e5_score_value(sb[1]))
+                            E5_STEP(6, e5_score_value(sb[2])) E5_STEP(7, e5_score_value(sb[3]))
+                            e5_scores_issue<4, LN>(lds0, cw, 12, sb);
+                            E5_STEP(8, e5_score_value(sa[0])) E5_STEP(9, e5_score_value(sa[1]))
+                            E5_STEP(10, e5_score_value(sa[2])) E5_STEP(11, e5_score_value(sa[3]))
+                            if (g + 1 < PPL) e5_scores_issue<4, LN>(lds0, nw, 0, sa);
+                            E5_STEP(12, e5_score_value(sb[0])) E5_STEP(13, e5_score_value(sb[1]))
+                            E5_STEP(14, e5_score_value(sb[2])) E5_STEP(15, e5_score_value(sb[3]))
+                        }
+                    };
+                    if (full) steps(std::true_type{});
+                    else steps(std::false_type{});
+#undef E5_STEP
+                    reached[g] = !full || relax5_reached<LN>(fhi);
+                }
             }
         } else {
 #pragma unroll
@@ -633,21 +687,23 @@
 __device__ __forceinline__ uint32_t lds_load(const uint32_t* p) { return __hip_atomic_load(p, __ATOMIC_RELAXED, __HIP_MEMORY_SCOPE_WORKGROUP); }
 __device__ __forceinline__ void lds_store(uint32_t* p, uint32_t v) { __hip_atomic_store(p, v, __ATOMIC_RELAXED, __HIP_MEMORY_SCOPE_WORKGROUP); }
 
-template <bool COLD>
+template <bool COLD, int LN = 0>
 __device__ __forceinline__ void e6_load_quarter(uint32_t tab, __amdgpu_buffer_rsrc_t cold, uint32_t hot_bytes,
                                                 const uint32_t (&iw)[8], int q, double (&sv)[4]) {
     if (COLD) {
-        e5_scores_cold<4>(tab, cold, iw, 4 * q, hot_bytes, sv);
+        e5_scores_cold<4, LN>(tab, cold, iw, 4 * q, hot_bytes, sv);
     } else {
         u32x2_t sp[4];
-        e5_scores_issue<4>(tab, iw, 4 * q, sp);
+        e5_scores_issue<4, LN>(tab, iw, 4 * q, sp);
 #pragma unroll
         for (int u = 0; u < 4; ++u) sv[u] = e5_score_value(sp[u]);
     }
 }
 
-template <bool DROPOUT, bool COLD>
+template <bool DROPOUT, bool COLD, int LN = 0>
 __global__ __launch_bounds__(64 * (1 + 4 * kE6Walkers), 8) void encode6_kernel(EncodeParams P, Encode5Params Q) {
+    static_assert(LN == 0 || !DROPOUT, "the dropout builds keep the kernel as it was");
+    static_assert((LN & (kLeanStep | kLeanBcast)) == 0, "encode6_kernel: the score fetch only (the lean step spills here)");
     extern __shared__ __align__(16) unsigned char smem[];
     constexpr uint32_t LM = 16;
     constexpr uint32_t K = kE6Walkers, G = kE6Slots;
@@ -749,30 +805,30 @@
                 uint32_t iwa[8], iwb[8];
                 double sva[4], svb[4];
                 load_iw(0, iwa);
-                e6_load_quarter<C>(lds0, values, hot_bytes, iwa, 0, sva);
+                e6_load_quarter<C, LN>(lds0, values, hot_bytes, iwa, 0, sva);
 #pragma unroll
                 for (int g = 0; g < 4; ++g) {
                     uint32_t (&iw)[8] = (g & 1) ? iwb : iwa;
                     uint32_t (&iwn)[8] = (g & 1) ? iwa : iwb;
                     fin[g] = kNoStep;
                     uint32_t fhi = 0xFFF00000u;
-                    e6_load_quarter<C>(lds0, values, hot_bytes, iw, 1, svb);
+                    e6_load_quarter<C, LN>(lds0, values, hot_bytes, iw, 1, svb);
                     if (g < 3) load_iw(g + 1, iwn);
                     relax5_step<0>(sva[0], acc, bpv, fin[g], fhi);
                     relax5_step<1>(sva[1], acc, bpv, fin[g], fhi);
                     relax5_step<2>(sva[2], acc, bpv, fin[g], fhi);
                     relax5_step<3>(sva[3], acc, bpv, fin[g], fhi);
-                    e6_load_quarter<C>(lds0, values, hot_bytes, iw, 2, sva);
+                    e6_load_quarter<C, LN>(lds0, values, hot_bytes, iw, 2, sva);
                     relax5_step<4>(svb[0], acc, bpv, fin[g], fhi);
                     relax5_step<5>(svb[1], acc, bpv, fin[g], fhi);
                     relax5_step<6>(svb[2], acc, bpv, fin[g], fhi);
                     relax5_step<7>(svb[3], acc, bpv, fin[g], fhi);
-                    e6_load_quarter<C>(lds0, values, hot_bytes, iw, 3, svb);
+                    e6_load_quarter<C, LN>(lds0, values, hot_bytes, iw, 3, svb);
                     relax5_step<8>(sva[0], acc, bpv, fin[g], fhi);
                     relax5_step<9>(sva[1], acc, bpv, fin[g], fhi);
                     relax5_step<10>(sva[2], acc, bpv, fin[g], fhi);
                     relax5_step<11>(sva[3], acc, bpv, fin[g], fhi);
-                    if (g < 3) e6_load_quarter<C>(lds0, values, hot_bytes, iwn, 0, sva);
+                    if (g < 3) e6_load_quarter<C, LN>(lds0, values, hot_bytes, iwn, 0, sva);
                     relax5_step<12>(svb[0], acc, bpv, fin[g], fhi);
                     relax5_step<13>(svb[1], acc, bpv, fin[g], fhi);
                     relax5_step<14>(svb[2], acc, bpv, fin[g], fhi);
@@ -1105,7 +1161,25 @@
 }
 
 typedef void (*encode5_fn)(EncodeParams, Encode5Params);
-static encode5_fn pick_encode5(bool dropout, bool cold, int ppl, bool long_tokens, int compact) {
+#ifdef TGX_E5_LEAN_ITEMS
+constexpr int kE5LeanHot = TGX_E5_LEAN_ITEMS, kE5LeanCold = TGX_E5_LEAN_ITEMS, kE5LeanCold3 = TGX_E5_LEAN_ITEMS;
+constexpr int kE6Lean = kLeanFetch;
+#else
+constexpr int kE5LeanHot = kLeanFetch;
+constexpr int kE5LeanCold = kLeanFetch;
+constexpr int kE5LeanCold3 = kLeanStep | kLeanBcast | kLeanFetch;
+constexpr int kE6Lean = kLeanFetch;
+#endif
+static_assert(kE5LeanHot > 0 && kE5LeanHot <= 7 && kE5LeanCold > 0 && kE5LeanCold <= 7 && kE5LeanCold3 > 0 && kE5LeanCold3 <= 7,
+              "a mask of kLeanStep, kLeanBcast, kLeanFetch");
+constexpr int lean_without_step(int items) { return items & ~kLeanStep; }
+bool encode5_has_lean(bool dropout, bool long_tokens) { return !dropout && !long_tokens; }
+int encode5_lean_items(bool cold, int ppl, bool step_ok) {
+    const int items = cold ? (ppl == 3 ? kE5LeanCold3 : kE5LeanCold) : kE5LeanHot;
+    return step_ok ? items : lean_without_step(items);
+}
+int encode6_lean_items() { return kE6Lean; }
+static encode5_fn pick_encode5(bool dropout, bool cold, int ppl, bool long_tokens, int compact, bool lean, bool step_ok) {
     if (long_tokens) {
         if (cold) return dropout ? encode5_kernel<true, true, 4, true> : encode5_kernel<false, true, 4, true>;
         return dropout ? encode5_kernel<true, false, 4, true> : encode5_kernel<false, false, 4, true>;
@@ -1122,20 +1196,29 @@
         if (ppl == 3) return encode5_kernel<true, false, 3, false>;
         return encode5_kernel<true, false, 4, false>;
     }
-#define TGX_E5K(C, PL) \
-    (compact == 4 ? encode5_kernel<false, C, PL, false, 4> : compact == 5 ? encode5_kernel<false, C, PL, false, 5> \
-     : compact == 6 ? encode5_kernel<false, C, PL, false, 6> : compact == 7 ? encode5_kernel<false, C, PL, false, 7> \
-     : compact == 8 ? encode5_kernel<false, C, PL, false, 8> : encode5_kernel<false, C, PL, false, 0>)
-    if (cold) {
-        if (ppl == 1) return encode5_kernel<false, true, 1, false>;
-        if (ppl == 2) return TGX_E5K(true, 2);
-        if (ppl == 3) return TGX_E5K(true, 3);
-        return TGX_E5K(true, 4);
-    }
-    if (ppl == 1) return encode5_kernel<false, false, 1, false>;
-    if (ppl == 2) return TGX_E5K(false, 2);
-    if (ppl == 3) return TGX_E5K(false, 3);
-    return TGX_E5K(false, 4);
+#define TGX_E5K(C, PL, LN) \
+    (compact == 4 ? encode5_kernel<false, C, PL, false, 4, LN> : compact == 5 ? encode5_kernel<false, C, PL, false, 5, LN> \
+     : compact == 6 ? encode5_kernel<false, C, PL, false, 6, LN> : compact == 7 ? encode5_kernel<false, C, PL, false, 7, LN> \
+     : compact == 8 ? encode5_kernel<false, C, PL, false, 8, LN> : encode5_kernel<false, C, PL, false, 0, LN>)
+#define TGX_E5L(LNH, LNC, LNC3) \
+    if (cold) { \
+        if (ppl == 1) return encode5_kernel<false, true, 1, false, 0, LNC>; \
+        if (ppl == 2) return TGX_E5K(true, 2, LNC); \
+        if (ppl == 3) return TGX_E5K(true, 3, LNC3); \
+        return TGX_E5K(true, 4, LNC); \
+    } \
+    if (ppl == 1) return encode5_kernel<false, false, 1, false, 0, LNH>; \
+    if (ppl == 2) return TGX_E5K(false, 2, LNH); \
+    if (ppl == 3) return TGX_E5K(false, 3, LNH); \
+    return TGX_E5K(false, 4, LNH);
+    if (lean && step_ok) {
+        TGX_E5L(kE5LeanHot, kE5LeanCold, kE5LeanCold3)
+    }
+    if (lean) {
+        TGX_E5L(lean_without_step(kE5LeanHot), lean_without_step(kE5LeanCold), lean_without_step(kE5LeanCold3))
+    }
+    TGX_E5L(0, 0, 0)
+#undef TGX_E5L
 #undef TGX_E5K
 }
 
@@ -1154,9 +1237,9 @@
     return budget > fixed + 64u ? (budget - fixed) / 8u : 0u;
 }
 
-hipError_t encode5_waves_per_simd(bool dropout, bool cold, int ppl, bool long_tokens, int compact, int* out) {
+hipError_t encode5_waves_per_simd(bool dropout, bool cold, int ppl, bool long_tokens, int compact, bool lean, bool step_ok, int* out) {
     hipFuncAttributes attr;
-    hipError_t e = hipFuncGetAttributes(&attr, reinterpret_cast<const void*>(pick_encode5(dropout, cold, ppl, long_tokens, compact)));
+    hipError_t e = hipFuncGetAttributes(&attr, reinterpret_cast<const void*>(pick_encode5(dropout, cold, ppl, long_tokens, compact, lean && encode5_has_lean(dropout, long_tokens), step_ok)));
     if (e != hipSuccess) return e;
     const int regs = (attr.numRegs + 7) & ~7;
     *out = regs > 0 ? (512 / regs > 8 ? 8 : 512 / regs) : 8;
@@ -1178,30 +1261,41 @@
     const uint32_t fixed = encode6_lds_layout(0u, pool, nullptr, nullptr, nullptr) + 512u;
     return budget > fixed + 64u ? (budget - fixed) / 8u : 0u;
 }
-hipError_t launch_encode6(const EncodeParams& p, Encode5Params q, bool cold, uint32_t blocks, hipStream_t stream) {
+static hipError_t lean_lds_check(const void* fn) {
+    hipFuncAttributes attr;
+    const hipError_t e = hipFuncGetAttributes(&attr, fn);
+    if (e != hipSuccess) return e;
+    return attr.sharedSizeBytes == 0 ? hipSuccess : hipErrorInvalidValue;
+}
+
+hipError_t launch_encode6(const EncodeParams& p, Encode5Params q, bool cold, bool lean, uint32_t blocks, hipStream_t stream) {
     q.ring_slots = kE6Slots;
     if (!cold) q.pool = 0u;
     const uint32_t lds = encode6_lds_layout(q.n_hot, q.pool, &q.root_off, &q.ctrl_off, &q.ring_off);
     if (lds > 160u * 1024u || q.n_hot > q.n_values || (!cold && q.n_hot != q.n_values) ||
         (uint64_t)q.n_values + 4ull * kE6Slots * q.pool > 65535ull)
         return hipErrorInvalidValue;
-    auto fn = cold ? (p.dropout > 0.0 ? encode6_kernel<true, true> : encode6_kernel<false, true>)
-                   : (p.dropout > 0.0 ? encode6_kernel<true, false> : encode6_kernel<false, false>);
+    lean = lean && encode5_has_lean(p.dropout > 0.0, false);
+    auto fn = cold ? (p.dropout > 0.0 ? encode6_kernel<true, true> : lean ? encode6_kernel<false, true, kE6Lean> : encode6_kernel<false, true>)
+                   : (p.dropout > 0.0 ? encode6_kernel<true, false> : lean ? encode6_kernel<false, false, kE6Lean> : encode6_kernel<false, false>);
     hipError_t e = hipFuncSetAttribute(reinterpret_cast<const void*>(fn), hipFuncAttributeMaxDynamicSharedMemorySize, 160 * 1024);
     if (e != hipSuccess) return e;
+    if (lean && (e = lean_lds_check(reinterpret_cast<const void*>(fn))) != hipSuccess) return e;
     hipLaunchKernelGGL(fn, dim3(blocks), dim3(64u * (1u + 4u * kE6Walkers)), lds, stream, p, q);
     return hipGetLastError();
 }
 
-hipError_t launch_encode5(const EncodeParams& p, Encode5Params q, bool cold, int ppl, bool long_tokens, int compact, int waves, uint32_t blocks,
-                          uint32_t min_lds, hipStream_t stream) {
+hipError_t launch_encode5(const EncodeParams& p, Encode5Params q, bool cold, int ppl, bool long_tokens, int compact, bool lean, bool step_ok,
+                          int waves, uint32_t blocks, uint32_t min_lds, hipStream_t stream) {
     uint32_t lds = encode5_lds_layout(q.n_hot, long_tokens, waves, ppl, &q.list_off, &q.root_off, &q.idx_off);
     if (lds > 160u * 1024u || q.n_hot > q.n_values || (!cold && q.n_hot != q.n_values) || (long_tokens && ppl != 4) ||
         (compact != 0 && (compact < 4 || compact > 8)))
         return hipErrorInvalidValue;
-    encode5_fn fn = pick_encode5(p.dropout > 0.0, cold, ppl, long_tokens, compact);
+    lean = lean && encode5_has_lean(p.dropout > 0.0, long_tokens);
+    encode5_fn fn = pick_encode5(p.dropout > 0.0, cold, ppl, long_tokens, compact, lean, step_ok);
     hipError_t e = hipFuncSetAttribute(reinterpret_cast<const void*>(fn), hipFuncAttributeMaxDynamicSharedMemorySize, 160 * 1024);
     if (e != hipSuccess) return e;
+    if (lean && (e = lean_lds_check(reinterpret_cast<const void*>(fn))) != hipSuccess) return e;
     if (lds < min_lds && min_lds <= 160u * 1024u) lds = min_lds;
     hipLaunchKernelGGL(fn, dim3(blocks), dim3(64u * (uint32_t)waves), lds, stream, p, q);
     return hipGetLastError();
diff --git a/tokengeex_amd/csrc/kernels.h b/tokengeex_amd/csrc/kernels.h
--- a/tokengeex_amd/csrc/kernels.h
+++ b/tokengeex_amd/csrc/kernels.h
@@ -261,15 +261,18 @@
 hipError_t launch_trace(const EncodeParams& p, uint32_t blocks, hipStream_t stream);
 uint32_t encode5_lds_layout(uint32_t n_hot, bool long_tokens, int waves, int ppl, uint32_t* list_off, uint32_t* root_off, uint32_t* idx_off);
 uint32_t encode5_max_hot(bool long_tokens, int waves, int ppl, uint32_t budget);
-hipError_t encode5_waves_per_simd(bool dropout, bool cold, int ppl, bool long_tokens, int compact, int* out);
+bool encode5_has_lean(bool dropout, bool long_tokens);
+int encode5_lean_items(bool cold, int ppl, bool step_ok);
+int encode6_lean_items();
+hipError_t encode5_waves_per_simd(bool dropout, bool cold, int ppl, bool long_tokens, int compact, bool lean, bool step_ok, int* out);
 uint32_t encode6_lds_layout(uint32_t n_hot, uint32_t pool, uint32_t* root_off, uint32_t* ctrl_off, uint32_t* ring_off);
 uint32_t encode6_max_hot(uint32_t budget, uint32_t pool);
 uint32_t encode6_pool_total(uint32_t pool);
 hipError_t estep5_waves_per_simd(bool dropout, bool cold, int ppl, int* out);
 hipError_t launch_estep5_fwd(const struct Estep4Params& p, Encode5Params q, bool cold, int ppl, int waves, uint32_t blocks, hipStream_t stream);
-hipError_t launch_encode6(const EncodeParams& p, Encode5Params q, bool cold, uint32_t blocks, hipStream_t stream);
-hipError_t launch_encode5(const EncodeParams& p, Encode5Params q, bool cold, int ppl, bool long_tokens, int compact, int waves, uint32_t blocks,
-                          uint32_t min_lds, hipStream_t stream);
+hipError_t launch_encode6(const EncodeParams& p, Encode5Params q, bool cold, bool lean, uint32_t blocks, hipStream_t stream);
+hipError_t launch_encode5(const EncodeParams& p, Encode5Params q, bool cold, int ppl, bool long_tokens, int compact, bool lean, bool step_ok,
+                          int waves, uint32_t blocks, uint32_t min_lds, hipStream_t stream);
 hipError_t launch_encode2(const EncodeParams& p, uint32_t num_cus, bool permuted, hipStream_t stream);
 hipError_t launch_trace32(const EncodeParams& p, uint32_t blocks, bool permuted, hipStream_t stream);
 hipError_t launch_encode4l(const EncodeParams& p, uint32_t num_cus, hipStream_t stream);
diff --git a/tokengeex_amd/csrc/lean_gate.h b/tokengeex_amd/csrc/lean_gate.h
--- /dev/null
+++ b/tokengeex_amd/csrc/lean_gate.h
@@ -0,0 +1,20 @@
+#pragma once
+#include <stddef.h>
+#include <stdint.h>
+#include <string.h>
+
+namespace tgx {
+
+constexpr int kLeanScoreExponent = 960;
+inline bool lean_score_ok(double score) {
+    uint64_t b;
+    memcpy(&b, &score, 8);
+    return (uint32_t)((b >> 52) & 0x7FFu) <= 1023u + (uint32_t)kLeanScoreExponent - 1u;
+}
+inline bool lean_scores_ok(const double* scores, size_t n) {
+    for (size_t i = 0; i < n; i++)
+        if (!lean_score_ok(scores[i])) return false;
+    return true;
+}
+
+}
diff --git a/tokengeex_amd/csrc/tgx_api.cpp b/tokengeex_amd/csrc/tgx_api.cpp
--- a/tokengeex_amd/csrc/tgx_api.cpp
+++ b/tokengeex_amd/csrc/tgx_api.cpp
@@ -25,6 +25,7 @@
 #include "front.h"
 #include "kernels.h"
 #include "layout.h"
+#include "lean_gate.h"
 #include "spans.h"
 #include "nbest.h"
 #include "sample.h"
@@ -259,6 +260,8 @@
     std::vector<double> value_coverage;
     uint32_t n_values = 0, root_base8 = 0;
     uint32_t last_n_hot = 0;
+    bool lean_scores_ok = false;
+    uint32_t last_lean_items = 0;
     bool have_trie8 = false;
     bool encode_tables_ready = false;
     bool estep_trie8_tried = false;
@@ -622,6 +625,7 @@
         fprintf(stderr, "[tgx] encode: S=%llu N=%llu lm=%u path=%s slots=%zu root_base=%u values=%u\n",
                 (unsigned long long)c->n_samples, (unsigned long long)c->n_bytes, p.lm, use4 ? (use5 ? "rows5" : "rows4") : (use2 ? "rows2" : "fused"),
                 m->flat.table.size(), p.root_base, m->n_values);
+    m->last_lean_items = 0;
     if (use5) {
         {
             const tgx_status rst = ensure_value_ranks(m, c);
@@ -712,9 +716,12 @@
         int ppl = 4, bpc = 1, hot_waves = 16;
         int compact = kE5CompactDepth;
         if (const char* e = knob("TGX_E5_COMPACT")) compact = (strcmp(e, "off") == 0 || atoi(e) == 0) ? 0 : std::min(8, std::max(4, atoi(e)));
+        bool lean = tgx::encode5_has_lean(dropout > 0.0, long_tokens);
+        if (const char* e = knob("TGX_E5_LEAN")) lean = lean && atoi(e) != 0;
+        const bool step_ok = m->lean_scores_ok;
         {
             int ps4 = 0;
-            HIP_TRY(tgx::encode5_waves_per_simd(dropout > 0.0, false, 4, long_tokens, compact, &ps4));
+            HIP_TRY(tgx::encode5_waves_per_simd(dropout > 0.0, false, 4, long_tokens, compact, lean, step_ok, &ps4));
             hot_waves = std::min(16, ps4 * 4);
             const int least = long_tokens ? 12 : 13;
             while (hot_waves >= least && m->n_values > tgx::encode5_max_hot(long_tokens, hot_waves, 4, 160u * 1024u)) hot_waves--;
@@ -753,12 +760,12 @@
         const uint32_t budget = 160u * 1024u / (uint32_t)bpc;
         bool cold = false;
         int per_simd = 0;
-        HIP_TRY(tgx::encode5_waves_per_simd(dropout > 0.0, false, ppl, long_tokens, compact, &per_simd));
+        HIP_TRY(tgx::encode5_waves_per_simd(dropout > 0.0, false, ppl, long_tokens, compact, lean, step_ok, &per_simd));
         int waves = std::min(16, (per_simd / bpc) * 4);
         if ((ppl == 4 || ppl == 3) && bpc == 1 && hot_waves > 0) waves = std::min(waves, hot_waves);
         if (m->n_values > tgx::encode5_max_hot(long_tokens, waves, ppl, budget)) {
             cold = true;
-            HIP_TRY(tgx::encode5_waves_per_simd(dropout > 0.0, true, ppl, long_tokens, compact, &per_simd));
+            HIP_TRY(tgx::encode5_waves_per_simd(dropout > 0.0, true, ppl, long_tokens, compact, lean, step_ok, &per_simd));
             waves = std::min(16, (per_simd / bpc) * 4);
         }
         if (balance_waves > 0 && ppl == 4 && bpc == 1) waves = std::min(waves, balance_waves);
@@ -769,6 +776,8 @@
         n_hot = knob_cap_hot("TGX_E5_HOT", n_hot);
         cold = n_hot < m->n_values;
         m->last_n_hot = n_hot;
+        m->last_lean_items = !lean ? 0u : ((rest_n ? (uint32_t)tgx::encode5_lean_items(cold, ppl, step_ok) : 0u) |
+                                           (n_long ? (uint32_t)tgx::encode6_lean_items() << 8 : 0u));
         m->last_encode_waves_per_cu = std::min(bpc, per_simd / ((waves + 3) / 4)) * waves;
         const uint64_t rows_per_block = 4 * (uint64_t)waves;
         const uint32_t blocks5 = (uint32_t)std::max<uint64_t>(
@@ -794,7 +803,7 @@
             q6.pool = cold6 ? pool6 : 0u;
             if (!corun_cus) {
                 time_begin(m, "encode6_kernel");
-                HIP_TRY(tgx::launch_encode6(p6, q6, cold6, blocks6, m->stream));
+                HIP_TRY(tgx::launch_encode6(p6, q6, cold6, lean, blocks6, m->stream));
                 time_end(m);
                 HIP_TRY(hipMemsetAsync(&m->d_ctrl->queue, 0x00, 8, m->stream));
             } else {
@@ -823,7 +832,7 @@
                 p.redo_list = c->d_counts;
                 HIP_TRY(hipMemsetAsync(&m->d_ctrl->encode_redo, 0x00, 8, m->stream));
             }
-            const hipError_t le = tgx::launch_encode5(p, q, cold, ppl, long_tokens, compact, waves, blocks5, corun_cus && n_long ? 84u * 1024u : 0u, m->stream);
+            const hipError_t le = tgx::launch_encode5(p, q, cold, ppl, long_tokens, compact, lean, step_ok, waves, blocks5, corun_cus && n_long ? 84u * 1024u : 0u, m->stream);
             if (le != hipSuccess) return fail(TGX_ERR_DEVICE, "encode5 launch failed: %s", hipGetErrorString(le));
         }
         bool joined = false, joined_slot = false;
@@ -843,7 +852,7 @@
                 }
                 if (timed_out && *started < blocks5) m->corun_wait_timeouts++;
             }
-            const hipError_t l6 = tgx::launch_encode6(p6, q6, cold6, blocks6, m->stream2);
+            const hipError_t l6 = tgx::launch_encode6(p6, q6, cold6, lean, blocks6, m->stream2);
             if (slot) (void)hipEventRecord(m->timed[m->n_timed + 1].stop, m->stream2);
             (void)hipEventRecord(m->ev_join, m->stream2);
             if (l6 != hipSuccess) return fail(TGX_ERR_DEVICE, "encode6 launch failed: %s", hipGetErrorString(l6));
@@ -1167,6 +1176,7 @@
         m->vocab_scores.assign(scores, scores + vocab_size);
         for (uint32_t i = 0; i < vocab_size; i++)
             if (!(scores[i] - scores[i] == 0.0)) m->scores_finite = false;
+        m->lean_scores_ok = tgx::lean_scores_ok(scores, vocab_size);
     } else {
         m->vocab_offs.assign(1, 0);
     }
@@ -4240,3 +4250,4 @@
 uint32_t tgx_encode_corun_timeouts(const tgx_model* m) { return m ? m->corun_wait_timeouts : 0; }
 uint32_t tgx_model_score_values(const tgx_model* m) { return m && m->have_trie8 ? m->n_values : 0u; }
 uint32_t tgx_last_encode_hot_values(const tgx_model* m) { return m ? m->last_n_hot : 0u; }
+uint32_t tgx_last_encode_lean_items(const tgx_model* m) { return m ? m->last_lean_items : 0u; }
```
